# alainjungo/reliability-challenges-uncertainty

Hardware: AMD Instinct MI355X
Metric: MC-sample-volumes/sec (4x160x192x128, T=20) (higher is better)
Workload: dtype f32; 1 GPU; BraTS baseline_mc: 2D U-Net(2,4,depth 4,start_filters 32,dropout 0.05) over 160 slices of 4x192x128, T=20 MC-dropout passes + weight-scaling pass + mean/entropy aggregation per step; T=20, ws_pass=True, slices=160, height=192, width=128, pass_group=4, lanes=2, samples_per_launch=640, outputs=mean + entropy (MultiPredictionSummary() as every shipped script constructs it)

## Files before the change

### reliability-challenges-uncertainty_amd/csrc/rcu_api.hip

```cpp
#include "../../include/rcu.h"
#include "rcu_kernels.h"
#include "rcu_wpack.h"

#include <algorithm>
#include <cmath>
#include <cstdio>
#include <cstring>
#include <map>
#include <memory>
#include <string>
#include <vector>

using namespace rcu;

static thread_local std::string g_last_error;

static int fail(int code, const std::string& msg)
{
    g_last_error = msg;
    return code;
}
int rcu::report_error(int code, const std::string& msg) { return fail(code, msg); }
static int hip_fail(hipError_t e, const char* what)
{
    return fail(RCU_ERR_HIP, std::string(what) + ": " + hipGetErrorString(e));
}
#define RCU_HIP(call)                                      \
    do {                                                   \
        hipError_t e_ = (call);                            \
        if (e_ != hipSuccess) return hip_fail(e_, #call);  \
    } while (0)

static inline int round_up(int v, int m) { return (v + m - 1) / m * m; }

struct ConvLayer {
    std::string name;
    std::string bn;
    std::string name2, bn2;
    int cin1 = 0, cin2 = 0;
    int c1p = 0, c2p = 0;
    int cout = 0;
    int coutp = 0;
    int csplit = 0;
    int H = 0, W = 0;
    int level = 0;
    int gh = 0, gw = 0;
    int upsample = 0, relu = 0;
    int is_1x1 = 0;
    int accumulate = 0;
    int site = -1, site2 = -1;
    int cfg = 0, NT = 0;
    int t_src1 = -1, t_src2 = -1, t_out = -1, t_pool = -1;
    float *wpack = nullptr, *alpha = nullptr, *betab = nullptr, *beta = nullptr;
    size_t wpack_floats = 0;
};

struct Tensor {
    size_t floats_per_slice = 0;
    float* dev = nullptr;
    bool zero_fill = false;
    int H = 0, W = 0, cp = 0;
    int Hr = 0, Wr = 0;
    bool padded() const { return H != Hr || W != Wr; }
    bool blocked = false;
};

struct Workspace {
    std::vector<float*> dev;
    std::vector<size_t> bytes;
    int max_batch = 0;
    ~Workspace()
    {
        for (float* p : dev)
            if (p) (void)hipFree(p);
    }
};

struct rcu_unet {
    rcu_unet_desc d{};
    rcu_unet_options opt{};
    std::shared_ptr<Workspace> ws;
    bool ws_borrowed = false;
    std::vector<ConvLayer> layers;
    std::vector<Tensor> tensors;
    std::vector<std::pair<int, int>> level_ext;
    std::vector<std::pair<std::string, int>> sites;
    std::vector<int> site_offset;
    int mask_floats = 0;
    int in_cp = 0, head_cp = 0, head_cph = 0;
    int t_input = -1, t_head = -1;
    int t_features = -1;
    std::map<std::string, std::vector<float>> host_weights;
    float *w_cls = nullptr, *b_cls = nullptr, *w_sig = nullptr, *b_sig = nullptr;
    double temperature = 1.0;
    bool finalized = false;
    bool plan_only = false;
    int64_t workspace_bytes = 0;
    std::vector<void*> allocs;
    std::vector<hipEvent_t> prof_events;
    int prof_capacity = 0, prof_used = 0;
};

static int prof_slots(const rcu_unet* h) { return (int)h->layers.size() + 3; }

static int new_tensor(rcu_unet* h, int level, int Hr, int Wr, int cp)
{
    Tensor t;
    t.Hr = Hr; t.Wr = Wr; t.cp = cp;
    t.H = level >= 0 ? h->level_ext[level].first : Hr;
    t.W = level >= 0 ? h->level_ext[level].second : Wr;
    t.floats_per_slice = (size_t)t.H * t.W * cp;
    h->tensors.push_back(t);
    return (int)h->tensors.size() - 1;
}

static bool unit_has_dropout(const rcu_unet_desc& d, int level, bool is_down, int i)
{
    if (!d.has_dropout) return false;
    if (d.dropout_center < 0) return true;
    if (level == d.depth) return false;
    if (level + d.dropout_center >= d.depth) return is_down ? (i == 1) : (i == 0);
    return false;
}

static bool is_head_unit(const ConvLayer& L) { return L.name.rfind("conv_cls.0", 0) == 0; }

constexpr long kUpconv4MinItems = 480;
constexpr long long kUpconv4MinPlanPixels = 480LL * 192 * 128;
static bool upconv4_wins(int cfg, const ConvLayer& L, int n_slices)
{
    const ConvConfigInfo& ci = conv_config_info(cfg);
    const long items = (long)((n_slices + ci.TS - 1) / ci.TS) * (L.gh / ci.TH) * (L.gw / ci.TW) * (L.coutp / ci.BN);
    const int l = L.level - 1;
    const long long plan_pixels = (long long)n_slices * ((long long)L.H << l) * ((long long)L.W << l);
    return items >= kUpconv4MinItems && plan_pixels >= kUpconv4MinPlanPixels;
}

static int pick_config(const ConvLayer& L, int n_slices, const rcu_unet_options& opt, int oh, int ow)
{
    const bool wino_on = opt.conv_winograd != 0 && !L.accumulate;
    const int gh = L.gh, gw = L.gw;
    const size_t in_px = (size_t)gh * gw;
    const size_t max_bytes = (size_t)n_slices * std::max(in_px * (size_t)std::max(L.c1p, L.c2p), (size_t)oh * ow * (size_t)L.coutp) * 4;
    const bool center_pad = L.upsample && (2 * (L.H / 2) != L.H || 2 * (L.W / 2) != L.W);
    if (L.upsample && !center_pad && wino_on && L.c1p % 32 == 0 && L.c2p == 0 && max_bytes < ((size_t)1 << 31)) {
        const int lh = gh, lw = gw;
        const int u4_mode = opt.upconv_winograd4;
        const bool u4_fits = u4_mode != 0 && 2 * lh == L.H && 2 * lw == L.W && oh == L.H && ow == L.W &&
                             (size_t)(n_slices + 8) * std::max(in_px * (size_t)L.c1p, (size_t)oh * ow * (size_t)L.coutp) * 4 < ((size_t)1 << 32);
        if (u4_fits) {
            const int cfg4 = (lh % 16 == 0 && lw % 16 == 0) ? CONV_CFG_UPW4_T32x32_N32
                             : (lh % 8 == 0 && lw % 16 == 0) ? CONV_CFG_UPW4_S2T16x32_N32
                             : (lh % 4 == 0 && lw == 8)      ? CONV_CFG_UPW4_S8T8x16_N32
                                                             : -1;
            if (cfg4 >= 0 && (u4_mode == 2 || upconv4_wins(cfg4, L, n_slices))) return cfg4;
        }
        if (L.coutp == 32 && lh % 16 == 0 && lw % 32 == 0) return CONV_CFG_UPW_T16x32_N32;
        if (L.coutp > 32 && lh % 16 == 0 && lw % 16 == 0) return CONV_CFG_UPW_T16x16_N64;
        if (L.coutp > 32 && lh % 8 == 0 && lw % 16 == 0) return CONV_CFG_UPW_S2T8x16_N64;
        if (L.coutp > 32 && lh % 4 == 0 && lw == 8) return CONV_CFG_UPW_S8T4x8_N64;
    }
    if (L.upsample) {
        if (L.coutp <= 32) return (gh % 16 == 0 && gw % 16 == 0) ? CONV_CFG_UP_T16x16_N32 : CONV_CFG_UP_T8x16_N32;
        if (gh == 12 && gw == 8) return CONV_CFG_UP_S2T12x8_N64;
        return CONV_CFG_UP_T8x16_N64;
    }
    if (L.c1p + L.c2p == 8) {
        const bool first_on = opt.conv_first != 0;
        if (first_on && L.c2p == 0 && gh % 8 == 0 && gw % 32 == 0 && (L.coutp == 32 || L.coutp == 64) && L.t_pool < 0 &&
            L.name2.empty() && !L.accumulate)
            return CONV_CFG_FIRST_T8x32;
        return CONV_CFG_T8x16_N32_FIRST;
    }
    if (wino_on && (L.c1p + L.c2p) % 32 == 0 && (L.c2p == 0 || L.c2p == L.c1p) && max_bytes < ((size_t)1 << 31)) {
        const int w4_mode = opt.conv_winograd4;
        const bool lone_head = is_head_unit(L) && L.name2.empty();
        const bool w4_ok = w4_mode != 0 && (L.coutp >= 64 || w4_mode != 3) &&
                           !(lone_head && (opt.head_winograd4 == 0 || L.coutp != 32 || gh % 32 != 0 || gw % 32 != 0));
        if (w4_ok && gw % 32 == 0) {
            if (gh % 32 == 0) return CONV_CFG_WINO4_T32x32_N32;
            if (gh % 16 == 0) return CONV_CFG_WINO4_S2T16x32_N32;
        }
        if (w4_ok && gw == 32 && gh % 8 == 0) return CONV_CFG_WINO4_S4T8x32_N32;
        if (w4_ok && gw == 16 && gh % 8 == 0) return CONV_CFG_WINO4_S8T8x16_N32;
        if (w4_ok && gw == 8 && gh % 12 == 0 && L.t_pool < 0) {
            const long long plan_pixels = (long long)n_slices * ((long long)L.H << L.level) * ((long long)L.W << L.level);
            const long groups2 = (n_slices + 7) / 8;
            const long groups4 = plan_pixels >= kUpconv4MinPlanPixels ? (n_slices + 9) / 10 : groups2;
            const long rounds4 = (groups4 * (gh / 12) * (L.coutp / 32) + 255) / 256;
            const long rounds2 = (groups2 * (gh / 4) * ((L.coutp + 63) / 64) + 255) / 256;
            if (w4_mode == 2 || L.coutp <= 32 || (double)rounds4 * 1.35 < (double)rounds2) return CONV_CFG_WINO4_S8T12x8_N32;
        }
        if (L.coutp == 32 && gh % 16 == 0 && gw % 32 == 0) return CONV_CFG_WINO_T16x32_N32;
        if (L.coutp > 32 && gh % 16 == 0 && gw % 16 == 0) return CONV_CFG_WINO_T16x16_N64;
        if (L.coutp > 32 && gh % 8 == 0 && gw % 16 == 0) return CONV_CFG_WINO_S2T8x16_N64;
        if (L.coutp > 32 && gh % 4 == 0 && gw == 8) return CONV_CFG_WINO_S8T4x8_N64;
    }
    if (L.coutp > 32) {
        if (gh == 12 && gw == 8) return CONV_CFG_S2T12x8_N64;
        const int nt = (L.coutp + 63) / 64;
        const long items = (long)((gh + 7) / 8) * ((gw + 15) / 16) * n_slices * nt;
        const double fill = (double)items / (double)((items + 767) / 768 * 768);
        if (nt == 1 || fill < 0.9) {
            if (gh % 16 == 0 && gw % 16 == 0) return CONV_CFG_T16x16_N64;
            if (gh % 8 == 0 && gw % 16 == 0 && n_slices % 2 == 0) return CONV_CFG_S2T8x16_N64;
        }
        return CONV_CFG_T8x16_N64;
    }
    return (gh % 16 == 0 && gw % 16 == 0) ? CONV_CFG_T16x16_N32 : CONV_CFG_T8x16_N32;
}

static void add_unit(rcu_unet* h, const std::string& prefix, int cin1, int c1p, int cin2, int c2p, int cout, int level, int H, int W,
                     bool dropout, int t_src1, int t_src2, int t_out, int t_pool, bool residual_tail = false)
{
    ConvLayer L;
    L.name = prefix + ".conv2d_batch_relu.conv";
    if (h->d.bn) L.bn = prefix + ".conv2d_batch_relu.bn";
    L.cin1 = cin1; L.c1p = c1p; L.cin2 = cin2; L.c2p = c2p;
    L.cout = cout; L.coutp = round_up(cout, 32); L.csplit = L.coutp;
    L.H = H; L.W = W; L.relu = residual_tail ? 0 : 1;
    L.level = level; L.gh = h->level_ext[level].first; L.gw = h->level_ext[level].second;
    L.accumulate = residual_tail ? 1 : 0;
    if (dropout) {
        L.site = (int)h->sites.size();
        h->sites.push_back({prefix + ".conv2d_batch_relu.dropout", cout});
    }
    L.t_src1 = t_src1; L.t_src2 = t_src2; L.t_out = t_out; L.t_pool = t_pool;
    h->layers.push_back(L);
}

static void add_residual_conv(rcu_unet* h, const std::string& prefix, int cin1, int c1p, int cin2, int c2p, int cout, int level, int H, int W,
                              int t_src1, int t_src2, int t_out)
{
    ConvLayer L;
    L.name = prefix + ".residual";
    L.is_1x1 = 1;
    L.cin1 = cin1; L.c1p = c1p; L.cin2 = cin2; L.c2p = c2p;
    L.cout = cout; L.coutp = round_up(cout, 32); L.csplit = L.coutp;
    L.H = H; L.W = W; L.relu = 0;
    L.level = level; L.gh = h->level_ext[level].first; L.gw = h->level_ext[level].second;
    L.t_src1 = t_src1; L.t_src2 = t_src2; L.t_out = t_out;
    h->layers.push_back(L);
}

static void assign_layouts(rcu_unet* h);

static bool cfg_handles_padding(int cfg) { return conv_config_info(cfg).family.part; }

static int build_plan_for(rcu_unet* h, bool* valid)
{
    const rcu_unet_desc& d = h->d;
    const int depth = d.depth;
    h->layers.clear();
    h->tensors.clear();
    h->sites.clear();
    h->in_cp = round_up(d.in_channels, 8);
    h->t_input = new_tensor(h, 0, d.height, d.width, h->in_cp);
    std::vector<int> skip(depth), skip_c(depth);
    int cur = h->t_input, cur_c = d.in_channels, cur_cp = h->in_cp;
    int c = d.start_filters;
    char buf[128];
    for (int l = 0; l < depth; ++l) {
        const int H = d.height >> l, W = d.width >> l, cp = round_up(c, 32);
        const int t_tmp = new_tensor(h, l, H, W, cp), t_skip = new_tensor(h, l, H, W, cp);
        const int t_pool = new_tensor(h, l + 1, H / 2, W / 2, cp);
        snprintf(buf, sizeof buf, "down_convs.%d.block.block.0", l);
        add_unit(h, buf, cur_c, cur_cp, 0, 0, c, l, H, W, unit_has_dropout(d, l, true, 0), cur, -1, t_tmp, -1);
        if (d.residual) {
            snprintf(buf, sizeof buf, "down_convs.%d.block", l);
            add_residual_conv(h, buf, cur_c, cur_cp, 0, 0, c, l, H, W, cur, -1, t_skip);
        }
        snprintf(buf, sizeof buf, "down_convs.%d.block.block.1", l);
        add_unit(h, buf, c, cp, 0, 0, c, l, H, W, unit_has_dropout(d, l, true, 1), t_tmp, -1, t_skip, t_pool, d.residual != 0);
        skip[l] = t_skip; skip_c[l] = c;
        cur = t_pool; cur_c = c; cur_cp = cp;
        c *= 2;
    }
    {
        const int H = d.height >> depth, W = d.width >> depth, cp = round_up(c, 32);
        const int t_tmp = new_tensor(h, depth, H, W, cp), t_out = new_tensor(h, depth, H, W, cp);
        add_unit(h, "bottom_convs.block.0", cur_c, cur_cp, 0, 0, c, depth, H, W, unit_has_dropout(d, depth, true, 0), cur, -1,
                 t_tmp, -1);
        if (d.residual) add_residual_conv(h, "bottom_convs", cur_c, cur_cp, 0, 0, c, depth, H, W, cur, -1, t_out);
        add_unit(h, "bottom_convs.block.1", c, cp, 0, 0, c, depth, H, W, unit_has_dropout(d, depth, true, 1), t_tmp, -1, t_out,
                 -1, d.residual != 0);
        cur = t_out; cur_c = c; cur_cp = cp;
    }
    for (int j = 0; j < depth; ++j) {
        const int l = depth - 1 - j;
        const int H = d.height >> l, W = d.width >> l;
        const int co = cur_c / 2, cop = round_up(co, 32);
        const int t_up = new_tensor(h, l, H, W, cop), t_tmp = new_tensor(h, l, H, W, cop), t_out = new_tensor(h, l, H, W, cop);
        ConvLayer U;
        snprintf(buf, sizeof buf, "up_convs.%d.upconv.1", j);
        U.name = buf;
        U.cin1 = cur_c; U.c1p = cur_cp; U.cout = co; U.coutp = cop; U.csplit = cop;
        U.H = H; U.W = W; U.upsample = 1; U.relu = 0;
        U.level = l + 1; U.gh = h->level_ext[l + 1].first; U.gw = h->level_ext[l + 1].second;
        U.t_src1 = cur; U.t_out = t_up;
        if (2 * (H / 2) != H || 2 * (W / 2) != W) h->tensors[t_up].zero_fill = true;
        h->layers.push_back(U);
        snprintf(buf, sizeof buf, "up_convs.%d.block.block.0", j);
        add_unit(h, buf, co, cop, skip_c[l], round_up(skip_c[l], 32), co, l, H, W, unit_has_dropout(d, l, false, 0), t_up,
                 skip[l], t_tmp, -1);
        if (d.residual) {
            snprintf(buf, sizeof buf, "up_convs.%d.block", j);
            add_residual_conv(h, buf, co, cop, skip_c[l], round_up(skip_c[l], 32), co, l, H, W, t_up, skip[l], t_out);
        }
        snprintf(buf, sizeof buf, "up_convs.%d.block.block.1", j);
        add_unit(h, buf, co, cop, 0, 0, co, l, H, W, unit_has_dropout(d, l, false, 1), t_tmp, -1, t_out, -1, d.residual != 0);
        cur = t_out; cur_c = co; cur_cp = cop;
    }
    {
        const int cp = round_up(cur_c, 32);
        h->head_cph = cp;
        h->head_cp = d.sigma_out ? 2 * cp : cp;
        h->t_head = new_tensor(h, -1, d.height, d.width, h->head_cp);
        add_unit(h, "conv_cls.0", cur_c, cur_cp, 0, 0, cur_c, 0, d.height, d.width, d.has_dropout != 0, cur, -1, h->t_head,
                 -1);
        ConvLayer& L = h->layers.back();
        if (d.sigma_out) {
            L.name2 = "conv_sigma.0.conv2d_batch_relu.conv";
            if (d.bn) L.bn2 = "conv_sigma.0.conv2d_batch_relu.bn";
            L.csplit = cp;
            L.coutp = 2 * cp;
            if (d.has_dropout) {
                L.site2 = (int)h->sites.size();
                h->sites.push_back({"conv_sigma.0.conv2d_batch_relu.dropout", cur_c});
            }
        }
    }
    h->t_features = -1;
    if (d.provide_features && h->tensors[h->layers.back().t_src1].padded()) {
        const Tensor& f = h->tensors[h->layers.back().t_src1];
        h->t_features = new_tensor(h, -1, f.Hr, f.Wr, f.cp);
    }
    h->site_offset.assign(h->sites.size() + 1, 0);
    for (size_t s = 0; s < h->sites.size(); ++s) h->site_offset[s + 1] = h->site_offset[s] + h->sites[s].second;
    h->mask_floats = h->site_offset.back();
    if (valid) *valid = true;
    for (ConvLayer& L : h->layers) {
        const Tensor& to = h->tensors[L.t_out];
        L.cfg = pick_config(L, h->d.max_batch, h->opt, to.H, to.W);
        const ConvConfigInfo& ci = conv_config_info(L.cfg);
        if ((L.c1p % ci.KC) != 0 || (L.c2p % ci.KC) != 0)
            return fail(RCU_ERR_INVALID, "internal: channel chunking does not divide for layer " + L.name);
        L.NT = (L.coutp + ci.BN - 1) / ci.BN;
        const bool src_padded = h->tensors[L.t_src1].padded() && L.t_src1 != h->t_input;
        const bool first_reads_caller = L.t_src1 == h->t_input && h->tensors[L.t_src1].padded();
        const bool out_padded = to.padded() && !(L.upsample && !cfg_handles_padding(L.cfg) && !h->tensors[L.t_src1].padded());
        if ((src_padded || first_reads_caller || out_padded) && !cfg_handles_padding(L.cfg) && valid) *valid = false;
    }
    assign_layouts(h);
    return RCU_OK;
}

static double plan_cost(const rcu_unet* h)
{
    double total = 0.0;
    for (const ConvLayer& L : h->layers) {
        const ConvConfigInfo& ci = conv_config_info(L.cfg);
        const double tiles = (double)((L.gh + ci.TH - 1) / ci.TH) * ((L.gw + ci.TW - 1) / ci.TW);
        const double px = tiles * ci.TH * ci.TW;
        const double kn = (double)(L.c1p + L.c2p) * (double)(L.NT * ci.BN);
        double eff = 0.0;
        switch (ci.family.id) {
            case ConvFamily::First: eff = 0.25; break;
            case ConvFamily::Wino4: eff = (L.c1p + L.c2p) <= 32 ? 0.45 : 0.58; break;
            case ConvFamily::Wino2Up: eff = 0.72; break;
            case ConvFamily::Wino4Up: eff = 0.70; break;
            case ConvFamily::Wino2: eff = 0.62; break;
            case ConvFamily::DirectUp: eff = 0.72; break;
            case ConvFamily::Direct: eff = 0.75; break;
        }
        total += px * kn * (ci.family.mults * ci.slot_factor) / eff;
    }
    return total;
}

static int choose_level_extents(rcu_unet* h)
{
    const rcu_unet_desc& d = h->d;
    h->level_ext.resize(d.depth + 1);
    for (int l = 0; l <= d.depth; ++l) h->level_ext[l] = {d.height >> l, d.width >> l};
    bool valid = true;
    int rc = build_plan_for(h, &valid);
    if (rc != RCU_OK || h->opt.pad_levels == 0 || h->opt.conv_winograd == 0) return rc;
    double best = plan_cost(h);
    static const int kRound[] = {4, 8, 12, 16, 32};
    for (int sweep = 0; sweep < 2; ++sweep)
        for (int l = 0; l <= d.depth; ++l) {
            const int Hl = d.height >> l, Wl = d.width >> l;
            std::pair<int, int> keep = h->level_ext[l];
            for (int rh : kRound)
                for (int rw : kRound) {
                    const std::pair<int, int> cand = {round_up(Hl, rh), round_up(Wl, rw)};
                    if (cand == keep || (rw == 12)) continue;
                    h->level_ext[l] = cand;
                    rc = build_plan_for(h, &valid);
                    if (rc != RCU_OK) return rc;
                    const double cost = plan_cost(h);
                    if (valid && cost < best * 0.999) {
                        best = cost;
                        keep = cand;
                    }
                }
            h->level_ext[l] = keep;
        }
    return build_plan_for(h, &valid);
}

static int build_plan(rcu_unet* h) { return choose_level_extents(h); }

static void assign_layouts(rcu_unet* h)
{
    const bool on = h->opt.act_layout == 0;
    for (Tensor& t : h->tensors) t.blocked = on && t.cp % 8 == 0 && !t.zero_fill;
    h->tensors[h->t_input].blocked = false;
    h->tensors[h->t_head].blocked = false;
    if (h->d.provide_features) h->tensors[h->layers.back().t_src1].blocked = false;
    for (bool changed = true; changed;) {
        changed = false;
        auto clear = [&](int t) {
            if (t >= 0 && h->tensors[t].blocked) {
                h->tensors[t].blocked = false;
                changed = true;
            }
        };
        for (const ConvLayer& L : h->layers) {
            const ConvFamilyTraits& family = conv_config_info(L.cfg).family;
            if (!family.reads_blocked) {
                clear(L.t_src1);
                clear(L.t_src2);
            }
            if (!family.writes_blocked) {
                clear(L.t_out);
                clear(L.t_pool);
            }
            if (L.t_src2 >= 0 && h->tensors[L.t_src1].blocked != h->tensors[L.t_src2].blocked) {
                clear(L.t_src1);
                clear(L.t_src2);
            }
        }
    }
}

extern "C" const char* rcu_last_error(void) { return g_last_error.c_str(); }
extern "C" const char* rcu_version(void) { return "librcu_hip 0.1.0 gfx950"; }

extern "C" void rcu_unet_default_options(rcu_unet_options* opts)
{
    if (!opts) return;
    std::memset(opts, 0, sizeof *opts);
    opts->conv_winograd = 1;
    opts->conv_winograd4 = 1;
    opts->conv_first = 1;
    opts->act_layout = 0;
    opts->fuse_head = 1;
    opts->head_winograd4 = 1;
    opts->pad_levels = 1;
    opts->upconv_winograd4 = 1;
}

static int make_plan(const rcu_unet_desc* desc, const rcu_unet_options* opts, const rcu_unet* donor, rcu_unet** out)
{
    if (!desc || !out) return fail(RCU_ERR_INVALID, "rcu_unet_create: null argument");
    const rcu_unet_desc& d = *desc;
    if (d.nb_classes < 1 || d.nb_classes > MAX_CLASSES) return fail(RCU_ERR_INVALID, "nb_classes must be in 1..8");
    if (d.in_channels < 1 || d.depth < 1 || d.depth > 8 || d.start_filters < 1 || d.max_batch < 1)
        return fail(RCU_ERR_INVALID, "rcu_unet_create: bad in_channels / depth / start_filters / max_batch");
    if (d.in_channels > 8 && d.in_channels % 32 != 0)
        return fail(RCU_ERR_INVALID, "in_channels must be <= 8 or a multiple of 32");
    const int div = 1 << d.depth;
    if (d.height < div || d.width < div)
        return fail(RCU_ERR_INVALID, "height and width must be at least 2^depth (one pixel at the bottom level)");
    rcu_unet_options o;
    rcu_unet_default_options(&o);
    if (opts) {
        o = *opts;
        if ((o.conv_winograd | 1) != 1 || (o.conv_winograd4 < 0 || o.conv_winograd4 > 3) ||
            (o.conv_first | 1) != 1 || (o.act_layout | 1) != 1 || (o.fuse_head | 1) != 1 || (o.head_winograd4 | 1) != 1 || (o.pad_levels | 1) != 1 ||
            (o.upconv_winograd4 < 0 || o.upconv_winograd4 > 2))
            return fail(RCU_ERR_INVALID, "rcu_unet_create_with: bad rcu_unet_options value");
    }
    rcu_unet* h = new rcu_unet();
    h->d = d;
    h->opt = o;
    if (donor && donor->ws && donor->ws->max_batch >= d.max_batch) h->d.max_batch = donor->ws->max_batch;
    int rc = build_plan(h);
    if (rc != RCU_OK) {
        delete h;
        return rc;
    }
    *out = h;
    return RCU_OK;
}

extern "C" int rcu_unet_plan(const rcu_unet_desc* desc, const rcu_unet_options* opts, rcu_unet** out)
{
    int rc = make_plan(desc, opts, nullptr, out);
    if (rc == RCU_OK) (*out)->plan_only = true;
    return rc;
}

extern "C" int rcu_unet_create_with(const rcu_unet_desc* desc, const rcu_unet_options* opts, rcu_unet* donor, rcu_unet** out)
{
    rcu_unet* h = nullptr;
    int rc = make_plan(desc, opts, donor, &h);
    if (rc != RCU_OK) return rc;
    const rcu_unet_desc& d = *desc;
    for (const Tensor& t : h->tensors)
        if (t.floats_per_slice * (size_t)h->d.max_batch >= (size_t)1 << 31) {
            delete h;
            return fail(RCU_ERR_INVALID, "max_batch too large: an activation tensor would exceed 2^31 elements");
        }
    if (donor) {
        bool same = donor->ws && donor->tensors.size() == h->tensors.size() && donor->ws->max_batch >= d.max_batch;
        for (size_t i = 0; same && i < h->tensors.size(); ++i) {
            const Tensor &a = h->tensors[i], &b = donor->tensors[i];
            same = a.floats_per_slice == b.floats_per_slice && a.H == b.H && a.W == b.W && a.Hr == b.Hr && a.Wr == b.Wr && a.cp == b.cp &&
                   a.blocked == b.blocked && a.zero_fill == b.zero_fill;
        }
        if (!same) {
            delete h;
            return fail(RCU_ERR_INVALID, "rcu_unet_create_with: the workspace donor's plan differs (shape, options) or is sized for a smaller batch");
        }
        h->ws = donor->ws;
        h->ws_borrowed = true;
        for (size_t i = 0; i < h->tensors.size(); ++i) h->tensors[i].dev = h->ws->dev[i];
        *out = h;
        return RCU_OK;
    }
    h->ws = std::make_shared<Workspace>();
    h->ws->max_batch = d.max_batch;
    bool zeroed = false;
    for (Tensor& t : h->tensors) {
        const size_t bytes = t.floats_per_slice * (size_t)d.max_batch * sizeof(float);
        hipError_t e = hipMalloc(reinterpret_cast<void**>(&t.dev), bytes);
        if (e != hipSuccess) {
            rcu_unet_destroy(h);
            return hip_fail(e, "hipMalloc(activation workspace)");
        }
        h->ws->dev.push_back(t.dev);
        h->ws->bytes.push_back(bytes);
        h->workspace_bytes += (int64_t)bytes;
        if (t.zero_fill || t.padded()) {
            e = hipMemset(t.dev, 0, bytes);
            if (e != hipSuccess) {
                rcu_unet_destroy(h);
                return hip_fail(e, "hipMemset(centre-pad border / level padding)");
            }
            zeroed = true;
        }
    }
    if (zeroed) {
        hipError_t e = hipStreamSynchronize(nullptr);
        if (e != hipSuccess) {
            rcu_unet_destroy(h);
            return hip_fail(e, "hipStreamSynchronize(level padding)");
        }
    }
    *out = h;
    return RCU_OK;
}

extern "C" int rcu_unet_create(const rcu_unet_desc* desc, rcu_unet** out) { return rcu_unet_create_with(desc, nullptr, nullptr, out); }

extern "C" int rcu_unet_set_fuse_head(rcu_unet* h, int on)
{
    if (!h) return fail(RCU_ERR_INVALID, "rcu_unet_set_fuse_head: null handle");
    h->opt.fuse_head = on ? 1 : 0;
    return RCU_OK;
}

extern "C" int rcu_unet_set_temperature(rcu_unet* h, double temperature)
{
    if (!h) return fail(RCU_ERR_INVALID, "rcu_unet_set_temperature: null handle");
    if (!std::isfinite(temperature) || !(temperature > 0.0))
        return fail(RCU_ERR_INVALID, "rcu_unet_set_temperature: the temperature must be finite and > 0");
    if (h->d.sigma_out)
        return fail(RCU_ERR_INVALID, "rcu_unet_set_temperature: a sigma_out model's sigma is in logit units; scaling the logits alone is not defined");
    if (h->finalized) return fail(RCU_ERR_STATE, "rcu_unet_set_temperature after rcu_unet_finalize_weights");
    h->temperature = temperature;
    return RCU_OK;
}

extern "C" int rcu_unet_destroy(rcu_unet* h)
{
    if (!h) return RCU_OK;
    for (void* p : h->allocs) (void)hipFree(p);
    for (hipEvent_t e : h->prof_events) (void)hipEventDestroy(e);
    delete h;
    return RCU_OK;
}

extern "C" int64_t rcu_unet_workspace_bytes(const rcu_unet* h) { return h ? h->workspace_bytes : 0; }
extern "C" int rcu_unet_num_dropout_sites(const rcu_unet* h) { return h ? (int)h->sites.size() : 0; }
extern "C" int rcu_unet_dropout_site_channels(const rcu_unet* h, int site)
{
    if (!h || site < 0 || site >= (int)h->sites.size()) return fail(RCU_ERR_INVALID, "bad dropout site index");
    return h->sites[site].second;
}
extern "C" const char* rcu_unet_dropout_site_name(const rcu_unet* h, int site)
{
    if (!h || site < 0 || site >= (int)h->sites.size()) return "";
    return h->sites[site].first.c_str();
}
extern "C" int rcu_unet_mask_floats_per_sample(const rcu_unet* h) { return h ? h->mask_floats : 0; }

extern "C" int rcu_unet_load_weight(rcu_unet* h, const char* name, const float* data, size_t count)
{
    if (!h || !name || (!data && count)) return fail(RCU_ERR_INVALID, "rcu_unet_load_weight: null argument");
    std::string key(name);
    if (key.rfind("module.", 0) == 0) key = key.substr(7);
    h->host_weights[key].assign(data, data + count);
    h->finalized = false;
    return RCU_OK;
}

static int get_weight(rcu_unet* h, const std::string& key, size_t count, const std::vector<float>** out)
{
    auto it = h->host_weights.find(key);
    if (it == h->host_weights.end()) return fail(RCU_ERR_WEIGHTS, "missing weight tensor '" + key + "'");
    if (it->second.size() != count)
        return fail(RCU_ERR_WEIGHTS, "weight tensor '" + key + "' has " + std::to_string(it->second.size()) +
                                         " elements, expected " + std::to_string(count));
    *out = &it->second;
    return RCU_OK;
}

template <typename T>
static int upload(rcu_unet* h, const std::vector<T>& host, T** dev)
{
    RCU_HIP(hipMalloc(reinterpret_cast<void**>(dev), host.size() * sizeof(T)));
    h->allocs.push_back(*dev);
    h->workspace_bytes += (int64_t)(host.size() * sizeof(T));
    RCU_HIP(hipMemcpy(*dev, host.data(), host.size() * sizeof(T), hipMemcpyHostToDevice));
    return RCU_OK;
}

static int fold_conv(rcu_unet* h, const ConvLayer& L, const std::string& conv, const std::string& bn, int co0,
                     std::vector<float>& wpack, std::vector<float>& alpha, std::vector<float>& betab,
                     std::vector<float>& beta)
{
    const int cin = L.cin1 + L.cin2;
    const std::vector<float>*w, *b;
    std::vector<float> w_centre;
    int rc;
    if (L.is_1x1) {
        if ((rc = get_weight(h, conv + ".weight", (size_t)L.cout * cin, &w))) return rc;
        w_centre.assign((size_t)L.cout * cin * 9, 0.f);
        for (size_t i = 0; i < (size_t)L.cout * cin; ++i) w_centre[i * 9 + 4] = (*w)[i];
        w = &w_centre;
    } else {
        rc = get_weight(h, conv + ".weight", (size_t)L.cout * cin * 9, &w);
    }
    if (rc) return rc;
    rc = get_weight(h, conv + ".bias", (size_t)L.cout, &b);
    if (rc) return rc;
    const std::vector<float>*g = nullptr, *bt = nullptr, *mu = nullptr, *var = nullptr;
    if (!bn.empty()) {
        if ((rc = get_weight(h, bn + ".weight", L.cout, &g))) return rc;
        if ((rc = get_weight(h, bn + ".bias", L.cout, &bt))) return rc;
        if ((rc = get_weight(h, bn + ".running_mean", L.cout, &mu))) return rc;
        if ((rc = get_weight(h, bn + ".running_var", L.cout, &var))) return rc;
    }
    for (int co = 0; co < L.cout; ++co) {
        float A = 1.f, B = 0.f;
        if (g) {
            A = (*g)[co] / std::sqrt((*var)[co] + 1e-5f);
            B = (*bt)[co] - A * (*mu)[co];
        }
        alpha[co0 + co] = A;
        betab[co0 + co] = A * (*b)[co];
        beta[co0 + co] = B;
    }
    pack_conv_weights(wpack_kernel(conv_config_info(L.cfg)), WpackLayer{L.cin1, L.c1p, L.cin2, L.cout, L.NT, L.upsample}, w->data(), co0, wpack.data());
    return RCU_OK;
}

extern "C" int rcu_unet_finalize_weights(rcu_unet* h)
{
    if (!h) return fail(RCU_ERR_INVALID, "null handle");
    if (h->plan_only) return fail(RCU_ERR_STATE, "rcu_unet_finalize_weights: the handle is a plan without a workspace (rcu_unet_plan)");
    if (h->finalized) return RCU_OK;
    for (ConvLayer& L : h->layers) {
        const ConvConfigInfo& ci = conv_config_info(L.cfg);
        L.wpack_floats = wpack_floats(wpack_kernel(ci), L.c1p + L.c2p, L.NT);
        std::vector<float> wpack(L.wpack_floats, 0.f);
        const int cpad = L.NT * ci.BN;
        std::vector<float> alpha(cpad, 0.f), betab(cpad, 0.f), beta(cpad, 0.f);
        int rc = fold_conv(h, L, L.name, L.bn, 0, wpack, alpha, betab, beta);
        if (rc) return rc;
        if (!L.name2.empty()) {
            rc = fold_conv(h, L, L.name2, L.bn2, L.csplit, wpack, alpha, betab, beta);
            if (rc) return rc;
        }
        if ((rc = upload(h, wpack, &L.wpack))) return rc;
        if ((rc = upload(h, alpha, &L.alpha))) return rc;
        if ((rc = upload(h, betab, &L.betab))) return rc;
        if ((rc = upload(h, beta, &L.beta))) return rc;
    }
    const int C = h->d.nb_classes, cph = h->head_cph, creal = h->layers.back().cout;
    auto head = [&](const std::string& key, float** w_dev, float** b_dev, double temperature) -> int {
        const std::vector<float>*w, *b;
        int rc = get_weight(h, key + ".weight", (size_t)C * creal, &w);
        if (rc) return rc;
        if ((rc = get_weight(h, key + ".bias", (size_t)C, &b))) return rc;
        auto scaled = [temperature](float v) { return temperature == 1.0 ? v : (float)((double)v / temperature); };
        std::vector<float> wp((size_t)C * cph, 0.f);
        for (int c = 0; c < C; ++c)
            for (int k = 0; k < creal; ++k) wp[(size_t)c * cph + k] = scaled((*w)[(size_t)c * creal + k]);
        if ((rc = upload(h, wp, w_dev))) return rc;
        std::vector<float> bp(b->size());
        for (size_t c = 0; c < b->size(); ++c) bp[c] = scaled((*b)[c]);
        return upload(h, bp, b_dev);
    };
    int rc = head("conv_cls.1", &h->w_cls, &h->b_cls, h->temperature);
    if (rc) return rc;
    if (h->d.sigma_out && (rc = head("conv_sigma.1", &h->w_sig, &h->b_sig, 1.0))) return rc;
    h->host_weights.clear();
    h->finalized = true;
    return RCU_OK;
}

static bool head_fusable(const rcu_unet* h)
{
    const ConvLayer& last = h->layers.back();
    return conv_config_info(last.cfg).head_cfg >= 0 && h->d.nb_classes == 2 && last.name2.empty() && h->head_cph == 32;
}

struct FusedHead {
    float* logits;
    void* stats;
    int flags;
    int passes;
};

static int run_layer(rcu_unet* h, const ConvLayer& L, int n, const float* masks, hipStream_t stream, const FusedHead* head = nullptr,
                     const float* x_nchw = nullptr, int n_images = 0)
{
    const ConvConfigInfo& ci = conv_config_info(L.cfg);
    ConvArgs a{};
    a.src1 = h->tensors[L.t_src1].dev;
    a.src2 = L.t_src2 >= 0 ? h->tensors[L.t_src2].dev : nullptr;
    a.wpack = L.wpack; a.alpha = L.alpha; a.betab = L.betab; a.beta = L.beta;
    a.mask = (masks && L.site >= 0) ? masks + (size_t)n * h->site_offset[L.site] : nullptr;
    a.mask2 = (masks && L.site2 >= 0) ? masks + (size_t)n * h->site_offset[L.site2] : nullptr;
    a.out = h->tensors[L.t_out].dev;
    a.pooled = L.t_pool >= 0 ? h->tensors[L.t_pool].dev : nullptr;
    const int gh = L.gh, gw = L.gw;
    a.N = n; a.H = gh; a.W = gw;
    const Tensor& tsrc = h->tensors[L.t_src1];
    const Tensor& tout = h->tensors[L.t_out];
    const int os = L.upsample ? 2 : 1;
    if (cfg_handles_padding(L.cfg)) {
        const bool pool_differs = L.t_pool >= 0 && (h->tensors[L.t_pool].H != gh / 2 || h->tensors[L.t_pool].W != gw / 2);
        if (tsrc.padded() || tout.H != os * gh || tout.W != os * gw || pool_differs) {
            a.part = 1;
            a.Hr = L.upsample ? 2 * (L.H / 2) : L.H;
            a.Wr = L.upsample ? 2 * (L.W / 2) : L.W;
            a.out_H = tout.H; a.out_W = tout.W;
            if (L.t_pool >= 0) { a.pool_H = h->tensors[L.t_pool].H; a.pool_W = h->tensors[L.t_pool].W; }
        }
    } else if (L.t_pool >= 0 && h->tensors[L.t_pool].padded()) {
        a.pool_H = h->tensors[L.t_pool].H; a.pool_W = h->tensors[L.t_pool].W;
    } else if (L.upsample && (2 * gh != tout.H || 2 * gw != tout.W)) {
        a.out_H = tout.H; a.out_W = tout.W;
        a.out_y0 = (L.H - 2 * gh) / 2; a.out_x0 = (L.W - 2 * gw) / 2;
    }
    a.C1 = L.c1p; a.C2 = L.c2p; a.CoutP = L.coutp;
    a.cin_real = L.cin1;
    a.x_nchw = ci.family.id == ConvFamily::First ? x_nchw : nullptr;
    a.n_images = n_images;
    a.Cmask = L.cout; a.Csplit = L.csplit; a.Cmask2 = L.cout;
    a.relu = L.relu;
    a.accumulate = L.accumulate;
    a.tiles_y = (gh + ci.TH - 1) / ci.TH;
    a.tiles_x = (gw + ci.TW - 1) / ci.TW;
    a.slice_groups = (n + ci.TS - 1) / ci.TS;
    a.NT = L.NT;
    a.NTW_total = L.NT * ci.family.weight_sets;
    {
        const unsigned long long items = (unsigned long long)a.NTW_total * a.tiles_x * a.tiles_y * a.slice_groups;
        auto magic = [&](int d) -> uint32_t {
            return (d > 1 && items * (unsigned long long)d < (1ull << 32)) ? (uint32_t)(((1ull << 32) + d - 1) / d) : 0u;
        };
        a.magic_ntw = magic(a.NTW_total); a.magic_tx = magic(a.tiles_x); a.magic_ty = magic(a.tiles_y);
    }
    {
        auto strides = [](const Tensor& t, uint32_t& pix_bytes, uint32_t& chunk_bytes) {
            pix_bytes = t.blocked ? 32u : (uint32_t)t.cp * 4u;
            chunk_bytes = t.blocked ? (uint32_t)(t.H * t.W) * 32u : 32u;
        };
        strides(h->tensors[L.t_src1], a.in_pix_bytes, a.in_chunk_bytes);
        strides(h->tensors[L.t_out], a.out_pix_bytes, a.out_chunk_bytes);
        if (L.t_pool >= 0) strides(h->tensors[L.t_pool], a.pool_pix_bytes, a.pool_chunk_bytes);
    }
    a.src1_bytes = (uint32_t)std::min<size_t>(h->tensors[L.t_src1].floats_per_slice * (size_t)n * 4, 0xFFFFFFFFu);
    a.src2_bytes = L.t_src2 >= 0 ? (uint32_t)std::min<size_t>(h->tensors[L.t_src2].floats_per_slice * (size_t)n * 4, 0xFFFFFFFFu) : 0u;
    a.wpack_bytes = (uint32_t)std::min<size_t>(L.wpack_floats * 4, 0xFFFFFFFFu);
    int cfg = L.cfg;
    if (head) {
        cfg = ci.head_cfg;
        a.head_w = h->w_cls; a.head_b = h->b_cls;
        a.head_logits = head->logits; a.head_stats = head->stats; a.head_flags = head->flags;
        a.head_passes = head->passes;
        a.head_images = n / head->passes;
        a.head_V = (size_t)a.head_images * L.H * L.W;
    }
    RCU_HIP(launch_conv3x3(cfg, a, stream));
    return RCU_OK;
}

struct HeadSampling {
    const uint64_t* keys;
    uint64_t first_sample;
    int samples;
};

struct HeadVotes {
    uint32_t* plane;
    int n_words;
    const int32_t* bits;
};

static int forward_impl(rcu_unet* h, const float* x, int n, const float* masks, float* logits, float* sigma, void* stats,
                        int flags, hipStream_t stream, int passes = 1, float* sigma_sum = nullptr, int sigma_log = 0,
                        const HeadSampling* sampling = nullptr, const HeadVotes* votes = nullptr)
{
    if (!h || !x) return fail(RCU_ERR_INVALID, "rcu_unet_forward: null argument");
    if (!h->finalized) return fail(RCU_ERR_STATE, "rcu_unet_forward before rcu_unet_finalize_weights");
    if (n < 1 || passes < 1 || (long)n * passes > h->d.max_batch)
        return fail(RCU_ERR_INVALID, "batch size (times passes) outside 1..max_batch");
    if (passes > 1 && (!stats || logits || sigma)) return fail(RCU_ERR_INVALID, "pass groups only feed the statistics");
    const int n_one = n;
    n *= passes;
    if ((sigma || sigma_sum) && !h->d.sigma_out) return fail(RCU_ERR_INVALID, "sigma output requested from a model without sigma_out");
    hipEvent_t* ev = nullptr;
    if (h->prof_capacity > 0 && h->prof_used < h->prof_capacity)
        ev = h->prof_events.data() + (size_t)(h->prof_used++) * prof_slots(h);
    if (ev) RCU_HIP(hipEventRecord(*ev++, stream));
    const bool direct_input = conv_config_info(h->layers.front().cfg).family.id == ConvFamily::First;
    if (!direct_input)
        RCU_HIP(launch_pack_input(x, h->tensors[h->t_input].dev, n_one, h->d.in_channels, h->in_cp, h->d.height, h->d.width,
                                  h->tensors[h->t_input].H, h->tensors[h->t_input].W, passes, stream));
    if (ev) RCU_HIP(hipEventRecord(*ev++, stream));
    const ConvLayer& last = h->layers.back();
    const bool fuse = head_fusable(h) && sigma == nullptr && (logits != nullptr || stats != nullptr) && h->opt.fuse_head != 0 && sampling == nullptr &&
                      votes == nullptr;
    for (const ConvLayer& L : h->layers) {
        const FusedHead fh{logits, stats, flags, passes};
        int rc = run_layer(h, L, n, masks, stream, (fuse && &L == &last) ? &fh : nullptr, direct_input ? x : nullptr, n_one);
        if (rc) return rc;
        if (ev) RCU_HIP(hipEventRecord(*ev++, stream));
    }
    if (h->t_features >= 0) {
        const Tensor& f = h->tensors[h->layers.back().t_src1];
        RCU_HIP(launch_crop_nhwc(f.dev, h->tensors[h->t_features].dev, n, f.Hr, f.Wr, f.H, f.W, f.cp, stream));
    }
    if (fuse) {
        if (ev) RCU_HIP(hipEventRecord(*ev++, stream));
        return RCU_OK;
    }
    HeadArgs a{};
    a.act = h->tensors[h->t_head].dev;
    a.w_cls = h->w_cls; a.b_cls = h->b_cls; a.w_sig = h->w_sig; a.b_sig = h->b_sig;
    a.logits = logits; a.sigma = sigma; a.stats = stats;
    a.sigma_sum = sigma_sum; a.sigma_log = sigma_log;
    a.C = h->d.nb_classes; a.CP = h->head_cp; a.CPh = h->head_cph; a.stats_flags = flags;
    a.HW = (size_t)h->d.height * h->d.width;
    a.V = a.HW * n_one;
    a.passes = passes;
    if (sampling) {
        static_assert(sizeof(unsigned long long) == sizeof(uint64_t), "pass keys");
        RCU_HIP(launch_head_sampled(a, reinterpret_cast<const unsigned long long*>(sampling->keys), sampling->first_sample, sampling->samples, stream));
    } else if (votes) {
        RCU_HIP(launch_head_votes(a, votes->plane, votes->n_words, votes->bits, stream));
    } else {
        RCU_HIP(launch_head(a, stream));
    }
    if (ev) RCU_HIP(hipEventRecord(*ev++, stream));
    return RCU_OK;
}

extern "C" int rcu_unet_profile_begin(rcu_unet* h, int max_forwards)
{
    if (!h || max_forwards < 0) return fail(RCU_ERR_INVALID, "rcu_unet_profile_begin: bad argument");
    for (hipEvent_t e : h->prof_events) (void)hipEventDestroy(e);
    h->prof_events.clear();
    h->prof_capacity = h->prof_used = 0;
    const size_t total = (size_t)max_forwards * prof_slots(h);
    h->prof_events.resize(total);
    for (size_t i = 0; i < total; ++i) {
        hipError_t e = hipEventCreate(&h->prof_events[i]);
        if (e != hipSuccess) {
            h->prof_events.resize(i);
            return hip_fail(e, "hipEventCreate");
        }
    }
    h->prof_capacity = max_forwards;
    return RCU_OK;
}

extern "C" int rcu_unet_profile_collect(rcu_unet* h, double* ms_sum, int* forwards)
{
    if (!h || !ms_sum || !forwards) return fail(RCU_ERR_INVALID, "rcu_unet_profile_collect: null argument");
    const int slots = prof_slots(h);
    for (int i = 0; i < slots - 1; ++i) ms_sum[i] = 0.0;
    for (int f = 0; f < h->prof_used; ++f) {
        hipEvent_t* ev = h->prof_events.data() + (size_t)f * slots;
        RCU_HIP(hipEventSynchronize(ev[slots - 1]));
        for (int i = 0; i < slots - 1; ++i) {
            float ms = 0.f;
            RCU_HIP(hipEventElapsedTime(&ms, ev[i], ev[i + 1]));
            ms_sum[i] += ms;
        }
    }
    *forwards = h->prof_used;
    h->prof_used = 0;
    return RCU_OK;
}

extern "C" int rcu_unet_forward(rcu_unet* h, const float* x_dev, int n, const float* masks_dev, float* logits_dev,
                                float* sigma_dev, void* stream)
{
    return forward_impl(h, x_dev, n, masks_dev, logits_dev, sigma_dev, nullptr, 0, static_cast<hipStream_t>(stream));
}

extern "C" int rcu_unet_forward_accumulate(rcu_unet* h, const float* x_dev, int n, const float* masks_dev, void* stats_dev,
                                           int flags, void* stream)
{
    if (!stats_dev) return fail(RCU_ERR_INVALID, "rcu_unet_forward_accumulate: null stats");
    return forward_impl(h, x_dev, n, masks_dev, nullptr, nullptr, stats_dev, flags & (RCU_MC_MI | RCU_MC_VAR | RCU_MC_EXACT),
                        static_cast<hipStream_t>(stream));
}

extern "C" int rcu_unet_forward_accumulate_sigma(rcu_unet* h, const float* x_dev, int n, const float* masks_dev, void* stats_dev,
                                                 int flags, float* sigma_sum_dev, int is_log_sigma, void* stream)
{
    if (!stats_dev || !sigma_sum_dev) return fail(RCU_ERR_INVALID, "rcu_unet_forward_accumulate_sigma: null stats / sigma sum");
    return forward_impl(h, x_dev, n, masks_dev, nullptr, nullptr, stats_dev, flags & (RCU_MC_MI | RCU_MC_VAR | RCU_MC_EXACT),
                        static_cast<hipStream_t>(stream), 1, sigma_sum_dev, is_log_sigma ? 1 : 0);
}

extern "C" int rcu_unet_forward_accumulate_sigma_passes(rcu_unet* h, const float* x_dev, int n, int passes, const float* masks_dev,
                                                        void* stats_dev, int flags, float* sigma_sum_dev, int is_log_sigma, void* stream)
{
    if (!stats_dev || !sigma_sum_dev) return fail(RCU_ERR_INVALID, "rcu_unet_forward_accumulate_sigma_passes: null stats / sigma sum");
    return forward_impl(h, x_dev, n, masks_dev, nullptr, nullptr, stats_dev, flags & (RCU_MC_MI | RCU_MC_VAR | RCU_MC_EXACT),
                        static_cast<hipStream_t>(stream), passes, sigma_sum_dev, is_log_sigma ? 1 : 0);
}

extern "C" int rcu_unet_forward_sample_sigma_passes(rcu_unet* h, const float* x_dev, int n, int passes, const float* masks_dev,
                                                    const uint64_t* keys_host, uint64_t first_sample, int samples, void* stats_dev, int flags,
                                                    float* sigma_sum_dev, int is_log_sigma, void* stream)
{
    const char* fn = "rcu_unet_forward_sample_sigma_passes";
    if (!h) return fail(RCU_ERR_INVALID, std::string(fn) + ": null handle");
    if (!x_dev || !keys_host || !stats_dev || !sigma_sum_dev)
        return fail(RCU_ERR_INVALID, std::string(fn) + ": null x_dev / keys_host / stats_dev / sigma_sum_dev");
    if (!h->d.sigma_out) return fail(RCU_ERR_INVALID, std::string(fn) + ": the handle has no sigma head (sigma_out = 0)");
    if (n < 1 || passes < 1 || (long)n * passes > h->d.max_batch)
        return fail(RCU_ERR_INVALID, std::string(fn) + ": batch size (times passes) outside 1..max_batch");
    if (int st = check_logit_sampling_shape(fn, (size_t)n, (size_t)h->d.height * h->d.width, h->d.nb_classes, samples)) return st;
    const HeadSampling sampling{keys_host, first_sample, samples};
    return forward_impl(h, x_dev, n, masks_dev, nullptr, nullptr, stats_dev, flags & (RCU_MC_MI | RCU_MC_VAR | RCU_MC_EXACT),
                        static_cast<hipStream_t>(stream), passes, sigma_sum_dev, is_log_sigma ? 1 : 0, &sampling);
}

extern "C" int rcu_unet_features(const rcu_unet* h, const float** features_dev, int* channels, int* channel_pitch)
{
    if (!h || !features_dev) return fail(RCU_ERR_INVALID, "rcu_unet_features: null argument");
    if (!h->finalized) return fail(RCU_ERR_STATE, "rcu_unet_features before rcu_unet_finalize_weights");
    for (const ConvLayer& L : h->layers)
        if (L.name == "conv_cls.0.conv2d_batch_relu.conv") {
            if (h->tensors[L.t_src1].blocked || (h->tensors[L.t_src1].padded() && h->t_features < 0))
                return fail(RCU_ERR_STATE, "rcu_unet_features: the handle was created without rcu_unet_desc.provide_features (the feature "
                                           "tensor is held channel-blocked / on a padded level)");
            *features_dev = h->t_features >= 0 ? h->tensors[h->t_features].dev : h->tensors[L.t_src1].dev;
            if (channels) *channels = L.cin1;
            if (channel_pitch) *channel_pitch = L.c1p;
            return RCU_OK;
        }
    return fail(RCU_ERR_STATE, "rcu_unet_features: no conv_cls layer in the plan");
}

struct rcu_postnet {
    int in_channels = 0, nb_classes = 0, nb_convs = 0, bn = 1;
    std::map<std::string, std::vector<float>> host_weights;
    float* packed = nullptr;
    float* packed_mc = nullptr;
    bool finalized = false;
};

extern "C" int rcu_postnet_create(int in_channels, int nb_classes, int nb_convs, int bn, rcu_postnet** out)
{
    if (!out) return fail(RCU_ERR_INVALID, "rcu_postnet_create: null argument");
    if (in_channels < 1 || in_channels > 32 * PN_MAX_BLOCKS)
        return fail(RCU_ERR_INVALID, "PostNet kernel handles 1.." + std::to_string(32 * PN_MAX_BLOCKS) + " feature channels");
    if (nb_classes < 1 || nb_classes > 32) return fail(RCU_ERR_INVALID, "PostNet kernel handles 1..32 classes");
    if (nb_convs < 0 || nb_convs + 1 > PN_MAX_LAYERS)
        return fail(RCU_ERR_INVALID, "PostNet kernel handles at most " + std::to_string(PN_MAX_LAYERS - 1) + " hidden convs");
    const int cb = (in_channels + 31) / 32;
    if ((size_t)(nb_convs + 1) * pn_layer_floats(cb) * sizeof(float) > 160 * 1024)
        return fail(RCU_ERR_INVALID, "PostNet: the packed layers of " + std::to_string(nb_convs) + " hidden convs over " +
                                         std::to_string(in_channels) + " channels do not fit the 160 KB of LDS");
    rcu_postnet* h = new rcu_postnet;
    h->in_channels = in_channels; h->nb_classes = nb_classes; h->nb_convs = nb_convs; h->bn = bn ? 1 : 0;
    *out = h;
    return RCU_OK;
}

extern "C" void rcu_postnet_destroy(rcu_postnet* h)
{
    if (!h) return;
    if (h->packed) (void)hipFree(h->packed);
    if (h->packed_mc) (void)hipFree(h->packed_mc);
    delete h;
}

extern "C" int rcu_postnet_load_weight(rcu_postnet* h, const char* name, const float* data, size_t count)
{
    if (!h || !name || (!data && count)) return fail(RCU_ERR_INVALID, "rcu_postnet_load_weight: null argument");
    std::string key(name);
    if (key.rfind("module.", 0) == 0) key = key.substr(7);
    h->host_weights[key].assign(data, data + count);
    h->finalized = false;
    return RCU_OK;
}

static int postnet_weight(rcu_postnet* h, const std::string& key, size_t count, const std::vector<float>** out)
{
    auto it = h->host_weights.find(key);
    if (it == h->host_weights.end()) return fail(RCU_ERR_WEIGHTS, "missing weight tensor '" + key + "'");
    if (it->second.size() != count)
        return fail(RCU_ERR_WEIGHTS, "weight tensor '" + key + "' has " + std::to_string(it->second.size()) +
                                         " elements, expected " + std::to_string(count));
    *out = &it->second;
    return RCU_OK;
}

static void postnet_pack_layer(int cb, const std::vector<float>& w, const std::vector<float>& start, const std::vector<float>& after,
                               float* dst)
{
    const int cp = 32 * cb;
    for (int cob = 0; cob < cb; ++cob)
        for (int cib = 0; cib < cb; ++cib)
            for (int j = 0; j < 4; ++j)
                for (int lane = 0; lane < 64; ++lane)
                    for (int e = 0; e < 4; ++e)
                        dst[((((cob * cb + cib) * 4 + j) * 64) + lane) * 4 + e] =
                            w[(size_t)(32 * cob + (lane & 31)) * cp + 32 * cib + 8 * j + 4 * (lane >> 5) + e];
    float* bd = dst + cb * cb * 1024;
    for (int which = 0; which < 2; ++which)
        for (int cob = 0; cob < cb; ++cob)
            for (int j = 0; j < 4; ++j)
                for (int hf = 0; hf < 2; ++hf)
                    for (int e = 0; e < 4; ++e)
                        bd[which * cb * 32 + ((cob * 4 + j) * 2 + hf) * 4 + e] = (which ? after : start)[32 * cob + 8 * j + 4 * hf + e];
}

extern "C" int rcu_postnet_finalize_weights(rcu_postnet* h)
{
    if (!h) return fail(RCU_ERR_INVALID, "rcu_postnet_finalize_weights: null handle");
    const int C = h->in_channels, L = h->nb_convs + 1, cb = (C + 31) / 32, cp = 32 * cb;
    const size_t layer = pn_layer_floats(cb);
    std::vector<float> packed((size_t)L * layer, 0.f), packed_mc((size_t)L * layer, 0.f);
    for (int l = 0; l < L; ++l) {
        const bool last = (l == h->nb_convs);
        const std::string pre = last ? "conv_logits" : "convs." + std::to_string(l) + ".conv2d_batch_relu.conv";
        const int cout = last ? h->nb_classes : C;
        const std::vector<float>*w, *b;
        int rc = postnet_weight(h, pre + ".weight", (size_t)cout * C, &w);
        if (rc) return rc;
        if ((rc = postnet_weight(h, pre + ".bias", cout, &b))) return rc;
        std::vector<float> wf((size_t)cp * cp, 0.f), b_conv(cp, 0.f), b_shift(cp, 0.f), b_all(cp, 0.f);
        for (int o = 0; o < cout; ++o) {
            float alpha = 1.f, beta = 0.f, mean = 0.f;
            if (!last && h->bn) {
                const std::string bp = "convs." + std::to_string(l) + ".conv2d_batch_relu.bn";
                const std::vector<float>*g, *be, *rm, *rv;
                if ((rc = postnet_weight(h, bp + ".weight", C, &g))) return rc;
                if ((rc = postnet_weight(h, bp + ".bias", C, &be))) return rc;
                if ((rc = postnet_weight(h, bp + ".running_mean", C, &rm))) return rc;
                if ((rc = postnet_weight(h, bp + ".running_var", C, &rv))) return rc;
                alpha = (float)((double)(*g)[o] / std::sqrt((double)(*rv)[o] + 1e-5));
                beta = (*be)[o];
                mean = (*rm)[o];
            }
            for (int i = 0; i < C; ++i) wf[(size_t)o * cp + i] = alpha * (*w)[(size_t)o * C + i];
            b_all[o] = alpha * ((*b)[o] - mean) + beta;
            b_conv[o] = alpha * (*b)[o];
            b_shift[o] = beta - alpha * mean;
        }
        postnet_pack_layer(cb, wf, b_all, std::vector<float>(cp, 0.f), packed.data() + (size_t)l * layer);
        postnet_pack_layer(cb, wf, last ? b_all : b_conv, b_shift, packed_mc.data() + (size_t)l * layer);
    }
    if (!h->packed) RCU_HIP(hipMalloc(reinterpret_cast<void**>(&h->packed), packed.size() * sizeof(float)));
    if (!h->packed_mc) RCU_HIP(hipMalloc(reinterpret_cast<void**>(&h->packed_mc), packed_mc.size() * sizeof(float)));
    RCU_HIP(hipMemcpy(h->packed, packed.data(), packed.size() * sizeof(float), hipMemcpyHostToDevice));
    RCU_HIP(hipMemcpy(h->packed_mc, packed_mc.data(), packed_mc.size() * sizeof(float), hipMemcpyHostToDevice));
    h->finalized = true;
    return RCU_OK;
}

extern "C" int rcu_postnet_forward(rcu_postnet* h, const float* features_dev, int channel_pitch, int n, int hw,
                                   const float* masks_dev, float* logits_dev, void* stream)
{
    if (!h || !features_dev || !logits_dev) return fail(RCU_ERR_INVALID, "rcu_postnet_forward: null argument");
    if (!h->finalized) return fail(RCU_ERR_STATE, "rcu_postnet_forward before rcu_postnet_finalize_weights");
    if (n < 0 || hw < 1) return fail(RCU_ERR_INVALID, "rcu_postnet_forward: bad shape");
    const int cb = (h->in_channels + 31) / 32;
    if (channel_pitch < 32 * cb || channel_pitch % 4)
        return fail(RCU_ERR_INVALID, "rcu_postnet_forward: channel pitch must be >= in_channels rounded up to 32 and a multiple of 4");
    RCU_HIP(launch_postnet(features_dev, channel_pitch, (size_t)n * hw, hw, masks_dev ? h->packed_mc : h->packed, h->nb_convs + 1,
                           h->nb_classes, h->in_channels, masks_dev, logits_dev, static_cast<hipStream_t>(stream)));
    return RCU_OK;
}

extern "C" int rcu_unet_forward_accumulate_passes(rcu_unet* h, const float* x_dev, int n, int passes, const float* masks_dev,
                                                  void* stats_dev, int flags, void* stream)
{
    if (!stats_dev) return fail(RCU_ERR_INVALID, "rcu_unet_forward_accumulate_passes: null stats");
    return forward_impl(h, x_dev, n, masks_dev, nullptr, nullptr, stats_dev, flags & (RCU_MC_MI | RCU_MC_VAR | RCU_MC_EXACT),
                        static_cast<hipStream_t>(stream), passes);
}

static int check_vote_plane(const std::string& fn, int n_words)
{
    if (n_words < 1 || n_words > RCU_VOTES_MAX_PASSES / 32) return fail(RCU_ERR_INVALID, fn + ": n_words must be in 1..2, got " + std::to_string(n_words));
    return RCU_OK;
}
static int check_vote_bit(const std::string& fn, int bit, int n_words)
{
    if (bit < 0 || bit >= 32 * n_words)
        return fail(RCU_ERR_INVALID, fn + ": bit " + std::to_string(bit) + " outside [0, " + std::to_string(32 * n_words) + ")");
    return RCU_OK;
}

extern "C" int rcu_unet_forward_accumulate_votes(rcu_unet* h, const float* x_dev, int n, int passes, const float* masks_dev, void* stats_dev,
                                                 int flags, uint32_t* votes_dev, int n_words, const int32_t* bits_host, void* stream)
{
    const std::string fn = "rcu_unet_forward_accumulate_votes";
    if (!h) return fail(RCU_ERR_INVALID, fn + ": null handle");
    if (!x_dev || !stats_dev || !votes_dev || !bits_host) return fail(RCU_ERR_INVALID, fn + ": null x_dev / stats_dev / votes_dev / bits_host");
    if (int st = check_vote_plane(fn, n_words)) return st;
    if (h->d.nb_classes < 1 || h->d.nb_classes > MAX_CLASSES) return fail(RCU_ERR_INVALID, fn + ": nb_classes must be in 1..8");
    if (n < 1 || passes < 1 || (long)n * passes > h->d.max_batch) return fail(RCU_ERR_INVALID, fn + ": batch size (times passes) outside 1..max_batch");
    for (int t = 0; t < passes; ++t)
        if (int st = check_vote_bit(fn, bits_host[t], n_words)) return st;
    const HeadVotes votes{votes_dev, n_words, bits_host};
    return forward_impl(h, x_dev, n, masks_dev, nullptr, nullptr, stats_dev, flags & (RCU_MC_MI | RCU_MC_VAR | RCU_MC_EXACT),
                        static_cast<hipStream_t>(stream), passes, nullptr, 0, nullptr, &votes);
}

extern "C" int rcu_mc_votes(const float* in_dev, size_t n, size_t hw, int nb_classes, int flags, uint32_t* votes_dev, int n_words, int bit, void* stream)
{
    const std::string fn = "rcu_mc_votes";
    if (!in_dev || !votes_dev) return fail(RCU_ERR_INVALID, fn + ": null in_dev / votes_dev");
    if (int st = check_vote_plane(fn, n_words)) return st;
    if (int st = check_vote_bit(fn, bit, n_words)) return st;
    if (nb_classes < 1 || nb_classes > MAX_CLASSES) return fail(RCU_ERR_INVALID, fn + ": nb_classes must be in 1..8");
    if (n * hw == 0) return RCU_OK;
    RCU_HIP(launch_mc_votes(in_dev, nb_classes, n, hw, flags & RCU_MC_INPUT_PROBS, votes_dev, bit, static_cast<hipStream_t>(stream)));
    return RCU_OK;
}

extern "C" int rcu_unet_num_layers(const rcu_unet* h) { return h ? (int)h->layers.size() : 0; }

extern "C" int rcu_unet_layer_info(const rcu_unet* h, int layer, rcu_layer_info* out)
{
    if (!h || !out || layer < 0 || layer >= (int)h->layers.size()) return fail(RCU_ERR_INVALID, "bad layer index");
    const ConvLayer& L = h->layers[layer];
    std::memset(out, 0, sizeof *out);
    std::snprintf(out->name, sizeof out->name, "%s", L.name.c_str());
    std::snprintf(out->kernel, sizeof out->kernel, "%s", conv_config_info(L.cfg).kernel_name);
    out->cin = L.cin1 + L.cin2;
    out->cout = L.name2.empty() ? L.cout : 2 * L.cout;
    out->height = L.H; out->width = L.W;
    out->grid_height = L.gh; out->grid_width = L.gw;
    out->upsample = L.upsample; out->pooled = L.t_pool >= 0; out->dual_source = L.t_src2 >= 0;
    out->head_fusable = (layer + 1 == (int)h->layers.size() && head_fusable(h)) ? 1 : 0;
    out->flops_per_slice = 2.0 * out->cin * out->cout * (L.is_1x1 ? 1.0 : 9.0) * (L.upsample ? 4.0 * (L.H / 2) * (L.W / 2) : (double)L.H * L.W);
    {
        const ConvConfigInfo& ci = conv_config_info(L.cfg);
        const double tiles = (double)((L.gh + ci.TH - 1) / ci.TH) * ((L.gw + ci.TW - 1) / ci.TW);
        const double px = tiles * ci.TH * ci.TW;
        const double ncols = (double)L.NT * ci.BN;
        const int k = ci.family.id == ConvFamily::First ? (L.cin1 > 4 ? 8 : 4) : L.c1p + L.c2p;
        out->mfma_flops_per_slice = 2.0 * k * ncols * ci.family.mults * px * ci.slot_factor;
    }
    return RCU_OK;
}

extern "C" int rcu_unet_run_layer(rcu_unet* h, int layer, int n, const float* masks_dev, void* stream)
{
    if (!h || layer < 0 || layer >= (int)h->layers.size()) return fail(RCU_ERR_INVALID, "bad layer index");
    if (!h->finalized) return fail(RCU_ERR_STATE, "rcu_unet_run_layer before rcu_unet_finalize_weights");
    if (n < 1 || n > h->d.max_batch) return fail(RCU_ERR_INVALID, "batch size outside 1..max_batch");
    return run_layer(h, h->layers[layer], n, masks_dev, static_cast<hipStream_t>(stream));
}

static int check_classes(int c)
{
    if (c < 1 || c > MAX_CLASSES) return fail(RCU_ERR_INVALID, "nb_classes must be in 1..8");
    return RCU_OK;
}

extern "C" size_t rcu_mc_stats_bytes(size_t n, size_t hw, int C, int flags)
{
    const size_t V = n * hw;
    const size_t mi = (flags & RCU_MC_MI) ? 1 : 0;
    if (flags & (RCU_MC_VAR | RCU_MC_EXACT)) return V * ((size_t)C + ((flags & RCU_MC_VAR) ? (size_t)C : 0) + mi) * sizeof(double);
    return V * ((size_t)C + mi) * sizeof(float);
}

extern "C" int rcu_mc_begin(void* stats, size_t n, size_t hw, int C, int flags, void* stream)
{
    if (!stats) return fail(RCU_ERR_INVALID, "rcu_mc_begin: null stats");
    if (check_classes(C)) return RCU_ERR_INVALID;
    RCU_HIP(hipMemsetAsync(stats, 0, rcu_mc_stats_bytes(n, hw, C, flags), static_cast<hipStream_t>(stream)));
    return RCU_OK;
}

extern "C" int rcu_mc_accumulate(const float* in, void* stats, size_t n, size_t hw, int C, int flags, void* stream)
{
    if (!in || !stats) return fail(RCU_ERR_INVALID, "rcu_mc_accumulate: null argument");
    if (check_classes(C)) return RCU_ERR_INVALID;
    if (n * hw == 0) return RCU_OK;
    RCU_HIP(launch_mc_accumulate(in, stats, C, n, hw, flags, static_cast<hipStream_t>(stream)));
    return RCU_OK;
}

extern "C" int rcu_mc_finalize(const void* stats, size_t n, size_t hw, int C, int T, int flags, float* mean, float* entropy,
                               float* mi, float* var, void* stream)
{
    if (!stats) return fail(RCU_ERR_INVALID, "rcu_mc_finalize: null stats");
    if (check_classes(C)) return RCU_ERR_INVALID;
    if (T < 1) return fail(RCU_ERR_INVALID, "rcu_mc_finalize: T must be >= 1");
    if (mi && !(flags & RCU_MC_MI)) return fail(RCU_ERR_INVALID, "mutual_info requested without RCU_MC_MI statistics");
    if (var && !(flags & RCU_MC_VAR)) return fail(RCU_ERR_INVALID, "variance requested without RCU_MC_VAR statistics");
    if ((flags & RCU_MC_EXACT) && T > RCU_MC_EXACT_MAX_PASSES)
        return fail(RCU_ERR_INVALID, "RCU_MC_EXACT statistics hold at most 2048 passes (sums of multiples of 2^-40 below 2^13)");
    if (n * hw == 0) return RCU_OK;
    RCU_HIP(launch_mc_finalize(stats, C, n, hw, T, flags, mean, entropy, mi, var, static_cast<hipStream_t>(stream)));
    return RCU_OK;
}

extern "C" int rcu_softmax(const float* logits, float* probs, size_t n, size_t hw, int C, void* stream)
{
    if (!logits || !probs) return fail(RCU_ERR_INVALID, "rcu_softmax: null argument");
    if (check_classes(C)) return RCU_ERR_INVALID;
    if (n * hw == 0) return RCU_OK;
    RCU_HIP(launch_softmax_nchw(logits, probs, C, n, hw, static_cast<hipStream_t>(stream)));
    return RCU_OK;
}

extern "C" int rcu_aleatoric(const float* logits, const float* sigma_raw, size_t n, size_t hw, int C, int is_log_sigma,
                             float* probs, float* sigma, uint8_t* prediction, float* sigma_pred, void* stream)
{
    if (!logits || !sigma_raw) return fail(RCU_ERR_INVALID, "rcu_aleatoric: null argument");
    if (check_classes(C)) return RCU_ERR_INVALID;
    if (n * hw == 0) return RCU_OK;
    RCU_HIP(launch_aleatoric(logits, sigma_raw, C, n, hw, is_log_sigma, probs, sigma, prediction, sigma_pred,
                             static_cast<hipStream_t>(stream)));
    return RCU_OK;
}

extern "C" int rcu_prediction_and_foreground(const float* probs, size_t n, size_t hw, int C, uint8_t* prediction,
                                             float* p_fg, void* stream)
{
    if (!probs) return fail(RCU_ERR_INVALID, "rcu_prediction_and_foreground: null argument");
    if (check_classes(C)) return RCU_ERR_INVALID;
    if (n * hw == 0) return RCU_OK;
    RCU_HIP(launch_argmax_fg(probs, C, n, hw, prediction, p_fg, static_cast<hipStream_t>(stream)));
    return RCU_OK;
}

static int draw_dropout_masks(const std::string& fn, const uint64_t* seeds, int passes, int n, uint64_t first_sample, const int64_t* sample_index_dev,
                              const int32_t* site_channels, const float* site_keep, int n_sites, float* out, void* stream)
{
    if (!seeds || !site_channels || !site_keep || !out) return fail(RCU_ERR_INVALID, fn + ": null argument");
    if (passes < 1 || n < 1 || n_sites < 1 || n_sites > MASK_MAX_SITES) return fail(RCU_ERR_INVALID, fn + ": passes, n >= 1 and 1 <= n_sites <= 40");
    MaskArgs a{};
    long end = 0;
    for (int s = 0; s < n_sites; ++s) {
        if (site_channels[s] < 1 || !(site_keep[s] <= 1.f)) return fail(RCU_ERR_INVALID, fn + ": site_channels >= 1, site_keep <= 1");
        end += (long)n * site_channels[s];
        if (end * (long)passes >= (1l << 31)) return fail(RCU_ERR_INVALID, fn + ": more than 2^31 factors");
        a.site_end[s] = (int)end;
        a.site_keep[s] = site_keep[s];
        a.site_ch[s] = site_channels[s];
        a.site_off[s] = a.per_sample;
        a.per_sample += site_channels[s];
    }
    a.first_sample = first_sample;
    a.sites = n_sites;
    a.per_pass = (int)end;
    a.passes = passes;
    for (a.first = 0; a.first < passes; a.first += MASK_MAX_PASSES) {
        a.count = std::min(MASK_MAX_PASSES, passes - a.first);
        for (int t = 0; t < a.count; ++t) a.seed[t] = seeds[a.first + t];
        if (sample_index_dev) {
            RCU_HIP(launch_dropout_masks_indexed(a, reinterpret_cast<const long long*>(sample_index_dev), out, static_cast<hipStream_t>(stream)));
        } else {
            RCU_HIP(launch_dropout_masks(a, out, static_cast<hipStream_t>(stream)));
        }
    }
    return RCU_OK;
}

extern "C" int rcu_dropout_masks(const uint64_t* seeds, int passes, int n, uint64_t first_sample, const int32_t* site_channels,
                                 const float* site_keep, int n_sites, float* out, void* stream)
{
    return draw_dropout_masks("rcu_dropout_masks", seeds, passes, n, first_sample, nullptr, site_channels, site_keep, n_sites, out, stream);
}

static int check_adaptive_shape(const char* fn, size_t n, size_t hw, int C)
{
    if (check_classes(C)) return RCU_ERR_INVALID;
    if (n < 1 || hw < 1 || n > ((size_t)1 << 20) || hw > ((size_t)1 << 30))
        return fail(RCU_ERR_INVALID, std::string(fn) + ": n must be in 1..2^20 and hw in 1..2^30");
    return RCU_OK;
}

extern "C" int rcu_mc_slice_scores(const void* stats_dev, size_t n, size_t hw, int C, int flags, int64_t thr_q, uint32_t* unsettled_dev,
                                   int64_t* margin_q_dev, void* stream)
{
    if (!stats_dev || !unsettled_dev || !margin_q_dev) return fail(RCU_ERR_INVALID, "rcu_mc_slice_scores: null argument");
    if (check_adaptive_shape("rcu_mc_slice_scores", n, hw, C)) return RCU_ERR_INVALID;
    if (!(flags & RCU_MC_EXACT) || (flags & ~(RCU_MC_MI | RCU_MC_VAR | RCU_MC_EXACT)))
        return fail(RCU_ERR_INVALID, "rcu_mc_slice_scores: needs RCU_MC_EXACT statistics (the decision is made on exact integer sums), got flags " +
                                         std::to_string(flags));
    if (thr_q < 0) return fail(RCU_ERR_INVALID, "rcu_mc_slice_scores: thr_q must be >= 0");
    if (reinterpret_cast<uintptr_t>(stats_dev) % 8 != 0) return fail(RCU_ERR_INVALID, "rcu_mc_slice_scores: stats must be 8-byte aligned");
    RCU_HIP(launch_mc_slice_scores(stats_dev, C, n, hw, (long long)thr_q, unsettled_dev, reinterpret_cast<long long*>(margin_q_dev),
                                   static_cast<hipStream_t>(stream)));
    return RCU_OK;
}

extern "C" int rcu_dropout_masks_indexed(const uint64_t* seeds, int passes, int n, const int64_t* sample_index_dev, const int32_t* site_channels,
                                         const float* site_keep, int n_sites, float* out, void* stream)
{
    if (!sample_index_dev) return fail(RCU_ERR_INVALID, "rcu_dropout_masks_indexed: null argument");
    return draw_dropout_masks("rcu_dropout_masks_indexed", seeds, passes, n, 0, sample_index_dev, site_channels, site_keep, n_sites, out, stream);
}

extern "C" int rcu_mc_merge_slices(const void* src_stats_dev, size_t m, void* dst_stats_dev, size_t n, size_t hw, int C, int flags,
                                   const int32_t* index_dev, void* stream)
{
    if (!src_stats_dev || !dst_stats_dev || !index_dev) return fail(RCU_ERR_INVALID, "rcu_mc_merge_slices: null argument");
    if (check_adaptive_shape("rcu_mc_merge_slices", n, hw, C) || check_adaptive_shape("rcu_mc_merge_slices", m, hw, C)) return RCU_ERR_INVALID;
    if (flags & ~(RCU_MC_MI | RCU_MC_VAR | RCU_MC_EXACT))
        return fail(RCU_ERR_INVALID, "rcu_mc_merge_slices: flags must be a combination of RCU_MC_MI, RCU_MC_VAR and RCU_MC_EXACT, got " +
                                         std::to_string(flags));
    const uintptr_t s = reinterpret_cast<uintptr_t>(src_stats_dev), d = reinterpret_cast<uintptr_t>(dst_stats_dev);
    const size_t element = (flags & (RCU_MC_VAR | RCU_MC_EXACT)) ? 8 : 4;
    if (s % element != 0 || d % element != 0) return fail(RCU_ERR_INVALID, "rcu_mc_merge_slices: blobs must be aligned to their element");
    if (s < d + rcu_mc_stats_bytes(n, hw, C, flags) && d < s + rcu_mc_stats_bytes(m, hw, C, flags))
        return fail(RCU_ERR_INVALID, "rcu_mc_merge_slices: src and dst must not overlap");
    RCU_HIP(launch_mc_merge_slices(src_stats_dev, m, dst_stats_dev, n, hw, C, flags, index_dev, static_cast<hipStream_t>(stream)));
    return RCU_OK;
}

extern "C" int rcu_mc_finalize_counts(const void* stats, size_t n, size_t hw, int C, const int32_t* counts_dev, int flags, float* mean,
                                      float* entropy, float* mi, float* var, void* stream)
{
    if (!stats || !counts_dev) return fail(RCU_ERR_INVALID, "rcu_mc_finalize_counts: null argument");
    if (check_classes(C)) return RCU_ERR_INVALID;
    if (mi && !(flags & RCU_MC_MI)) return fail(RCU_ERR_INVALID, "mutual_info requested without RCU_MC_MI statistics");
    if (var && !(flags & RCU_MC_VAR)) return fail(RCU_ERR_INVALID, "variance requested without RCU_MC_VAR statistics");
    if (n * hw == 0) return RCU_OK;
    RCU_HIP(launch_mc_finalize_counts(stats, C, n, hw, counts_dev, flags, mean, entropy, mi, var, static_cast<hipStream_t>(stream)));
    return RCU_OK;
}

static_assert(sizeof(rcu_ece_result) == sizeof(EceResult), "ABI struct mismatch");
static_assert(RCU_MAX_BINS == MAX_BINS && RCU_MAX_THRESHOLDS == MAX_THR, "ABI constant mismatch");

extern "C" int rcu_ece_thresholds(int n_bins, float* thr)
{
    if (n_bins < 1 || n_bins > MAX_BINS || !thr) return fail(RCU_ERR_INVALID, "n_bins must be in 1..32");
    const double stop = 1.0 + 1e-8, step = stop / n_bins;
    for (int k = 1; k < n_bins; ++k) {
        const double edge = k * step;
        float t = (float)edge;
        if ((double)t < edge) t = std::nextafterf(t, INFINITY);
        thr[k - 1] = t;
    }
    return RCU_OK;
}

extern "C" size_t rcu_ece_workspace_bytes(size_t n, int nv) { return ece_workspace_bytes(n, nv < 1 ? 1 : nv); }

extern "C" int rcu_ece_hist(const float* p, const uint8_t* target, const uint8_t* mask, size_t n, int n_volumes,
                            const float* thr, int n_bins, rcu_ece_result* result, void* workspace, void* stream)
{
    if (!result || !thr || (n && (!p || !target || !workspace)))
        return fail(RCU_ERR_INVALID, "rcu_ece_hist: null argument");
    if (n_bins < 1 || n_bins > MAX_BINS || n_volumes < 1) return fail(RCU_ERR_INVALID, "rcu_ece_hist: bad n_bins / n_volumes");
    RCU_HIP(launch_ece_hist(p, target, mask, n, n_volumes, thr, n_bins, reinterpret_cast<EceResult*>(result), workspace,
                            static_cast<hipStream_t>(stream)));
    return RCU_OK;
}

extern "C" int rcu_ece_bin_ids(const float* p, size_t n, const float* thr, int n_bins, uint8_t* ids, void* stream)
{
    if ((n && (!p || !ids)) || !thr) return fail(RCU_ERR_INVALID, "rcu_ece_bin_ids: null argument");
    if (n_bins < 1 || n_bins > MAX_BINS) return fail(RCU_ERR_INVALID, "n_bins must be in 1..32");
    RCU_HIP(launch_bin_ids(p, n, thr, n_bins, ids, static_cast<hipStream_t>(stream)));
    return RCU_OK;
}

extern "C" int rcu_calib_set_blocks_per_workgroup(int ece_blocks, int unc_blocks)
{
    if (ece_blocks < 0 || unc_blocks < 0) return fail(RCU_ERR_INVALID, "rcu_calib_set_blocks_per_workgroup: negative block count");
    calib_set_blocks_per_workgroup(ece_blocks, unc_blocks);
    return RCU_OK;
}

extern "C" size_t rcu_unc_workspace_bytes(size_t n, int nv) { return unc_workspace_bytes(n, nv < 1 ? 1 : nv); }

extern "C" int rcu_unc_counts(const void* unc, int unc_is_f64, const uint8_t* prediction, const uint8_t* target,
                              const uint8_t* mask, size_t n, int n_volumes, const double* thr, int n_thr, uint64_t* counts,
                              void* workspace, void* stream)
{
    if (!counts || !thr || (n && (!unc || !prediction || !target || !workspace)))
        return fail(RCU_ERR_INVALID, "rcu_unc_counts: null argument");
    if (n_thr < 1 || n_thr > MAX_THR || n_volumes < 1)
        return fail(RCU_ERR_INVALID, "rcu_unc_counts: n_thr must be in 1..16 and n_volumes >= 1");
    RCU_HIP(launch_unc_counts(unc, unc_is_f64, prediction, target, mask, n, n_volumes, thr, n_thr,
                              reinterpret_cast<unsigned long long*>(counts), workspace, static_cast<hipStream_t>(stream)));
    return RCU_OK;
}

extern "C" int rcu_unc_from_p_num_thresholds(void) { return unc_from_p_num_thresholds(); }
extern "C" double rcu_unc_from_p_threshold(int i) { return unc_from_p_threshold(i); }
extern "C" int rcu_unc_from_p_supported(const double* thr, int n_thr) { return (thr && unc_from_p_supported(thr, n_thr)) ? 1 : 0; }
extern "C" int rcu_unc_from_p_exceeded(float p, const double* thr, int n_thr)
{
    if (!thr || n_thr < 1 || n_thr > MAX_THR) return -1;
    return unc_from_p_exceeded_host(p, thr, n_thr);
}
extern "C" size_t rcu_unc_from_p_workspace_bytes(size_t n, int nv) { return unc_from_p_workspace_bytes(n, nv < 1 ? 1 : nv); }

extern "C" int rcu_unc_counts_from_p(const float* p, const uint8_t* prediction, const uint8_t* target, const uint8_t* mask, size_t n,
                                     int n_volumes, const double* thr, int n_thr, uint64_t* counts, void* workspace, void* stream)
{
    if (!thr || !counts || !workspace || (n && (!p || !prediction || !target)))
        return fail(RCU_ERR_INVALID, "rcu_unc_counts_from_p: null argument");
    if (n_thr < 1 || n_thr > MAX_THR || n_volumes < 1) return fail(RCU_ERR_INVALID, "rcu_unc_counts_from_p: bad n_thr / n_volumes");
    if (!unc_from_p_supported(thr, n_thr))
        return fail(RCU_ERR_INVALID, "rcu_unc_counts_from_p: thresholds must be strictly ascending values of the built-in table (rcu_unc_from_p_threshold)");
    RCU_HIP(launch_unc_counts_from_p(p, prediction, target, mask, n, n_volumes, thr, n_thr, reinterpret_cast<unsigned long long*>(counts),
                                     workspace, static_cast<hipStream_t>(stream)));
    return RCU_OK;
}

extern "C" int rcu_normalised_entropy(const float* p_fg, size_t n, double* out64, float* out32, void* stream)
{
    if (n && !p_fg) return fail(RCU_ERR_INVALID, "rcu_normalised_entropy: null argument");
    RCU_HIP(launch_norm_entropy(p_fg, n, out64, out32, static_cast<hipStream_t>(stream)));
    return RCU_OK;
}
```

### reliability-challenges-uncertainty_amd/csrc/rcu_first.hip

```cpp
#include "rcu_kernels.h"

namespace rcu {

namespace {

typedef float f32x4 __attribute__((ext_vector_type(4)));

constexpr int FIRST_TH = 8, FIRST_TW = 32, FIRST_THREADS = 256;
constexpr int FIRST_HR = FIRST_TH + 2, FIRST_HC = FIRST_TW + 2;
constexpr int FIRST_TILE_FLOATS = 3072;

template <int KS, int NB>
__global__ __launch_bounds__(FIRST_THREADS) void conv3x3_first_kernel(const ConvArgs a, const int tiles_total)
{
    __shared__ __attribute__((aligned(16))) float tile[KS][FIRST_HR][FIRST_HC][4];
    const int tid = threadIdx.x, lane = tid & 63, wave = tid >> 6;
    const int n16 = lane & 15, g = lane >> 4;

    float wr[9][KS][NB];
#pragma unroll
    for (int tap = 0; tap < 9; ++tap)
#pragma unroll
        for (int ks = 0; ks < KS; ++ks)
#pragma unroll
            for (int b = 0; b < NB; ++b) {
                const int co = b * 16 + n16;
                wr[tap][ks][b] = a.wpack[(size_t)(co >> 5) * FIRST_TILE_FLOATS + (tap * 32 + (co & 31)) * 8 + ks * 4 + g];
            }
    f32x4 al[NB], bb[NB], be[NB];
#pragma unroll
    for (int b = 0; b < NB; ++b) {
        al[b] = *reinterpret_cast<const f32x4*>(a.alpha + b * 16 + 4 * g);
        bb[b] = *reinterpret_cast<const f32x4*>(a.betab + b * 16 + 4 * g);
        be[b] = *reinterpret_cast<const f32x4*>(a.beta + b * 16 + 4 * g);
    }
    const int tiles_x = a.W / FIRST_TW, tiles_y = a.H / FIRST_TH;
    const float floor_v = a.relu ? 0.f : -__builtin_inff();
    const int Hr = a.part ? a.Hr : a.H, Wr = a.part ? a.Wr : a.W;

    const int images = tiles_total / (tiles_x * tiles_y);
    const int passes = a.N / images;
    for (int t = blockIdx.x; t < tiles_total; t += gridDim.x) {
        const int tx = t % tiles_x, ty = (t / tiles_x) % tiles_y, n = t / (tiles_x * tiles_y);
        const int y0 = ty * FIRST_TH, x0 = tx * FIRST_TW;
        __syncthreads();
        for (int i = tid; i < KS * FIRST_HR * FIRST_HC; i += FIRST_THREADS) {
            const int ks = i / (FIRST_HR * FIRST_HC), rem = i % (FIRST_HR * FIRST_HC);
            const int r = rem / FIRST_HC, c = rem % FIRST_HC;
            const int gy = y0 + r - 1, gx = x0 + c - 1;
            f32x4 v = {0.f, 0.f, 0.f, 0.f};
            if (gy >= 0 && gy < Hr && gx >= 0 && gx < Wr) {
                if (a.x_nchw != nullptr) {
                    const size_t HW = (size_t)Hr * Wr;
                    const float* const px = a.x_nchw + (size_t)(n % a.n_images) * a.cin_real * HW + (size_t)gy * Wr + gx;
#pragma unroll
                    for (int k = 0; k < 4; ++k)
                        if (ks * 4 + k < a.cin_real) v[k] = px[(size_t)(ks * 4 + k) * HW];
                } else {
                    v = *reinterpret_cast<const f32x4*>(a.src1 + ((size_t)(n * a.H + gy) * a.W + gx) * a.C1 + ks * 4);
                }
            }
            *reinterpret_cast<f32x4*>(&tile[ks][r][c][0]) = v;
        }
        __syncthreads();
        f32x4 acc[4][NB];
#pragma unroll
        for (int seg = 0; seg < 4; ++seg) {
            const int r = 2 * wave + (seg >> 1), c0 = 16 * (seg & 1);
#pragma unroll
            for (int b = 0; b < NB; ++b) acc[seg][b] = f32x4{0.f, 0.f, 0.f, 0.f};
#pragma unroll
            for (int tap = 0; tap < 9; ++tap)
#pragma unroll
                for (int ks = 0; ks < KS; ++ks) {
                    const float xv = tile[ks][r + tap / 3][c0 + n16 + tap % 3][g];
#pragma unroll
                    for (int b = 0; b < NB; ++b) acc[seg][b] = __builtin_amdgcn_mfma_f32_16x16x4f32(wr[tap][ks][b], xv, acc[seg][b], 0, 0, 0);
                }
        }
        for (int pass = 0; pass < passes; ++pass) {
            const int ns = pass * images + n;
            f32x4 scale[NB], shift[NB];
#pragma unroll
            for (int b = 0; b < NB; ++b) {
                f32x4 mk = {1.f, 1.f, 1.f, 1.f};
                if (a.mask != nullptr) {
#pragma unroll
                    for (int j = 0; j < 4; ++j) {
                        const int c = b * 16 + 4 * g + j;
                        if (c < a.Cmask) mk[j] = a.mask[(size_t)ns * a.Cmask + c];
                    }
                }
                scale[b] = al[b] * mk;
                shift[b] = bb[b] * mk + be[b];
            }
#pragma unroll
            for (int seg = 0; seg < 4; ++seg) {
                const int r = 2 * wave + (seg >> 1), c0 = 16 * (seg & 1);
                if (y0 + r >= Hr || x0 + c0 + n16 >= Wr) continue;
                char* const op = reinterpret_cast<char*>(a.out) + (size_t)ns * a.H * a.W * a.CoutP * 4 +
                                 (size_t)((y0 + r) * a.W + x0 + c0 + n16) * a.out_pix_bytes + (size_t)(g >> 1) * a.out_chunk_bytes + (g & 1) * 16;
#pragma unroll
                for (int b = 0; b < NB; ++b) {
                    f32x4 v = acc[seg][b] * scale[b] + shift[b];
#pragma unroll
                    for (int j = 0; j < 4; ++j) v[j] = fmaxf(v[j], floor_v);
                    *reinterpret_cast<f32x4*>(op + (size_t)(2 * b) * a.out_chunk_bytes) = v;
                }
            }
        }
    }
}

template <int KS, int NB>
hipError_t launch_first(const ConvArgs& a, hipStream_t stream)
{
    const int images = (a.x_nchw != nullptr && a.n_images > 0 && a.N % a.n_images == 0) ? a.n_images : a.N;
    const int tiles = (a.H / FIRST_TH) * (a.W / FIRST_TW) * images;
    const int grid = tiles < 256 * 8 ? tiles : 256 * 8;
    hipLaunchKernelGGL((conv3x3_first_kernel<KS, NB>), dim3(grid), dim3(FIRST_THREADS), 0, stream, a, tiles);
    return hipGetLastError();
}

const ConvConfigInfo kFirstInfo = {1, FIRST_TH, FIRST_TW, 32, 8, 9, "conv3x3_first<T8x32,K36>", 8, 0, {ConvFamily::First, false, false, true, true, 1, 9.0}};

}

const ConvConfigInfo& first_config_info() { return kFirstInfo; }

hipError_t launch_conv_first(const ConvArgs& a, hipStream_t stream)
{
    if (a.C1 != 8 || a.C2 != 0 || a.H % FIRST_TH != 0 || a.W % FIRST_TW != 0 || a.pooled != nullptr || a.mask2 != nullptr ||
        (a.CoutP != 32 && a.CoutP != 64))
        return hipErrorInvalidValue;
    const bool wide = a.cin_real > 4;
    if (a.CoutP == 32) return wide ? launch_first<2, 2>(a, stream) : launch_first<1, 2>(a, stream);
    return wide ? launch_first<2, 4>(a, stream) : launch_first<1, 4>(a, stream);
}

}
```

### reliability-challenges-uncertainty_amd/csrc/rcu_kernels.h

```cpp
#pragma once
#include <hip/hip_runtime.h>
#include <stddef.h>
#include <stdint.h>

#include <string>

#include "../../include/rcu.h"

namespace rcu {

int report_error(int code, const std::string& msg);

inline int hip_failed(const char* fn, hipError_t e) { return report_error(RCU_ERR_HIP, std::string(fn) + ": " + hipGetErrorString(e)); }
inline size_t round256(size_t b) { return (b + 255) & ~(size_t)255; }
inline int check_n_volumes(const std::string& f, int n_volumes, int max_volumes)
{
    if (n_volumes >= 1 && n_volumes <= max_volumes) return RCU_OK;
    return report_error(RCU_ERR_INVALID, f + "n_volumes must be in 1.." + std::to_string(max_volumes) + ", got " + std::to_string(n_volumes));
}
inline bool batch_n_ok(size_t n) { return n != 0 && n < (size_t)0x7fffffff; }
inline bool batch_total_ok(size_t n, int n_volumes) { return (unsigned long long)n * (unsigned long long)n_volumes <= 0xffffffffull; }
inline bool batch_ok(size_t n, int n_volumes, int max_volumes)
{
    return batch_n_ok(n) && n_volumes >= 1 && n_volumes <= max_volumes && batch_total_ok(n, n_volumes);
}
inline int check_batch(const std::string& f, size_t n, int n_volumes, int max_volumes)
{
    if (!batch_n_ok(n)) return report_error(RCU_ERR_INVALID, f + "n_per_volume must be in 1..2^31-2, got " + std::to_string(n));
    if (int st = check_n_volumes(f, n_volumes, max_volumes)) return st;
    if (!batch_total_ok(n, n_volumes)) return report_error(RCU_ERR_INVALID, f + "n_per_volume * n_volumes must be below 2^32");
    return RCU_OK;
}

struct ConvArgs {
    const float* src1;
    const float* src2;
    const float* wpack;
    const float* alpha;
    const float* betab;
    const float* beta;
    const float* mask;
    const float* mask2;
    float* out;
    float* pooled;
    int out_H, out_W;
    int out_y0, out_x0;
    int N, H, W;
    int part;
    int Hr, Wr;
    int pool_H, pool_W;
    int C1, C2;
    int cin_real;
    const float* x_nchw;
    int n_images;
    int CoutP;
    int Cmask;
    int Csplit, Cmask2;
    int relu;
    int accumulate;
    int tiles_y, tiles_x, slice_groups;
    int NT;
    uint32_t magic_ntw, magic_tx, magic_ty;
    int NTW_total;
    uint32_t src1_bytes, src2_bytes, wpack_bytes;
    uint32_t in_pix_bytes, in_chunk_bytes;
    uint32_t out_pix_bytes, out_chunk_bytes;
    uint32_t pool_pix_bytes, pool_chunk_bytes;
    const float* head_w;
    const float* head_b;
    float* head_logits;
    void* head_stats;
    int head_flags;
    size_t head_V;
    int head_passes;
    int head_images;
};

enum ConvConfig {
    CONV_CFG_T8x16_N64 = 0,
    CONV_CFG_T8x16_N32 = 1,
    CONV_CFG_T8x16_N32_FIRST = 2,
    CONV_CFG_S2T12x8_N64 = 3,
    CONV_CFG_UP_T8x16_N64 = 4,
    CONV_CFG_UP_T8x16_N32 = 5,
    CONV_CFG_UP_S2T12x8_N64 = 6,
    CONV_CFG_T16x16_N32 = 7,
    CONV_CFG_UP_T16x16_N32 = 8,
    CONV_CFG_T16x16_N64 = 9,
    CONV_CFG_S2T8x16_N64 = 10,
    CONV_CFG_COUNT,
    CONV_CFG_WINO_T16x16_N64 = CONV_CFG_COUNT,
    CONV_CFG_WINO_T16x32_N32,
    CONV_CFG_WINO_S2T8x16_N64,
    CONV_CFG_WINO_S8T4x8_N64,
    CONV_CFG_WINO_T16x32_N32_HEAD,
    CONV_CFG_UPW_T16x16_N64,
    CONV_CFG_UPW_T16x32_N32,
    CONV_CFG_UPW_S2T8x16_N64,
    CONV_CFG_UPW_S8T4x8_N64,
    CONV_CFG_FIRST_T8x32,
    CONV_CFG_WINO4_T32x32_N32,
    CONV_CFG_WINO4_S2T16x32_N32,
    CONV_CFG_WINO4_S8T8x16_N32,
    CONV_CFG_WINO4_S8T12x8_N32,
    CONV_CFG_WINO4_T32x32_N32_HEAD,
    CONV_CFG_WINO4_S4T8x32_N32,
    CONV_CFG_UPW4_T32x32_N32,
    CONV_CFG_UPW4_S2T16x32_N32,
    CONV_CFG_UPW4_S8T8x16_N32,
    CONV_CFG_END
};

enum class ConvFamily {
    Direct,
    DirectUp,
    First,
    Wino2,
    Wino2Up,
    Wino4,
    Wino4Up,
};
struct ConvFamilyTraits {
    ConvFamily id;
    bool winograd;
    bool reads_blocked;
    bool writes_blocked;
    bool part;
    int weight_sets;
    double mults;
};
struct ConvConfigInfo {
    int TS, TH, TW, BN, KC, TAPS;
    const char* kernel_name;
    int KCP;
    int SWZ;
    ConvFamilyTraits family;
    double slot_factor = 1.0;
    int head_cfg = -1;
};
const ConvConfigInfo& conv_config_info(int cfg);
const ConvConfigInfo& wino_config_info(int cfg);
const ConvConfigInfo& wino_up_config_info(int cfg);
const ConvConfigInfo& wino4_config_info(int cfg);
const ConvConfigInfo& wino4_up_config_info(int cfg);
const ConvConfigInfo& first_config_info();
hipError_t launch_conv3x3(int cfg, const ConvArgs& a, hipStream_t stream);
hipError_t launch_conv_wino(int cfg, const ConvArgs& a, hipStream_t stream);
hipError_t launch_upconv_wino(int cfg, const ConvArgs& a, hipStream_t stream);
hipError_t launch_conv_wino4(int cfg, const ConvArgs& a, hipStream_t stream);
hipError_t launch_upconv_wino4(int cfg, const ConvArgs& a, hipStream_t stream);
hipError_t launch_conv_first(const ConvArgs& a, hipStream_t stream);

#if defined(__HIPCC__)
template <class V>
__device__ __forceinline__ V stream_load_as(const void* p)
{
    return __builtin_nontemporal_load(reinterpret_cast<const V*>(p));
}
__device__ __forceinline__ float stream_load(const float* p) { return stream_load_as<float>(p); }
__device__ __forceinline__ unsigned stream_load(const unsigned* p) { return stream_load_as<unsigned>(p); }
__device__ __forceinline__ float4 stream_load(const float4* p)
{
    typedef float v4 __attribute__((ext_vector_type(4)));
    const v4 v = stream_load_as<v4>(p);
    return float4{v.x, v.y, v.z, v.w};
}
__device__ __forceinline__ double2 stream_load(const double2* p)
{
    typedef double v2 __attribute__((ext_vector_type(2)));
    const v2 v = stream_load_as<v2>(p);
    return double2{v.x, v.y};
}
__device__ __forceinline__ void load4(const float* src, float (&q)[4])
{
    const float4 v = stream_load(reinterpret_cast<const float4*>(src));
    q[0] = v.x, q[1] = v.y, q[2] = v.z, q[3] = v.w;
}
__device__ __forceinline__ void load4(const double* src, double (&q)[4])
{
    const double2 a = stream_load(reinterpret_cast<const double2*>(src)), b = stream_load(reinterpret_cast<const double2*>(src + 2));
    q[0] = a.x, q[1] = a.y, q[2] = b.x, q[3] = b.y;
}
#endif

hipError_t set_max_dynamic_lds(const void* kernel, int bytes);

hipError_t launch_pack_input(const float* x_nchw, float* out_nhwc, int N, int C, int CP, int H, int W, int PH, int PW, int replicas,
                             hipStream_t stream);

hipError_t launch_crop_nhwc(const float* src, float* dst, int N, int H, int W, int PH, int PW, int CP, hipStream_t stream);

constexpr int MC_MI = 1;
constexpr int MC_VAR = 2;
constexpr int MC_INPUT_PROBS = 4;
constexpr int MC_EXACT = 8;
constexpr int MAX_CLASSES = 8;

struct HeadArgs {
    const float* act;
    const float* w_cls;
    const float* b_cls;
    const float* w_sig;
    const float* b_sig;
    float* logits;
    float* sigma;
    float* sigma_sum;
    int sigma_log;
    void* stats;
    int C, CP, CPh, stats_flags;
    size_t V, HW;
    int passes;
};
hipError_t launch_head(const HeadArgs& a, hipStream_t stream);
constexpr int LOGIT_MAX_SAMPLES = 1024;
constexpr int SAMPLE_MAX_PASSES = 32;
struct SampleArgs {
    unsigned long long keys[SAMPLE_MAX_PASSES];
    unsigned long long first_sample;
    int samples;
};
hipError_t launch_head_sampled(const HeadArgs& a, const unsigned long long* keys_host, unsigned long long first_sample, int samples,
                               hipStream_t stream);
constexpr int VOTES_MAX_PASSES = RCU_VOTES_MAX_PASSES;
struct VoteArgs {
    uint32_t* plane;
    int n_words;
    int word;
    unsigned char bit[SAMPLE_MAX_PASSES];
};
hipError_t launch_head_votes(const HeadArgs& a, uint32_t* votes, int n_words, const int32_t* bits_host, hipStream_t stream);
hipError_t launch_mc_votes(const float* in_nchw, int C, size_t N, size_t HW, int flags, uint32_t* votes, int bit, hipStream_t stream);
hipError_t launch_logit_normals(unsigned long long key, unsigned long long first_sample, size_t n, size_t hw, int C, int samples, float* out,
                                hipStream_t stream);
hipError_t launch_logit_sampling(const float* logits, const float* sigma_raw, size_t n, size_t hw, int C, int is_log_sigma, int samples,
                                 unsigned long long key, unsigned long long first_sample, float* probs, void* stats, int flags, hipStream_t stream);
int check_logit_sampling_shape(const char* fn, size_t n, size_t hw, int nb_classes, int samples);

hipError_t launch_mc_accumulate(const float* in_nchw, void* stats, int C, size_t N, size_t HW, int flags,
                                hipStream_t stream);
hipError_t launch_mc_finalize(const void* stats, int C, size_t N, size_t HW, int T, int flags, float* mean,
                              float* entropy, float* mi, float* var, hipStream_t stream);
hipError_t launch_softmax_nchw(const float* logits, float* probs, int C, size_t N, size_t HW, hipStream_t stream);
hipError_t launch_aleatoric(const float* logits, const float* sigma_raw, int C, size_t N, size_t HW, int is_log_sigma,
                            float* probs, float* sigma_out, uint8_t* prediction, float* sigma_pred,
                            hipStream_t stream);
hipError_t launch_argmax_fg(const float* probs_nchw, int C, size_t N, size_t HW, uint8_t* prediction, float* p_fg,
                            hipStream_t stream);
constexpr int MASK_MAX_PASSES = 32;
constexpr int MASK_MAX_SITES = 40;
struct MaskArgs {
    unsigned long long seed[MASK_MAX_PASSES];
    int site_end[MASK_MAX_SITES];
    float site_keep[MASK_MAX_SITES];
    int passes;
    int first, count;
    int sites, per_pass;
    int site_ch[MASK_MAX_SITES];
    int site_off[MASK_MAX_SITES];
    int per_sample;
    unsigned long long first_sample;
};
hipError_t launch_dropout_masks(const MaskArgs& a, float* out, hipStream_t stream);

hipError_t launch_mc_slice_scores(const void* stats, int C, size_t N, size_t HW, long long thr_q, uint32_t* unsettled, long long* margin_q,
                                  hipStream_t stream);
hipError_t launch_dropout_masks_indexed(const MaskArgs& a, const long long* sample_index, float* out, hipStream_t stream);
hipError_t launch_mc_merge_slices(const void* src, size_t M, void* dst, size_t N, size_t HW, int C, int flags, const int32_t* index, hipStream_t stream);
hipError_t launch_mc_finalize_counts(const void* stats, int C, size_t N, size_t HW, const int32_t* counts, int flags, float* mean, float* entropy,
                                     float* mi, float* var, hipStream_t stream);

constexpr int MAX_BINS = 32;
constexpr int MAX_THR = 16;
struct EceResult {
    unsigned long long count[MAX_BINS];
    double sum_conf[MAX_BINS];
    unsigned long long sum_pos[MAX_BINS];
};
void calib_set_blocks_per_workgroup(int ece, int unc);
size_t ece_workspace_bytes(size_t n_per_volume, int n_volumes);
hipError_t launch_ece_hist(const float* p, const uint8_t* target, const uint8_t* mask, size_t n_per_volume,
                           int n_volumes, const float* thr_host, int n_bins, EceResult* result_dev, void* workspace,
                           hipStream_t stream);
hipError_t launch_bin_ids(const float* p, size_t n, const float* thr_host, int n_bins, uint8_t* ids,
                          hipStream_t stream);
size_t unc_workspace_bytes(size_t n_per_volume, int n_volumes);
hipError_t launch_unc_counts(const void* unc, int unc_is_f64, const uint8_t* prediction, const uint8_t* target,
                             const uint8_t* mask, size_t n_per_volume, int n_volumes, const double* thr_host,
                             int n_thr, unsigned long long* out_dev, void* workspace, hipStream_t stream);
hipError_t launch_norm_entropy(const float* p_fg, size_t n, double* out_f64, float* out_f32, hipStream_t stream);
int unc_from_p_num_thresholds();
double unc_from_p_threshold(int i);
bool unc_from_p_supported(const double* thr, int n_thr);
int unc_from_p_exceeded_host(float p, const double* thr, int n_thr);
size_t unc_from_p_workspace_bytes(size_t n_per_volume, int n_volumes);
hipError_t launch_unc_counts_from_p(const float* p_fg, const uint8_t* prediction, const uint8_t* target, const uint8_t* mask, size_t n_per_volume,
                                    int n_volumes, const double* thr_host, int n_thr, unsigned long long* out_dev, void* workspace,
                                    hipStream_t stream);

constexpr int TN_MAX_CANDIDATES = 128;
size_t temperature_nll_workspace_bytes(size_t voxels, int n_candidates);

constexpr int pn_layer_floats(int cb) { return cb * cb * 1024 + 2 * cb * 32; }
constexpr int PN_MAX_LAYERS = 12;
constexpr int PN_MAX_BLOCKS = 3;
hipError_t launch_postnet(const float* x_nhwc, int channel_pitch, size_t nvox, int hw, const float* packed, int n_layers,
                          int nb_classes, int channels, const float* masks, float* logits_nchw, hipStream_t stream);

}
```

### reliability-challenges-uncertainty_amd/csrc/rcu_wino4.hip

```cpp
#include "rcu_wino_common.h"
#include "rcu_head_common.h"

namespace rcu {

template <int SB_, int BR_, int BC_, int WS_, int WR_, bool FULLW_ = false, bool FOLD_ = false>
struct Wino4Tile {
    static constexpr int SB = SB_, BR = BR_, BC = BC_, WS = WS_, WR = WR_;
    static constexpr bool FULLW = FULLW_, FOLD = FOLD_;
    static constexpr int FOLD_TS = 10;
    static constexpr int TS = FOLD ? FOLD_TS : SB * WS, TH = FOLD ? 12 : 4 * BR * WR, TW = FOLD ? 8 : 4 * BC;
    static constexpr int TCOLS = FOLD ? 2 : BC;
    static constexpr int BN = 32, KC = 8, THREADS = 256, WAVES = 4, NPOS = 36;
    static constexpr int XCOLS = FULLW ? TW : TW + 2;
    static constexpr int PITCH = (XCOLS + 3) / 4 * 4;
    static constexpr int SLICE_POS = ((TH + 2) * PITCH + 15) / 16 * 16;
    static constexpr int A_POS = 2 * TS * SLICE_POS;
    static constexpr int A_PIECES = (A_POS + 63) / 64;
    static constexpr int NA = (A_PIECES + WAVES - 1) / WAVES;
    static constexpr int A_DW = A_PIECES * 256;
    static constexpr int W_DW = NPOS * 4 * BN * 2;
    static constexpr int W_PIECES = W_DW / 256;
    static constexpr int NW = (W_PIECES + WAVES - 1) / WAVES;
    static constexpr int BUF_DW = A_DW + W_DW;
    static constexpr int LDS_BYTES = 2 * BUF_DW * 4;
    static_assert(SB * BR * BC == 16 && WS * WR == WAVES && BC % 4 == 0, "block geometry");
    static_assert(!FOLD || (SB == 2 && BR == 2 && BC == 4 && WS == 4 && WR == 1 && FULLW), "the folded 12x8 geometry descends from the S8 block");
    static_assert(!FOLD || 6 * TS <= 16 * WAVES, "a folded slice is 6 tiles");
    static_assert(W_DW % 256 == 0 && LDS_BYTES <= 160 * 1024, "LDS");
    static __device__ __forceinline__ void block_origin(int wave, int& s, int& y)
    {
        s = (wave / WR) * SB;
        y = (wave % WR) * (4 * BR);
    }
    static __device__ __forceinline__ void tile_of(int m, int& sb, int& tr, int& tc)
    {
        sb = m / (BR * BC);
        tr = (m / BC) % BR;
        tc = m % BC;
    }
    static __device__ __forceinline__ void row_tile(int wave, int m, int& s, int& y, int& tc)
    {
        if constexpr (FOLD) {
            const int k = min(16 * wave + m, 6 * TS - 1);
            s = k / 6;
            const int t = k - 6 * s;
            y = 4 * (t >> 1);
            tc = t & 1;
        } else {
            int bs, by, sb, tr;
            block_origin(wave, bs, by);
            tile_of(m, sb, tr, tc);
            s = bs + sb;
            y = by + 4 * tr;
        }
    }
    static __device__ __forceinline__ bool row_works(int wave, int m) { return !FOLD || 16 * wave + m < 6 * TS; }
    static __device__ __forceinline__ int swizzle(int x, int s, int R) { return (((x >> 3) ^ s) & 1) | (((R >> 2) & 1) << 1); }
};

template <class T>
__device__ __forceinline__ uint32_t wino4_slot_geometry(int j, int wave, int lane)
{
    const int f = (j * T::WAVES + wave) * 64 + lane;
    const int hh = f & 1, rem = f >> 1;
    const int s = rem / T::SLICE_POS, r2 = rem % T::SLICE_POS;
    const int yy = r2 / T::PITCH, pos = r2 % T::PITCH;
    const int x = pos ^ T::swizzle(pos, s, yy);
    const bool real = f < T::A_POS && yy < T::TH + 2 && x < T::XCOLS;
    return real ? (uint32_t)((x + (T::FULLW ? 1 : 0)) | (yy << 8) | (s << 16) | (hh << 24)) : 0xFFFFFFFFu;
}

template <class T>
__device__ __forceinline__ WinoEpiRaw wino4_epilogue_load(const ConvArgs& a, int ntile, int n0, int wave, int lane, int r = 0)
{
    WinoEpiRaw e;
    const int co = ntile * T::BN + 2 * (lane & 15);
    int s, ty, tc;
    T::row_tile(wave, 4 * (lane >> 4) + r, s, ty, tc);
    const float *alpha = a.alpha, *betab = a.betab, *beta = a.beta, *mask = a.mask, *mask2 = a.mask2;
    int N = a.N, Cmask = a.Cmask, Cmask2 = a.Cmask2, Csplit = a.Csplit;
    asm volatile("" : "+s"(alpha), "+s"(betab), "+s"(beta), "+s"(mask), "+s"(mask2), "+s"(N), "+s"(Cmask), "+s"(Cmask2), "+s"(Csplit));
    const int n = min(n0 + s, N - 1);
    e.al = *reinterpret_cast<const f32x2*>(alpha + co);
    e.bb = *reinterpret_cast<const f32x2*>(betab + co);
    e.be = *reinterpret_cast<const f32x2*>(beta + co);
    e.site = 0;
    e.mk[0] = e.mk[1] = 1.f;
    if (mask != nullptr) {
#pragma unroll
        for (int b = 0; b < 2; ++b) {
            const int c = co + b;
            const bool second = mask2 != nullptr && c >= Csplit;
            const int cm = second ? Cmask2 : Cmask, ci = second ? c - Csplit : c;
            const float* const row = second ? mask2 + (size_t)n * Cmask2 : mask + (size_t)n * Cmask;
            e.mk[b] = row[min(ci, cm - 1)];
            e.site |= (ci < cm ? 1 : 0) << b;
        }
    }
    return e;
}

#define WINO4_ALL_AGPRS \
    "a0", "a1", "a2", "a3", "a4", "a5", "a6", "a7", "a8", "a9", "a10", "a11", "a12", "a13", "a14", "a15", \
    "a16", "a17", "a18", "a19", "a20", "a21", "a22", "a23", "a24", "a25", "a26", "a27", "a28", "a29", "a30", "a31", \
    "a32", "a33", "a34", "a35", "a36", "a37", "a38", "a39", "a40", "a41", "a42", "a43", "a44", "a45", "a46", "a47", \
    "a48", "a49", "a50", "a51", "a52", "a53", "a54", "a55", "a56", "a57", "a58", "a59", "a60", "a61", "a62", "a63", \
    "a64", "a65", "a66", "a67", "a68", "a69", "a70", "a71", "a72", "a73", "a74", "a75", "a76", "a77", "a78", "a79", \
    "a80", "a81", "a82", "a83", "a84", "a85", "a86", "a87", "a88", "a89", "a90", "a91", "a92", "a93", "a94", "a95", \
    "a96", "a97", "a98", "a99", "a100", "a101", "a102", "a103", "a104", "a105", "a106", "a107", "a108", "a109", "a110", "a111", \
    "a112", "a113", "a114", "a115", "a116", "a117", "a118", "a119", "a120", "a121", "a122", "a123", "a124", "a125", "a126", "a127", \
    "a128", "a129", "a130", "a131", "a132", "a133", "a134", "a135", "a136", "a137", "a138", "a139", "a140", "a141", "a142", "a143", \
    "a144", "a145", "a146", "a147", "a148", "a149", "a150", "a151", "a152", "a153", "a154", "a155", "a156", "a157", "a158", "a159", \
    "a160", "a161", "a162", "a163", "a164", "a165", "a166", "a167", "a168", "a169", "a170", "a171", "a172", "a173", "a174", "a175", \
    "a176", "a177", "a178", "a179", "a180", "a181", "a182", "a183", "a184", "a185", "a186", "a187", "a188", "a189", "a190", "a191", \
    "a192", "a193", "a194", "a195", "a196", "a197", "a198", "a199", "a200", "a201", "a202", "a203", "a204", "a205", "a206", "a207", \
    "a208", "a209", "a210", "a211", "a212", "a213", "a214", "a215", "a216", "a217", "a218", "a219", "a220", "a221", "a222", "a223", \
    "a224", "a225", "a226", "a227", "a228", "a229", "a230", "a231", "a232", "a233", "a234", "a235", "a236", "a237", "a238", "a239", \
    "a240", "a241", "a242", "a243", "a244", "a245", "a246", "a247", "a248", "a249", "a250", "a251", "a252", "a253", "a254", "a255"
__host__ __device__ constexpr bool wino4_in_vgpr(int b, int p) { return b == 1 && p >= 18 && p < 26; }
__host__ __device__ constexpr int wino4_areg(int b, int p) { return 4 * (b == 0 ? p : 36 + (p < 18 ? p : p - 8)); }

template <int B, int P, bool ZERO>
__device__ __forceinline__ void wino4_mfma(f32x4 (&accv)[8], float av, float wv)
{
    if constexpr (wino4_in_vgpr(B, P)) {
        if constexpr (ZERO)
            asm volatile("s_nop 1\n\tv_mfma_f32_16x16x4_f32 %0, %1, %2, 0\n\ts_nop 11" : "=v"(accv[P - 18]) : "v"(av), "v"(wv));
        else
            asm volatile("s_nop 1\n\tv_mfma_f32_16x16x4_f32 %0, %1, %2, %0\n\ts_nop 11" : "+v"(accv[P - 18]) : "v"(av), "v"(wv));
    } else {
        constexpr int R = wino4_areg(B, P);
        if constexpr (ZERO)
            asm volatile("s_nop 1\n\tv_mfma_f32_16x16x4_f32 a[%c2:%c3], %0, %1, 0" ::"v"(av), "v"(wv), "i"(R), "i"(R + 3) : WINO4_ALL_AGPRS);
        else
            asm volatile("s_nop 1\n\tv_mfma_f32_16x16x4_f32 a[%c2:%c3], %0, %1, a[%c2:%c3]" ::"v"(av), "v"(wv), "i"(R), "i"(R + 3) : WINO4_ALL_AGPRS);
    }
}

template <int B, int P, int R>
__device__ __forceinline__ float wino4_acc(const f32x4 (&accv)[8])
{
    if constexpr (wino4_in_vgpr(B, P)) {
        return accv[P - 18][R];
    } else {
        float v;
        asm volatile("v_accvgpr_read_b32 %0, a%c1" : "=v"(v) : "i"(wino4_areg(B, P) + R));
        return v;
    }
}

struct Wino4StorePlan {
    uint32_t out, pool;
};
template <class T, bool PART>
__device__ __forceinline__ Wino4StorePlan wino4_store_plan(const ConvArgs& a, int wave, int lane)
{
    int s, ty, tc;
    T::row_tile(wave, 4 * (lane >> 4), s, ty, tc);
    if constexpr (T::FOLD) s = ty = tc = 0;
    const int n16 = lane & 15, odd = n16 & 1, c = 2 * n16 - 2 * odd;
    const int oH = PART ? a.out_H : a.H, oW = PART ? a.out_W : a.W;
    const int Hp = PART ? a.pool_H : a.H >> 1, Wp = PART ? a.pool_W : a.W >> 1;
    Wino4StorePlan p;
    p.out = wino_out_offset(s, oH * oW, a.CoutP, (uint32_t)(ty * oW + 4 * tc + odd), c, a.out_pix_bytes, a.out_chunk_bytes);
    p.pool = wino_out_offset(s, Hp * Wp, a.CoutP, (uint32_t)((ty >> 1) * Wp + 2 * tc + odd), c, a.pool_pix_bytes, a.pool_chunk_bytes);
    return p;
}

template <int R>
__device__ __forceinline__ void wino4_output_tile(const f32x4 (&accv)[8], const WinoEpi& ep, float relu_floor, f32x2 (&y)[4][4])
{
    constexpr int r = R;
    const f32x2 scale = {ep.scale[0], ep.scale[1]}, shift = {ep.shift[0], ep.shift[1]}, floor2 = {relu_floor, relu_floor};
    f32x2 nn[6][4];
    wino_static_for<0, 6>([&](auto i_c) {
        constexpr int i = decltype(i_c)::value;
        auto m = [&](auto j_c) {
            constexpr int j = decltype(j_c)::value;
            return f32x2{wino4_acc<0, 6 * i + j, r>(accv), wino4_acc<1, 6 * i + j, r>(accv)};
        };
        const f32x2 m0 = m(std::integral_constant<int, 0>{}), m1 = m(std::integral_constant<int, 1>{}), m2 = m(std::integral_constant<int, 2>{}),
                    m3 = m(std::integral_constant<int, 3>{}), m4 = m(std::integral_constant<int, 4>{}), m5 = m(std::integral_constant<int, 5>{});
        const f32x2 s1 = m1 + m2, s2 = m1 - m2, s3 = m3 + m4, s4 = m3 - m4;
        nn[i][0] = (m0 + s1) + s3;
        nn[i][1] = s2 + 2.f * s4;
        nn[i][2] = s1 + 4.f * s3;
        nn[i][3] = (s2 + 8.f * s4) + m5;
    });
#pragma unroll
    for (int q = 0; q < 4; ++q) {
        const f32x2 s1 = nn[1][q] + nn[2][q], s2 = nn[1][q] - nn[2][q], s3 = nn[3][q] + nn[4][q], s4 = nn[3][q] - nn[4][q];
        const f32x2 v0 = (nn[0][q] + s1) + s3;
        const f32x2 v1 = s2 + 2.f * s4;
        const f32x2 v2 = s1 + 4.f * s3;
        const f32x2 v3 = (s2 + 8.f * s4) + nn[5][q];
        y[0][q] = __builtin_elementwise_max(v0 * scale + shift, floor2);
        y[1][q] = __builtin_elementwise_max(v1 * scale + shift, floor2);
        y[2][q] = __builtin_elementwise_max(v2 * scale + shift, floor2);
        y[3][q] = __builtin_elementwise_max(v3 * scale + shift, floor2);
    }
}

template <class T, bool PART = false>
__device__ __forceinline__ void wino4_epilogue(const ConvArgs& a, const f32x4 (&accv)[8], const WinoEpi& ep, int ntile, int n0, int y0, int x0,
                                               int wave, int lane, const Wino4StorePlan& plan)
{
    asm volatile("s_nop 15\n\ts_nop 7");
    const int odd = lane & 1;
    const int H = a.H, W = a.W, CoutP = a.CoutP, N = a.N;
    const uint32_t px_bytes = a.out_pix_bytes, chunk_bytes = a.out_chunk_bytes, ppx_bytes = a.pool_pix_bytes, pchunk_bytes = a.pool_chunk_bytes;
    float* const out = a.out;
    float* const pooled = a.pooled;
    const float relu_floor = a.relu ? 0.f : -__builtin_inff();
    const bool pool = pooled != nullptr;
    const int oH = PART ? a.out_H : H, oW = PART ? a.out_W : W;
    const int Hp = PART ? a.pool_H : H >> 1, Wp = PART ? a.pool_W : W >> 1;
    const uint32_t row_bytes = (uint32_t)oW * px_bytes, prow_bytes = (uint32_t)Wp * ppx_bytes;
    const __amdgpu_buffer_rsrc_t ro = __builtin_amdgcn_make_buffer_rsrc(out, 0, (uint32_t)(N * oH * oW) * (uint32_t)CoutP * 4u, 0x00020000);
    const uint32_t vo = plan.out + wino_out_offset(n0, oH * oW, CoutP, (uint32_t)(y0 * oW + x0), ntile * T::BN, px_bytes, chunk_bytes);
    const __amdgpu_buffer_rsrc_t rp = __builtin_amdgcn_make_buffer_rsrc(pool ? pooled : out, 0, pool ? (uint32_t)(N * Hp * Wp * CoutP) * 4u : 0u, 0x00020000);
    const uint32_t vp = plan.pool + wino_out_offset(n0, Hp * Wp, CoutP, (uint32_t)((y0 >> 1) * Wp + (x0 >> 1)), ntile * T::BN, ppx_bytes, pchunk_bytes);
    [[maybe_unused]] int ylim = 0, xlim = 0, pylim = 0, pxlim = 0;
    [[maybe_unused]] int Hr = 0, Wr = 0;
    if constexpr (PART) {
        Hr = a.Hr;
        Wr = a.Wr;
        if constexpr (!T::FOLD) {
            int s, ty, tc;
            T::row_tile(wave, 4 * (lane >> 4), s, ty, tc);
            ylim = Hr - (y0 + ty);
            xlim = Wr - (x0 + 4 * tc + odd);
            pylim = (Hr >> 1) - ((y0 + ty) >> 1);
            pxlim = (Wr >> 1) - (((x0 + 4 * tc) >> 1) + odd);
        }
    }
    [[maybe_unused]] int s_first = 0;
    [[maybe_unused]] WinoEpi ep_last = ep;
    if constexpr (T::FOLD) {
        int ty, tc;
        T::row_tile(wave, 4 * (lane >> 4), s_first, ty, tc);
        ep_last = wino_epilogue_fold(wino4_epilogue_load<T>(a, ntile, n0, wave, lane, 3));
    }
    wino_static_for<0, 4>([&](auto r_c) {
        constexpr int r = decltype(r_c)::value;
        constexpr int tdx = T::FOLD ? 0 : 4 * r, tdy = 0;
        uint32_t vo_r = vo;
        WinoEpi ep_r = ep;
        if constexpr (T::FOLD) {
            int s, ty, tc;
            T::row_tile(wave, 4 * (lane >> 4) + r, s, ty, tc);
            vo_r = T::row_works(wave, 4 * (lane >> 4) + r) ? vo + wino_out_offset(s, oH * oW, CoutP, (uint32_t)(ty * oW + 4 * tc), 0, px_bytes, chunk_bytes) : WINO_OOB;
            if (s != s_first) ep_r = ep_last;
            if constexpr (PART) {
                ylim = Hr - (y0 + ty);
                xlim = Wr - (x0 + 4 * tc + odd);
            }
        }
        f32x2 y[4][4];
        wino4_output_tile<r>(accv, ep_r, relu_floor, y);
#pragma unroll
        for (int aa = 0; aa < 4; ++aa) {
#pragma unroll
            for (int h2 = 0; h2 < 2; ++h2) {
                const f32x2 keep = odd ? y[aa][2 * h2 + 1] : y[aa][2 * h2];
                const f32x2 send = odd ? y[aa][2 * h2] : y[aa][2 * h2 + 1];
                f32x2 recv;
                recv.x = wino_swap_adjacent(send.x);
                recv.y = wino_swap_adjacent(send.y);
                const f32x4 o = odd ? f32x4{recv.x, recv.y, keep.x, keep.y} : f32x4{keep.x, keep.y, recv.x, recv.y};
                const uint32_t vo_s = (PART && !(tdy + aa < ylim && tdx + 2 * h2 < xlim)) ? WINO_OOB : vo_r;
                wino_store16(o, ro, vo_s, (uint32_t)(tdx + 2 * h2) * px_bytes + (uint32_t)(tdy + aa) * row_bytes);
            }
        }
        if (!T::FOLD && pool) {
#pragma unroll
            for (int a2 = 0; a2 < 2; ++a2) {
                f32x2 mx[2];
#pragma unroll
                for (int b2 = 0; b2 < 2; ++b2)
                    mx[b2] = __builtin_elementwise_max(__builtin_elementwise_max(y[2 * a2][2 * b2], y[2 * a2][2 * b2 + 1]),
                                                       __builtin_elementwise_max(y[2 * a2 + 1][2 * b2], y[2 * a2 + 1][2 * b2 + 1]));
                const f32x2 keep = odd ? mx[1] : mx[0];
                const f32x2 send = odd ? mx[0] : mx[1];
                f32x2 recv;
                recv.x = wino_swap_adjacent(send.x);
                recv.y = wino_swap_adjacent(send.y);
                const f32x4 o = odd ? f32x4{recv.x, recv.y, keep.x, keep.y} : f32x4{keep.x, keep.y, recv.x, recv.y};
                const uint32_t vp_s = (PART && !(a2 < pylim && 2 * r < pxlim)) ? WINO_OOB : vp;
                wino_store16(o, rp, vp_s, (uint32_t)(2 * r) * ppx_bytes + (uint32_t)a2 * prow_bytes);
            }
        }
    });
}

constexpr int WINO4_HEAD_LDS_BYTES = 512;
template <class T, bool PART = false>
__device__ __forceinline__ void wino4_epilogue_head(const ConvArgs& a, const f32x4 (&accv)[8], const WinoEpi& ep, int n0, int nstat, int y0, int x0,
                                                    int wave, int lane, uint32_t area, uint32_t wlds)
{
    asm volatile("" : "+v"(lane));
    static_assert(T::TS == 1 && !T::FOLD && T::BC % 4 == 0 && T::BN == 32, "whole tiles of one slice, one 32-cout tile");
    static_assert(7 * 4096 + 3 * 1024 + 1024 <= T::W_DW * 4, "the hand-over area lies inside the weight region");
    asm volatile("s_nop 15\n\ts_nop 7");
    const int n16 = lane & 15, g = lane >> 4;
    const int H = PART ? a.Hr : a.H, W = PART ? a.Wr : a.W, flags = a.head_flags;
    float* const logits = a.head_logits;
    void* const stats = a.head_stats;
    const size_t V = a.head_V;
    const float relu_floor = a.relu ? 0.f : -__builtin_inff();
    int bs, by, sb, tr, tc;
    T::block_origin(wave, bs, by);
    T::tile_of(4 * g, sb, tr, tc);
    const size_t HW = (size_t)H * W;
    const size_t hw0 = (size_t)(y0 + by + 4 * tr + (n16 >> 2)) * W + (size_t)(x0 + 4 * tc + (n16 & 3));
    [[maybe_unused]] const bool row_in = y0 + by + 4 * tr + (n16 >> 2) < H;
    [[maybe_unused]] const int xlim = W - (x0 + 4 * tc + (n16 & 3));
    typedef volatile __attribute__((address_space(3))) f32x2 lds_f32x2;
    const uint32_t mine = area + (uint32_t)wave * 1024u + (uint32_t)g * 128u;
    const uint32_t wbase = mine + 8u * (uint32_t)n16;
    const uint32_t rbase = mine + (uint32_t)(n16 >> 1) * 4096u + (uint32_t)(n16 & 1) * 512u + 8u * (uint32_t)n16;
    wino_static_for<0, 4>([&](auto r_c) {
        constexpr int r = decltype(r_c)::value;
        const size_t hw = hw0 + 4 * r;
        const bool inside = !PART || (row_in && 4 * r < xlim);
        VoxelStats<2> st;
        if (stats != nullptr && inside) st.load(stats, (size_t)nstat * HW + hw, V, flags);
        {
            f32x2 y[4][4];
            wino4_output_tile<r>(accv, ep, relu_floor, y);
#pragma unroll
            for (int k = 0; k < 16; ++k)
                *(lds_f32x2*)(uintptr_t)((wbase ^ (8u * k)) + (uint32_t)((k >> 1) * 4096 + (k & 1) * 512)) = y[k >> 2][k & 3];
        }
        __builtin_amdgcn_fence(__ATOMIC_RELEASE, "wavefront");
        __builtin_amdgcn_wave_barrier();
        __builtin_amdgcn_fence(__ATOMIC_ACQUIRE, "wavefront");
        float row[32];
#pragma unroll
        for (int j = 0; j < 16; ++j) {
            const f32x2 v = *(lds_f32x2*)(uintptr_t)(rbase ^ (8u * j));
            row[2 * j] = v.x;
            row[2 * j + 1] = v.y;
        }
        __builtin_amdgcn_fence(__ATOMIC_RELEASE, "wavefront");
        __builtin_amdgcn_wave_barrier();
        float l[2];
#pragma unroll
        for (int c = 0; c < 2; ++c) {
            float p[8];
#pragma unroll
            for (int sgm = 0; sgm < 8; ++sgm) {
                const f32x4 w = *(const __attribute__((address_space(3))) f32x4*)(uintptr_t)(wlds + (uint32_t)(c * 32 + 4 * sgm) * 4u);
                float t = fmaf(w.x, row[4 * sgm], 0.f);
                t = fmaf(w.y, row[4 * sgm + 1], t);
                t = fmaf(w.z, row[4 * sgm + 2], t);
                p[sgm] = fmaf(w.w, row[4 * sgm + 3], t);
            }
            const float bias = *(const __attribute__((address_space(3))) float*)(uintptr_t)(wlds + (uint32_t)(64 + c) * 4u);
            l[c] = (((p[0] + p[1]) + (p[2] + p[3])) + ((p[4] + p[5]) + (p[6] + p[7]))) + bias;
        }
        if (logits != nullptr && inside) {
            logits[((size_t)n0 * 2 + 0) * HW + hw] = l[0];
            logits[((size_t)n0 * 2 + 1) * HW + hw] = l[1];
        }
        if (stats != nullptr && inside) {
            softmax_inplace<2>(l);
            st.add(flags, l);
            st.store(stats, (size_t)nstat * HW + hw, V, flags);
        }
    });
}

__host__ __device__ constexpr int wino4_row_of(int k) { return k == 0 ? 0 : k == 1 ? 5 : k - 1; }
__host__ __device__ constexpr int wino4_pos_of(int q) { return 6 * wino4_row_of(q / 6) + q % 6; }

template <class T, bool HEAD = false, bool PART = false>
__global__ __launch_bounds__(256, 1) void conv_wino4_stream(const ConvArgs a, const int total_items)
{
#if defined(__HIP_DEVICE_COMPILE__)
    extern __shared__ __attribute__((aligned(1024))) float smem[];
    constexpr int KC = T::KC;

    const int tid = threadIdx.x;
    const int lane = tid & 63;
    const int wave = __builtin_amdgcn_readfirstlane(tid >> 6);
    const int m16 = lane & 15, kq = lane >> 4;
    const int nchunks = (a.C1 + a.C2) / KC;
    const uint32_t wchunk_bytes = (uint32_t)a.NT * T::W_DW * 4u;
    const uint32_t in_chunk_bytes = a.in_chunk_bytes;

    const __amdgpu_buffer_rsrc_t rs1 = __builtin_amdgcn_make_buffer_rsrc(const_cast<float*>(a.src1), 0, a.src1_bytes, 0x00020000);
    const __amdgpu_buffer_rsrc_t rs2 =
        __builtin_amdgcn_make_buffer_rsrc(const_cast<float*>(a.src2 ? a.src2 : a.src1), 0, a.src2 ? a.src2_bytes : 0u, 0x00020000);
    const __amdgpu_buffer_rsrc_t rsw = __builtin_amdgcn_make_buffer_rsrc(const_cast<float*>(a.wpack), 0, a.wpack_bytes, 0x00020000);

    int aCol[2][6];
    bool zero_left = false, zero_right = false;
    {
        int s, R0, tc;
        T::row_tile(wave, m16, s, R0, tc);
        const int base = (s * T::SLICE_POS + R0 * T::PITCH) * 8 + 2 * kq;
#pragma unroll
        for (int ip = 0; ip < 2; ++ip)
#pragma unroll
            for (int j = 0; j < 6; ++j) {
                int x = 4 * tc + j - (T::FULLW ? 1 : 0);
                if (T::FULLW) x = min(max(x, 0), T::TW - 1);
                aCol[ip][j] = base + 8 * (x ^ T::swizzle(x, s, R0 + 4 * ip));
            }
        if (T::FULLW) {
            zero_left = tc == 0;
            zero_right = tc == T::TCOLS - 1;
        }
    }
    const int b_addr = T::A_DW + (kq * T::BN + 2 * m16) * 2;
    const uint32_t w_voff = (uint32_t)(lane * 16);

    int item = wino_xcd_virtual_block(a.NT < 4 ? 4 : a.NT);
    [[maybe_unused]] int pass = 0;
    auto more_passes = [&]() {
        if constexpr (HEAD) return pass + 1 < wino_cold_args().head_passes;
        return false;
    };
    bool has_next = more_passes() || item + (int)gridDim.x < total_items;
    WinoTileId tile = wino_tile_id<T>(a, item), ntile = tile;
    uint32_t dp[T::NA], dpn[T::NA], geo[T::NA];
    int dp_wtile = tile.wtile, dpn_wtile = tile.wtile;
#pragma unroll
    for (int j = 0; j < T::NA; ++j) {
        geo[j] = wino_slot_plan<T>(a, wino4_slot_geometry<T>(j, wave, lane));
        asm volatile("" : "+v"(geo[j]));
        dp[j] = dpn[j] = wino_slot_offset(geo[j], wino_tile_offset<T>(a, tile));
    }

    Wino4StorePlan store_plan = wino4_store_plan<T, PART>(a, wave, lane);
    asm volatile("" : "+v"(store_plan.out), "+v"(store_plan.pool));

    struct DmaJob {
        __amdgpu_buffer_rsrc_t rs;
        uint32_t cb, wso, lb;
    };
    auto dma_job = [&](int wtile, int kc, int buf, bool active) {
        DmaJob j;
        const int c0 = kc * KC;
        const bool first = c0 < a.C1;
        j.rs = first ? rs1 : rs2;
        j.cb = active ? wino_chunk_offset(in_chunk_bytes, first ? c0 : c0 - a.C1) : WINO_OOB;
        j.wso = active ? (uint32_t)kc * wchunk_bytes + (uint32_t)wtile * (T::W_DW * 4u) : WINO_OOB;
        j.lb = (uint32_t)buf * (T::BUF_DW * 4u);
        return j;
    };
    const uint32_t lds_base = (uint32_t)(uintptr_t)(lds_ptr_t)smem;
    auto dma_piece = [&](const DmaJob& job, const uint32_t (&off)[T::NA], auto i_c) {
        constexpr int I = decltype(i_c)::value;
        if constexpr (I < T::NA) {
            constexpr int j = I;
            if ((j + 1) * T::WAVES <= T::A_PIECES || j * T::WAVES + wave < T::A_PIECES)
                __builtin_amdgcn_raw_ptr_buffer_load_lds(job.rs, (lds_ptr_t)(uintptr_t)(lds_base + job.lb + (j * T::WAVES + wave) * 1024), 16, off[j],
                                                         job.cb, 0, 0);
        } else if constexpr (I < T::NW + T::NA) {
            constexpr int k = I - T::NA;
            if ((k + 1) * T::WAVES <= T::W_PIECES || k * T::WAVES + wave < T::W_PIECES)
                __builtin_amdgcn_raw_ptr_buffer_load_lds(rsw, (lds_ptr_t)(uintptr_t)(lds_base + job.lb + T::A_DW * 4 + (k * T::WAVES + wave) * 1024),
                                                         16, w_voff, job.wso + (uint32_t)(k * T::WAVES + wave) * 1024u, 0, 0);
        }
    };

    constexpr int PB = (T::TS == 1 && T::TH == 32) ? 4 : 0;
    static_assert(PB <= T::NA, "the back part consists of input pieces");
    {
        const DmaJob job = dma_job(dp_wtile, 0, 0, true);
        wino_static_for<0, T::NW + T::NA>([&](auto i_c) { dma_piece(job, dp, i_c); });
    }
    if constexpr (HEAD) {
        if (tid < 66) smem[2 * T::BUF_DW + tid] = tid < 64 ? a.head_w[tid] : a.head_b[tid - 64];
    }
    __builtin_amdgcn_s_waitcnt(0x0F70);
    __syncthreads();
    {
        const DmaJob job = dma_job(dp_wtile, 1, 1, true);
        wino_static_for<0, PB>([&](auto i_c) { dma_piece(job, dp, i_c); });
    }

    f32x4 accv[8];
    WinoEpiRaw epr;

    constexpr int AHEAD = 4, NPRE = 14;
    auto load_patch_row = [&](f32x2 (&d)[36], const float* Ab, int i) {
#pragma unroll
        for (int j = 0; j < 6; ++j)
            d[6 * i + j] = *(const volatile __attribute__((address_space(3))) f32x2*)(Ab + aCol[i >> 2][j] + i * (T::PITCH * 8));
        if constexpr (T::FULLW) {
            const f32x2 z = {0.f, 0.f};
            d[6 * i] = zero_left ? z : d[6 * i];
            d[6 * i + 5] = zero_right ? z : d[6 * i + 5];
        }
    };
    auto load_weights = [&](f32x4 (&bv)[36], const float* Ab, int p) { bv[p] = *reinterpret_cast<const f32x4*>(Ab + b_addr + p * (8 * T::BN)); };
    auto row_transform = [&](f32x2 (&d)[36], int i) {
        f32x2* const x = d + 6 * i;
        const f32x2 t0 = 4.f * x[0] + (x[4] - 5.f * x[2]);
        const f32x2 t5 = 4.f * x[1] + (x[5] - 5.f * x[3]);
        const f32x2 aa = x[4] - 4.f * x[2], bb = x[3] - 4.f * x[1], cc = x[4] - x[2], ee = x[3] - x[1];
        x[0] = t0;
        x[1] = aa + bb;
        x[2] = aa - bb;
        x[3] = cc + 2.f * ee;
        x[4] = cc - 2.f * ee;
        x[5] = t5;
    };
    auto transform_head = [&](f32x2 (&d)[36]) {
#pragma unroll
        for (int j = 0; j < 6; ++j) d[j] = 4.f * d[j] + (d[24 + j] - 5.f * d[12 + j]);
        row_transform(d, 0);
    };
    auto transform_clump = [&](f32x2 (&d)[36], int G) {
        if (G == 0) {
#pragma unroll
            for (int j = 0; j < 6; ++j) d[30 + j] = 4.f * d[6 + j] + (d[30 + j] - 5.f * d[18 + j]);
        }
        if (G == 1) row_transform(d, 5);
        if (G == 2 || G == 3) {
#pragma unroll
            for (int jj = 0; jj < 3; ++jj) {
                const int j = 3 * (G - 2) + jj;
                const f32x2 x1 = d[6 + j], x2 = d[12 + j], x3 = d[18 + j], x4 = d[24 + j];
                d[12 + j] = x4 - 4.f * x2;
                d[24 + j] = x4 - x2;
                d[6 + j] = x3 - 4.f * x1;
                d[18 + j] = x3 - x1;
            }
        }
        if (G == 4) {
#pragma unroll
            for (int j = 0; j < 6; ++j) {
                const f32x2 aa = d[12 + j], bb = d[6 + j];
                d[6 + j] = aa + bb;
                d[12 + j] = aa - bb;
            }
        }
        if (G == 5) row_transform(d, 1);
        if (G == 6) row_transform(d, 2);
        if (G == 7) {
#pragma unroll
            for (int j = 0; j < 6; ++j) {
                const f32x2 cc = d[24 + j], ee = d[18 + j];
                d[18 + j] = cc + 2.f * ee;
                d[24 + j] = cc - 2.f * ee;
            }
        }
        if (G == 8) row_transform(d, 3);
        if (G == 9) row_transform(d, 4);
    };

    auto chunk = [&](auto buf_c, auto first_c, int kc, f32x2 (&d)[36], f32x2 (&dn)[36], f32x4 (&bv)[36], f32x4 (&bvn)[36]) {
        constexpr int BUF = decltype(buf_c)::value;
        constexpr bool FIRST = decltype(first_c)::value;
        const float* const Ab = smem + BUF * T::BUF_DW;
        const float* const An = smem + (BUF ^ 1) * T::BUF_DW;
        const bool more = kc + 1 < nchunks, more2 = kc + 2 < nchunks;
        if (kc == nchunks - 2 && has_next) {
            const WinoTileConsts ca = wino_tile_consts(wino_cold_args());
            if (more_passes()) {
                ntile = tile;
                ntile.n0 = tile.n0 + wino_cold_args().head_images;
            } else {
                ntile = wino_tile_id<T>(ca, item + (int)gridDim.x);
            }
            dpn_wtile = ntile.wtile;
            const WinoTileOffset nto = wino_tile_offset<T>(ca, ntile);
#pragma unroll
            for (int j = 0; j < T::NA; ++j) dpn[j] = wino_slot_offset(geo[j], nto);
        }
        if (!more) {
            dp_wtile = dpn_wtile;
#pragma unroll
            for (int j = 0; j < T::NA; ++j) dp[j] = dpn[j];
        }
        if (kc == nchunks - 2) epr = wino4_epilogue_load<T>(wino_cold_args(), tile.wtile, tile.n0, wave, lane);
        const DmaJob job = dma_job(dp_wtile, more ? kc + 1 : 0, BUF ^ 1, more || has_next);
        const DmaJob jobb = dma_job(dpn_wtile, more2 ? kc + 2 : kc + 2 - nchunks, BUF, more2 || has_next);
        transform_head(d);
        wino_static_for<0, 18>([&](auto g_c) {
            constexpr int G = decltype(g_c)::value;
            constexpr int p0 = wino4_pos_of(2 * G), p1 = wino4_pos_of(2 * G + 1);
            __builtin_amdgcn_sched_barrier(0);
            if constexpr (G == NPRE) {
                __builtin_amdgcn_s_waitcnt(0x0F70);
                __syncthreads();
                __builtin_amdgcn_sched_barrier(0);
            }
            auto filler = [&](auto u_c) {
                constexpr int U = decltype(u_c)::value;
                if constexpr (G < NPRE) {
                    if constexpr (U == 0 || U == 4) {
                        constexpr int q = 2 * G + AHEAD + (U == 4 ? 1 : 0);
                        if constexpr (q < 2 * NPRE) load_weights(bv, Ab, wino4_pos_of(q));
                    }
                    if constexpr (G >= NPRE - 4 && (U == 2 || U == 6)) {
                        constexpr int q = 2 * NPRE + 2 * (G - (NPRE - 4)) + (U == 6 ? 1 : 0);
                        load_weights(bv, Ab, wino4_pos_of(q));
                    }
                    if constexpr (G < 10 && (U == 1 || U == 5)) dma_piece(job, dp, std::integral_constant<int, PB + 2 * G + (U == 5 ? 1 : 0)>{});
                } else {
                    if constexpr ((U == 1 || U == 5) && 2 * (G - NPRE) + (U == 5 ? 1 : 0) < PB)
                        dma_piece(jobb, dpn, std::integral_constant<int, 2 * (G - NPRE) + (U == 5 ? 1 : 0)>{});
                    {
                        constexpr int slot = 8 * (G - NPRE) + U;
                        constexpr int order[6] = {0, 2, 4, 1, 3, 5};
                        if constexpr (slot < 30) {
                            constexpr int r = order[slot / 5];
                            if constexpr (slot % 5 == 0) load_patch_row(dn, An, r);
                        }
                        if constexpr (slot == 30)
                            wino_static_for<0, AHEAD>([&](auto q_c) { load_weights(bvn, An, wino4_pos_of(decltype(q_c)::value)); });
                    }
                }
                __builtin_amdgcn_sched_barrier(0);
            };
            wino4_mfma<0, p0, FIRST>(accv, d[p0].x, bv[p0].x);
            filler(std::integral_constant<int, 0>{});
            wino4_mfma<1, p0, FIRST>(accv, d[p0].x, bv[p0].z);
            filler(std::integral_constant<int, 1>{});
            wino4_mfma<0, p1, FIRST>(accv, d[p1].x, bv[p1].x);
            filler(std::integral_constant<int, 2>{});
            wino4_mfma<1, p1, FIRST>(accv, d[p1].x, bv[p1].z);
            filler(std::integral_constant<int, 3>{});
            wino4_mfma<0, p0, false>(accv, d[p0].y, bv[p0].y);
            filler(std::integral_constant<int, 4>{});
            wino4_mfma<1, p0, false>(accv, d[p0].y, bv[p0].w);
            filler(std::integral_constant<int, 5>{});
            wino4_mfma<0, p1, false>(accv, d[p1].y, bv[p1].y);
            filler(std::integral_constant<int, 6>{});
            wino4_mfma<1, p1, false>(accv, d[p1].y, bv[p1].w);
            filler(std::integral_constant<int, 7>{});
            transform_clump(d, G);
        });
    };

    f32x2 dA[36], dB[36];
    f32x4 bvA[36], bvB[36];
    auto load_first = [&]() {
#pragma unroll
        for (int ii = 0; ii < 6; ++ii) load_patch_row(dA, smem, ii < 3 ? 2 * ii : 2 * (ii - 3) + 1);
        wino_static_for<0, AHEAD>([&](auto q_c) { load_weights(bvA, smem, wino4_pos_of(decltype(q_c)::value)); });
    };
    load_first();

    for (;;) {
        chunk(std::integral_constant<int, 0>{}, std::true_type{}, 0, dA, dB, bvA, bvB);
        chunk(std::integral_constant<int, 1>{}, std::false_type{}, 1, dB, dA, bvB, bvA);
        for (int kc = 2; kc < nchunks; kc += 2) {
            chunk(std::integral_constant<int, 0>{}, std::false_type{}, kc, dA, dB, bvA, bvB);
            chunk(std::integral_constant<int, 1>{}, std::false_type{}, kc + 1, dB, dA, bvB, bvA);
        }
        if constexpr (HEAD)
            wino4_epilogue_head<T, PART>(wino_cold_args(), accv, wino_epilogue_fold(epr), tile.n0, tile.n0 - pass * wino_cold_args().head_images, tile.y0, tile.x0,
                                         wave, lane, lds_base + (uint32_t)(T::BUF_DW + T::A_DW) * 4u, lds_base + (uint32_t)(2 * T::BUF_DW) * 4u);
        else
            wino4_epilogue<T, PART>(wino_cold_args(), accv, wino_epilogue_fold(epr), tile.wtile, tile.n0, tile.y0, tile.x0, wave, lane, store_plan);
        if (!has_next) break;
        load_first();
        if (more_passes()) {
            ++pass;
        } else {
            pass = 0;
            item += (int)gridDim.x;
        }
        tile = ntile;
        has_next = more_passes() || item + (int)gridDim.x < total_items;
    }
#endif
}

using W4Cfg0 = Wino4Tile<1, 2, 8, 1, 4>;
using W4Cfg1 = Wino4Tile<1, 2, 8, 2, 2>;
using W4Cfg2 = Wino4Tile<2, 2, 4, 4, 1, true>;
using W4Cfg3 = Wino4Tile<2, 2, 4, 4, 1, true, true>;
using W4Cfg4 = Wino4Tile<1, 2, 8, 4, 1, true>;

static constexpr ConvFamilyTraits kWino4 = {ConvFamily::Wino4, true, true, true, true, 1, 2.25};

static const ConvConfigInfo kWino4Info[6] = {
    {W4Cfg0::TS, W4Cfg0::TH, W4Cfg0::TW, W4Cfg0::BN, 8, 36, "conv3x3_winograd4<T32x32,N32,K8>", 8, 0, kWino4, 1.0, CONV_CFG_WINO4_T32x32_N32_HEAD},
    {W4Cfg1::TS, W4Cfg1::TH, W4Cfg1::TW, W4Cfg1::BN, 8, 36, "conv3x3_winograd4<S2T16x32,N32,K8>", 8, 0, kWino4},
    {W4Cfg2::TS, W4Cfg2::TH, W4Cfg2::TW, W4Cfg2::BN, 8, 36, "conv3x3_winograd4<S8T8x16,N32,K8>", 8, 0, kWino4},
    {W4Cfg3::TS, W4Cfg3::TH, W4Cfg3::TW, W4Cfg3::BN, 8, 36, "conv3x3_winograd4<S8T12x8,N32,K8>", 8, 0, kWino4, 64.0 / 60.0},
    {W4Cfg0::TS, W4Cfg0::TH, W4Cfg0::TW, W4Cfg0::BN, 8, 36, "conv3x3_winograd4<T32x32,N32,K8>+head", 8, 0, kWino4},
    {W4Cfg4::TS, W4Cfg4::TH, W4Cfg4::TW, W4Cfg4::BN, 8, 36, "conv3x3_winograd4<S4T8x32,N32,K8>", 8, 0, kWino4},
};

const ConvConfigInfo& wino4_config_info(int cfg) { return kWino4Info[cfg - CONV_CFG_WINO4_T32x32_N32]; }

template <class T, bool HEAD, bool PART>
static hipError_t launch_wino4_kernel(const ConvArgs& a, hipStream_t stream)
{
    constexpr int lds_bytes = T::LDS_BYTES + (HEAD ? WINO4_HEAD_LDS_BYTES : 0);
    static_assert(lds_bytes <= 160 * 1024, "LDS");
    hipError_t e = set_max_dynamic_lds(reinterpret_cast<const void*>(&conv_wino4_stream<T, HEAD, PART>), lds_bytes);
    if (e != hipSuccess) return e;
    const unsigned items = (unsigned)a.NT * a.tiles_x * a.tiles_y * (HEAD ? a.head_images : a.slice_groups);
    const unsigned grid = wino_persistent_grid(items);
    hipLaunchKernelGGL((conv_wino4_stream<T, HEAD, PART>), dim3(grid), dim3(T::THREADS), lds_bytes, stream, a, (int)items);
    return hipGetLastError();
}

template <class T, bool HEAD = false>
static hipError_t launch_wino4_cfg(const ConvArgs& a, hipStream_t stream)
{
    if (HEAD && (a.head_w == nullptr || a.head_b == nullptr || a.NT != 1 || a.pooled != nullptr || a.mask2 != nullptr || a.head_passes < 1 ||
                 a.head_images * a.head_passes != a.N || (a.head_passes > 1 && a.head_logits != nullptr) ||
                 (a.head_logits == nullptr && a.head_stats == nullptr)))
        return hipErrorInvalidValue;
    const int nchunks = (a.C1 + a.C2) / T::KC;
    if (nchunks < 4 || (nchunks & 1) != 0 || a.NTW_total != a.NT || a.src1_bytes == 0 || a.wpack_bytes == 0 ||
        (a.C2 != 0 && a.C2 != a.C1) || a.H % T::TH != 0 || a.W % T::TW != 0 || (T::FULLW && a.W != T::TW) || (T::FOLD && a.pooled != nullptr) ||
        (size_t)a.N * a.H * a.W * a.CoutP * 4 >= ((size_t)1 << 31))
        return hipErrorInvalidValue;
    if (a.part && (a.Hr < 1 || a.Wr < 1 || a.Hr > a.H || a.Wr > a.W || a.out_H < a.Hr || a.out_W < a.Wr ||
                   (size_t)a.N * a.out_H * a.out_W * a.CoutP * 4 >= ((size_t)1 << 31) ||
                   (a.pooled != nullptr && (a.pool_H < (a.Hr >> 1) || a.pool_W < (a.Wr >> 1)))))
        return hipErrorInvalidValue;
    if (a.part) return launch_wino4_kernel<T, HEAD, true>(a, stream);
    return launch_wino4_kernel<T, HEAD, false>(a, stream);
}

hipError_t launch_conv_wino4(int cfg, const ConvArgs& a, hipStream_t stream)
{
    switch (cfg) {
        case CONV_CFG_WINO4_T32x32_N32: return launch_wino4_cfg<W4Cfg0>(a, stream);
        case CONV_CFG_WINO4_S2T16x32_N32: return launch_wino4_cfg<W4Cfg1>(a, stream);
        case CONV_CFG_WINO4_S8T8x16_N32: return launch_wino4_cfg<W4Cfg2>(a, stream);
        case CONV_CFG_WINO4_S8T12x8_N32: return launch_wino4_cfg<W4Cfg3>(a, stream);
        case CONV_CFG_WINO4_T32x32_N32_HEAD: return launch_wino4_cfg<W4Cfg0, true>(a, stream);
        case CONV_CFG_WINO4_S4T8x32_N32: return launch_wino4_cfg<W4Cfg4>(a, stream);
        default: return hipErrorInvalidValue;
    }
}

}
```

### reliability-challenges-uncertainty_amd/csrc/rcu_wino_common.h

```cpp
#pragma once
#include "rcu_kernels.h"

#include <type_traits>

namespace rcu {

typedef float f32x2 __attribute__((ext_vector_type(2)));
typedef float f32x4 __attribute__((ext_vector_type(4)));
typedef unsigned u32x4 __attribute__((ext_vector_type(4)));
typedef __attribute__((address_space(3))) void* lds_ptr_t;

__device__ __forceinline__ float wino_swap_adjacent(float v)
{
    return __builtin_bit_cast(float, __builtin_amdgcn_update_dpp(0, __builtin_bit_cast(int, v), 0xB1, 0xF, 0xF, false));
}

__device__ __forceinline__ const ConvArgs& wino_cold_args()
{
    auto p = __builtin_amdgcn_kernarg_segment_ptr();
    asm volatile("" : "+s"(p));
    return *(const ConvArgs*)p;
}

__device__ __forceinline__ void wino_store16(const f32x4& v, __amdgpu_buffer_rsrc_t rsrc, uint32_t voff, uint32_t soff)
{
    __builtin_amdgcn_raw_buffer_store_b128(__builtin_bit_cast(u32x4, v), rsrc, voff, soff, 0);
    __builtin_amdgcn_sched_barrier(0);
    asm volatile("s_nop 1");
    __builtin_amdgcn_sched_barrier(0);
}

template <int I, int N, class F>
__device__ __forceinline__ void wino_static_for(F&& f)
{
    if constexpr (I < N) {
        f(std::integral_constant<int, I>{});
        wino_static_for<I + 1, N>(f);
    }
}

__device__ __forceinline__ int wino_xcd_virtual_block(int group)
{
    const int g = (int)gridDim.x, b = (int)blockIdx.x;
    if ((g & 7) != 0 || ((g >> 3) % group) != 0) return b;
    const int xcd = b & 7, slot = b >> 3;
    return ((slot / group) * 8 + xcd) * group + slot % group;
}

template <int TS_, int TH_, int TW_, int BN_, int WM_, int WN_, int SW_ = 1, int NPOS_ = 16>
struct WinoTile {
    static constexpr int TS = TS_, TH = TH_, TW = TW_, BN = BN_, WM = WM_, WN = WN_, SW = SW_;
    static constexpr int NPOS = NPOS_;
    static constexpr int KC = 8, THREADS = 512, WAVES = 8;
    static constexpr int TILES = TS * (TH / 2) * (TW / 2);
    static constexpr int BPS = (TH / 4) * (TW * SW / 16);
    static constexpr int PITCH = (TW + 2 + 7) / 8 * 8;
    static constexpr int SLICE_POS = (TH + 2) * PITCH + (SW == 2 ? 8 : 0);
    static constexpr int HALF_POS = TS * SLICE_POS;
    static constexpr int A_POS = 2 * HALF_POS;
    static constexpr int A_PIECES = (A_POS + 63) / 64;
    static constexpr int NA = (A_PIECES + WAVES - 1) / WAVES;
    static constexpr int A_DW = A_PIECES * 256;
    static constexpr int W_DW = NPOS * 4 * BN * 2;
    static constexpr int W_PIECES = W_DW / 256;
    static constexpr int NW = (W_PIECES + WAVES - 1) / WAVES;
    static constexpr int BUF_DW = A_DW + W_DW;
    static constexpr int LDS_BYTES = 2 * BUF_DW * 4;
    static_assert(WM * WN == 8, "8 waves per workgroup");
    static_assert(TILES == 16 * WM && BN == 32 * WN, "wave tiling");
    static_assert(TH % 4 == 0 && (TW * SW) % 16 == 0 && (SW == 1 || (SW == 2 && TW == 8 && TS % 2 == 0)), "block geometry");
    static_assert(SW == 1 || SLICE_POS % 16 == 8, "slice stride");
    static_assert(W_DW % 256 == 0, "weight staging");
    static_assert(LDS_BYTES <= 160 * 1024, "LDS");
    static __device__ __forceinline__ void block_origin(int blk, int& s, int& y, int& x)
    {
        const int grp = blk / BPS, rb = blk % BPS;
        s = grp * SW;
        y = 4 * (rb / (TW * SW / 16));
        x = SW == 1 ? 16 * (rb % (TW / 16)) : 0;
    }
};

struct WinoEpiRaw {
    f32x2 al, bb, be;
    float mk[2];
    int site;
};
struct WinoEpi {
    float scale[2], shift[2];
};
__device__ __forceinline__ WinoEpi wino_epilogue_fold(const WinoEpiRaw& r)
{
    WinoEpi e;
#pragma unroll
    for (int b = 0; b < 2; ++b) {
        const float mk = (r.site >> b) & 1 ? r.mk[b] : 1.f;
        e.scale[b] = r.al[b] * mk;
        e.shift[b] = r.bb[b] * mk + r.be[b];
    }
    return e;
}

template <class T>
__device__ __forceinline__ WinoEpiRaw wino_epilogue_load(const ConvArgs& a, int ntile, int n0, int wm, int wn, int lane)
{
    WinoEpiRaw e;
    const int co = ntile * T::BN + wn * 32 + 2 * (lane & 15);
    int bs, by, bx;
    T::block_origin(wm, bs, by, bx);
    const int n = min(n0 + bs + (T::SW == 2 ? (lane >> 4) & 1 : 0), a.N - 1);
    e.al = *reinterpret_cast<const f32x2*>(a.alpha + co);
    e.bb = *reinterpret_cast<const f32x2*>(a.betab + co);
    e.be = *reinterpret_cast<const f32x2*>(a.beta + co);
    e.site = 0;
    e.mk[0] = e.mk[1] = 1.f;
    if (a.mask != nullptr) {
#pragma unroll
        for (int b = 0; b < 2; ++b) {
            const int c = co + b;
            const bool second = a.mask2 != nullptr && c >= a.Csplit;
            const int cm = second ? a.Cmask2 : a.Cmask, ci = second ? c - a.Csplit : c;
            const float* const row = second ? a.mask2 + (size_t)n * a.Cmask2 : a.mask + (size_t)n * a.Cmask;
            e.mk[b] = row[min(ci, cm - 1)];
            e.site |= (ci < cm ? 1 : 0) << b;
        }
    }
    return e;
}

constexpr uint32_t WINO_OOB = 0x80000000u;

struct WinoTileId {
    int wtile, n0, y0, x0;
};

struct WinoTileConsts {
    int NTW_total, tiles_x, tiles_y, H, W, C1;
    uint32_t magic_ntw, magic_tx, magic_ty, in_pix_bytes;
};
__device__ __forceinline__ WinoTileConsts wino_tile_consts(const ConvArgs& a)
{
    WinoTileConsts c{a.NTW_total, a.tiles_x, a.tiles_y, a.H, a.W, a.C1, a.magic_ntw, a.magic_tx, a.magic_ty, a.in_pix_bytes};
    asm volatile("" : "+s"(c.NTW_total), "+s"(c.tiles_x), "+s"(c.tiles_y), "+s"(c.H), "+s"(c.W), "+s"(c.C1), "+s"(c.magic_ntw), "+s"(c.magic_tx),
                      "+s"(c.magic_ty), "+s"(c.in_pix_bytes));
    return c;
}

template <class T, class A>
__device__ __forceinline__ WinoTileId wino_tile_id(const A& a, int item)
{
    WinoTileId t;
    auto div = [](int x, int d, uint32_t magic) { return magic ? (int)__umulhi((uint32_t)x, magic) : x / d; };
    int mtile = div(item, a.NTW_total, a.magic_ntw);
    t.wtile = item - mtile * a.NTW_total;
    const int q = div(mtile, a.tiles_x, a.magic_tx);
    const int tx = mtile - q * a.tiles_x;
    const int sg = div(q, a.tiles_y, a.magic_ty);
    const int ty = q - sg * a.tiles_y;
    t.n0 = sg * T::TS;
    t.y0 = ty * T::TH;
    t.x0 = tx * T::TW;
    return t;
}

constexpr int WINO_POS_DW = 4;
template <class T>
__device__ __forceinline__ uint32_t wino_slot_geometry(int j, int wave, int lane)
{
    const int f = (j * T::WAVES + wave) * 64 + lane;
    const int hh = f / T::HALF_POS, rem = f % T::HALF_POS;
    const int s = rem / T::SLICE_POS, r2 = rem % T::SLICE_POS;
    const int yy = r2 / T::PITCH, pos = r2 % T::PITCH;
    const int x = pos ^ ((yy >> 1) & 1);
    const bool real = f < T::A_POS && yy < T::TH + 2 && x < T::TW + 2;
    return real ? (uint32_t)(x | (yy << 8) | (s << 16) | (hh << 24)) : 0xFFFFFFFFu;
}

template <class T>
__device__ __forceinline__ uint32_t wino_slot_plan(const ConvArgs& a, uint32_t geo)
{
    const int x = geo & 0xFF, yy = (geo >> 8) & 0xFF, s = (geo >> 16) & 0xFF, hh = (geo >> 24) & 1;
    const uint32_t off = (uint32_t)s * ((uint32_t)(a.H * a.W) * (uint32_t)a.C1 * 4u) + (uint32_t)((yy - 1) * a.W + (x - 1)) * a.in_pix_bytes + (uint32_t)hh * 16u;
    const uint32_t flags = (yy == 0 ? 1u : 0u) | (yy == T::TH + 1 ? 2u : 0u) | (x == 0 ? 4u : 0u) | (x == T::TW + 1 ? 8u : 0u);
    return geo != 0xFFFFFFFFu ? (off | flags) : 0x80000000u;
}

struct WinoTileOffset {
    uint32_t off, border;
};
template <class T, class A>
__device__ __forceinline__ WinoTileOffset wino_tile_offset(const A& a, const WinoTileId& t)
{
    WinoTileOffset o;
    o.off = (uint32_t)t.n0 * ((uint32_t)(a.H * a.W) * (uint32_t)a.C1 * 4u) + (uint32_t)(t.y0 * a.W + t.x0) * a.in_pix_bytes;
    o.border = (t.y0 == 0 ? 1u : 0u) | (t.y0 + T::TH == a.H ? 2u : 0u) | (t.x0 == 0 ? 4u : 0u) | (t.x0 + T::TW == a.W ? 8u : 0u);
    return o;
}

__device__ __forceinline__ uint32_t wino_slot_offset(uint32_t plan, const WinoTileOffset& t)
{
    return (plan & t.border) != 0u ? WINO_OOB : ((plan + t.off) & ~15u);
}

inline unsigned wino_persistent_grid(unsigned items)
{
    constexpr unsigned cap = 256u;
    return items < cap ? items : cap;
}

__device__ __forceinline__ uint32_t wino_chunk_offset(uint32_t in_chunk_bytes, int c0) { return (uint32_t)(c0 >> 3) * in_chunk_bytes; }

__device__ __forceinline__ uint32_t wino_out_offset(int n, int hw, int CoutP, uint32_t pix, int c, uint32_t pix_bytes, uint32_t chunk_bytes)
{
    return (uint32_t)n * ((uint32_t)hw * (uint32_t)CoutP * 4u) + (uint32_t)(c >> 3) * chunk_bytes + pix * pix_bytes + (uint32_t)(c & 7) * 4u;
}

}
```

### reliability-challenges-uncertainty_amd/model.py

```python
import ctypes
import itertools

import torch
import torch.nn as nn

from . import _lib


class _Holder(nn.Module):
    """Plain container; children are added by dotted path to reproduce the reference's key names."""


def _add(root, path, module):
    parts = path.split('.')
    cur = root
    for p in parts[:-1]:
        if p not in cur._modules:
            cur.add_module(p, _Holder())
        cur = cur._modules[p]
    cur.add_module(parts[-1], module)


def _dropout_rule(dropout_center, level, depth, is_down):
    if dropout_center is None:
        return 'all'
    if level == depth:
        return 'no'
    if level + dropout_center >= depth:
        return 'last' if is_down else 'first'
    return 'no'


def _has_dropout(dropout, rule, i):
    if dropout is None:
        return False
    return rule == 'all' or (rule == 'first' and i == 0) or (rule == 'last' and i == 1)


class UNet(nn.Module):
    DEFAULT_DEPTH = 4
    DEFAULT_START_FILTERS = 16
    DEFAULT_DROPOUT = 0.2
    MAX_HANDLES = 6
    PLAN_DEFAULTS = dict(conv_winograd=1, conv_winograd4=1, conv_first=1, act_layout=0, head_winograd4=1, pad_levels=1, upconv_winograd4=1)
    _generations = itertools.count(1)

    def __init__(self, nb_classes, in_channels, depth=DEFAULT_DEPTH, start_filters=DEFAULT_START_FILTERS,
                 dropout=DEFAULT_DROPOUT, dropout_center: int = None, residual=False, sigma_out=False,
                 provide_features=False, bn=True):
        super().__init__()
        self.nb_classes, self.in_channels, self.depth = nb_classes, in_channels, depth
        self.start_filters, self.dropout, self.dropout_center = start_filters, dropout, dropout_center
        self.sigma_out, self.bn, self.residual = sigma_out, bn, bool(residual)
        self.provide_features = provide_features
        self.features = None
        self._site_modules = []
        self._sites = None

        def unit(prefix, cin, cout, with_dropout):
            base = prefix + '.conv2d_batch_relu'
            _add(self, base + '.conv', nn.Conv2d(cin, cout, 3, padding=1))
            if with_dropout:
                do = nn.Dropout2d(p=dropout)
                _add(self, base + '.dropout', do)
                self._site_modules.append(do)
            if bn:
                _add(self, base + '.bn', nn.BatchNorm2d(cout))

        def block(prefix, cin, cout, rule):
            for i in range(2):
                unit('{}.{}'.format(prefix, i), cin if i == 0 else cout, cout, _has_dropout(dropout, rule, i))
            if residual:
                _add(self, prefix[:-len('.block')] + '.residual', nn.Conv2d(cin, cout, 1))

        cin, cout = in_channels, start_filters
        for lvl in range(depth):
            block('down_convs.{}.block.block'.format(lvl), cin, cout, _dropout_rule(dropout_center, lvl, depth, True))
            cin, cout = cout, cout * 2
        block('bottom_convs.block', cin, cout, _dropout_rule(dropout_center, depth, depth, True))
        for j, lvl in enumerate(range(depth - 1, -1, -1)):
            cin, cout = cout, cout // 2
            block('up_convs.{}.block.block'.format(j), 2 * cout, cout,
                  _dropout_rule(dropout_center, lvl, depth, False))
            _add(self, 'up_convs.{}.upconv.1'.format(j), nn.Conv2d(cin, cout, 3, padding=1))
        unit('conv_cls.0', cout, cout, dropout is not None)
        _add(self, 'conv_cls.1', nn.Conv2d(cout, nb_classes, 1))
        if sigma_out:
            unit('conv_sigma.0', cout, cout, dropout is not None)
            _add(self, 'conv_sigma.1', nn.Conv2d(cout, nb_classes, 1))
        for p in self.parameters():
            p.requires_grad = False
        self._handles = {}
        self._weights_version = 0
        self.plan_options = {}
        self.fuse_head = True
        self._donor = None
        self._last_generation = 0
        self.temperature = 1.0
        self.eval()

    def load_state_dict(self, state_dict, strict=True, **kwargs):
        state_dict = {(k[len('module.'):] if k.startswith('module.') else k): v for k, v in state_dict.items()}
        result = super().load_state_dict(state_dict, strict=strict, **kwargs)
        self.weights_changed()
        return result

    def weights_changed(self):
        self._weights_version += 1

    def set_temperature(self, t):
        import math
        try:
            value = float(t)
        except (TypeError, ValueError):
            raise ValueError('the temperature must be a number, got {!r}'.format(t)) from None
        if isinstance(t, bool) or not math.isfinite(value) or value <= 0:
            raise ValueError('the temperature must be finite and > 0, got {!r}'.format(t))
        if self.sigma_out:
            raise ValueError('temperature scaling is not defined for a sigma_out model (its sigma is in logit units)')
        if value != self.temperature:
            self.temperature = value
            self.weights_changed()

    def share_workspace(self, donor):
        if donor is self:
            donor = None
        if donor is not None:
            mine = (self.nb_classes, self.in_channels, self.depth, self.start_filters, self.dropout is not None, self.dropout_center,
                    self.residual, self.sigma_out, bool(self.provide_features), self.bn)
            theirs = (donor.nb_classes, donor.in_channels, donor.depth, donor.start_filters, donor.dropout is not None,
                      donor.dropout_center, donor.residual, donor.sigma_out, bool(donor.provide_features), donor.bn)
            if mine != theirs:
                raise ValueError('share_workspace: the donor is a different architecture')
            if donor._donor is not None:
                donor = donor._donor
            if donor is self:
                return
        self._release()
        self._donor = donor

    def set_fuse_head(self, on):
        self.fuse_head = bool(on)
        lib = _lib.load()
        for entry in self._handles.values():
            _lib.check(lib.rcu_unet_set_fuse_head(entry[0], int(self.fuse_head)))

    def _options(self):
        unknown = set(self.plan_options) - set(self.PLAN_DEFAULTS)
        if unknown:
            raise ValueError('unknown plan options: {}'.format(sorted(unknown)))
        return dict(self.PLAN_DEFAULTS, **self.plan_options)

    def _release(self):
        lib = _lib.load()
        for entry in self._handles.values():
            lib.rcu_unet_destroy(entry[0])
        self._handles = {}
        self.features = None

    def __del__(self):
        try:
            self._release()
        except Exception:
            pass

    def _handle(self, h, w, n, lane=0):
        lib = _lib.load()
        options = self._options()
        slot = (h, w) if lane == 0 else (h, w, lane)
        if self.provide_features:
            slot = slot + ('features',)
        slot = slot + (tuple(sorted(options.items())),)
        entry = self._handles.get(slot)
        donor_handle = None
        donor_key = None
        if self._donor is not None:
            donor_handle = self._donor._handle(h, w, n if entry is None else max(n, entry[1]), lane)
            donor_key = self._donor._last_generation
        if entry is not None and entry[1] >= n and entry[2] == self._weights_version and entry[3] == donor_key:
            self._handles[slot] = self._handles.pop(slot)
            self._last_generation = entry[4]
            return entry[0]
        max_batch = n if entry is None else max(n, entry[1])
        if entry is not None:
            lib.rcu_unet_destroy(entry[0])
            del self._handles[slot]
            self.features = None
        desc = _lib.UnetDesc(nb_classes=self.nb_classes, in_channels=self.in_channels, depth=self.depth,
                             start_filters=self.start_filters, has_dropout=int(self.dropout is not None),
                             dropout_center=-1 if self.dropout_center is None else int(self.dropout_center),
                             sigma_out=int(self.sigma_out), bn=int(self.bn), height=h, width=w, max_batch=max_batch,
                             residual=int(self.residual), provide_features=int(bool(self.provide_features)))
        opts = _lib.UnetOptions(fuse_head=int(self.fuse_head), **options)
        handle = ctypes.c_void_p()
        _lib.check(lib.rcu_unet_create_with(ctypes.byref(desc), ctypes.byref(opts), donor_handle, ctypes.byref(handle)))
        try:
            for key, value in self.state_dict().items():
                if not torch.is_floating_point(value):
                    continue
                host = value.detach().to('cpu', torch.float32).contiguous()
                _lib.check(lib.rcu_unet_load_weight(handle, key.encode(), ctypes.c_void_p(host.data_ptr()),
                                                    host.numel()))
            if self.temperature != 1.0:
                _lib.check(lib.rcu_unet_set_temperature(handle, float(self.temperature)))
            _lib.check(lib.rcu_unet_finalize_weights(handle))
        except Exception:
            lib.rcu_unet_destroy(handle)
            raise
        self._last_generation = next(UNet._generations)
        self._handles[slot] = (handle, max_batch, self._weights_version, donor_key, self._last_generation)
        while len(self._handles) > self.MAX_HANDLES:
            old = next(iter(self._handles))
            lib.rcu_unet_destroy(self._handles.pop(old)[0])
            self.features = None
        return handle

    def max_group_samples(self, h, w):
        widest = max(8, (self.start_filters + 31) // 32 * 32 * (2 if self.sigma_out else 1))
        h, w = int(h), int(w)
        if self._options().get('pad_levels', 1) and (h % 32 or w % 32):
            h, w = (h + 31) // 32 * 32, (w + 31) // 32 * 32
        return max(1, ((1 << 31) - 1) // (h * w * 4 * widest))

    def reserve(self, h, w, n, lane=0):
        self._handle(h, w, n, lane)

    def dropout_sites(self):
        if self._sites is None:
            modules = dict(self.named_modules())
            names = {id(m): n for n, m in modules.items()}
            self._sites = [(names[id(m)], modules[names[id(m)][:-len('.dropout')] + '.conv'].out_channels)
                           for m in self._site_modules]
        return list(self._sites)

    def mc_active(self):
        return any(m.training for m in self._site_modules)

    def sample_masks(self, n, device, generator=None):
        groups = []
        for m, (_, c) in zip(self._site_modules, self.dropout_sites()):
            state = float(m.p) if (m.training and m.p > 0) else None
            if groups and groups[-1][0] == state:
                groups[-1][1] += n * c
            else:
                groups.append([state, n * c])
        chunks = []
        for state, count in groups:
            if state is None:
                chunks.append(torch.ones(count, device=device))
            elif state >= 1:
                chunks.append(torch.zeros(count, device=device))
            else:
                keep = 1.0 - state
                chunks.append(torch.empty(count, device=device).bernoulli_(keep, generator=generator).div_(keep))
        if not chunks:
            return None
        return chunks[0] if len(chunks) == 1 else torch.cat(chunks)

    def seeded_masks(self, n, device, seeds, first_sample=0, sample_index=None):
        sites = self.dropout_sites()
        if not sites:
            return None
        g, count = len(seeds), len(sites)
        keeps = [(max(0.0, 1.0 - float(m.p)) if (m.training and m.p > 0) else -1.0) for m in self._site_modules]
        out = torch.empty(g * n * sum(c for _, c in sites), device=device, dtype=torch.float32)
        if sample_index is not None:
            if (not torch.is_tensor(sample_index) or sample_index.dtype != torch.int64 or sample_index.numel() != n or
                    not sample_index.is_contiguous() or sample_index.device != out.device):
                raise ValueError('sample_index must be a contiguous int64 tensor of {} entries on {}'.format(n, out.device))
            _lib.check(_lib.load().rcu_dropout_masks_indexed((ctypes.c_uint64 * g)(*[int(v) & 0xFFFFFFFFFFFFFFFF for v in seeds]), g, n,
                                                             _lib.ptr(sample_index), (ctypes.c_int32 * count)(*[c for _, c in sites]),
                                                             (ctypes.c_float * count)(*keeps), count, _lib.ptr(out), _lib.current_stream()))
            return out
        _lib.check(_lib.load().rcu_dropout_masks((ctypes.c_uint64 * g)(*[int(v) & 0xFFFFFFFFFFFFFFFF for v in seeds]), g, n, int(first_sample),
                                                 (ctypes.c_int32 * count)(*[c for _, c in sites]), (ctypes.c_float * count)(*keeps), count,
                                                 _lib.ptr(out), _lib.current_stream()))
        return out

    def pack_masks(self, masks, n, device):
        sites = self.dropout_sites()
        if len(masks) != len(sites):
            raise ValueError('expected {} dropout masks, got {}'.format(len(sites), len(masks)))
        flat = []
        for m, (_, c) in zip(masks, sites):
            t = torch.as_tensor(m, dtype=torch.float32)
            if tuple(t.shape) != (n, c):
                raise ValueError('mask shape {} does not match (n={}, channels={})'.format(tuple(t.shape), n, c))
            flat.append(t.reshape(-1))
        return torch.cat(flat).to(device).contiguous() if flat else None

    def _check_input(self, x):
        if not isinstance(x, torch.Tensor) or x.dim() != 4 or x.shape[1] != self.in_channels:
            raise ValueError('expected a [N, {}, H, W] tensor'.format(self.in_channels))
        if not x.is_cuda:
            raise RuntimeError('rcu_amd.model.UNet only runs on the GPU (librcu_hip); got a {} tensor'.format(x.device))
        return x.to(torch.float32).contiguous()

    def forward(self, x, masks=None):
        x = self._check_input(x)
        n, _, h, w = x.shape
        handle = self._handle(h, w, n)
        if masks is None and self.mc_active():
            masks = self.sample_masks(n, x.device)
        elif isinstance(masks, (list, tuple)):
            masks = self.pack_masks(masks, n, x.device)
        logits = torch.empty((n, self.nb_classes, h, w), device=x.device, dtype=torch.float32)
        sigma = torch.empty_like(logits) if self.sigma_out else None
        _lib.check(_lib.load().rcu_unet_forward(handle, _lib.ptr(x), n, _lib.ptr(masks), _lib.ptr(logits),
                                                _lib.ptr(sigma), _lib.current_stream()))
        if self.provide_features:
            self.features = self._features_view(handle, n, h, w, x.device)
        if self.sigma_out:
            return logits, sigma
        return logits

    def _features_view(self, handle, n, h, w, device):
        ptr, ch, pitch = ctypes.c_void_p(), ctypes.c_int(), ctypes.c_int()
        _lib.check(_lib.load().rcu_unet_features(handle, ctypes.byref(ptr), ctypes.byref(ch), ctypes.byref(pitch)))
        nhwc = _lib.device_view(ptr.value, (n, h, w, pitch.value), device, owner=self)
        return nhwc[..., :ch.value].permute(0, 3, 1, 2)

    def forward_accumulate(self, x, stats, masks=None, passes=1, lane=0, votes=None, bits=None):
        x = self._check_input(x)
        n, _, h, w = x.shape
        if (n, self.nb_classes, h * w) != (stats.n, stats.nb_classes, stats.hw):
            raise ValueError('statistics blob shape does not match the batch')
        if passes < 1:
            raise ValueError('passes must be >= 1')
        if votes is not None:
            bits = [int(b) for b in (bits if bits is not None else ())]
            if len(bits) != passes:
                raise ValueError('a voting pass needs one bit per pass (bits)')
            if tuple(votes.plane.shape[1:]) != (n, h, w) or votes.plane.device != x.device:
                raise ValueError('vote plane shape does not match the batch')
            if any(not 0 <= b < 32 * votes.n_words for b in bits):
                raise ValueError('vote bits must be in [0, {})'.format(32 * votes.n_words))
        handle = self._handle(h, w, n * passes, lane)
        if masks is None:
            if passes > 1 and not self.mc_active():
                raise ValueError('a pass group needs stochastic passes: set_dropout_mode(model, True) or inject masks')
            masks = self.sample_masks(n * passes, x.device) if self.mc_active() else None
        elif isinstance(masks, (list, tuple)):
            masks = self.group_masks(masks, n, x.device) if passes > 1 else self.pack_masks(masks, n, x.device)
        lib, stream = _lib.load(), _lib.current_stream()
        if votes is not None:
            status = lib.rcu_unet_forward_accumulate_votes(handle, _lib.ptr(x), n, passes, _lib.ptr(masks), _lib.ptr(stats.blob), stats.flags,
                                                           _lib.ptr(votes.plane), votes.n_words, (ctypes.c_int32 * passes)(*bits), stream)
        elif passes == 1:
            status = lib.rcu_unet_forward_accumulate(handle, _lib.ptr(x), n, _lib.ptr(masks), _lib.ptr(stats.blob), stats.flags, stream)
        else:
            status = lib.rcu_unet_forward_accumulate_passes(handle, _lib.ptr(x), n, passes, _lib.ptr(masks), _lib.ptr(stats.blob), stats.flags,
                                                            stream)
        _lib.check(status)
        stats.count += passes

    def forward_accumulate_sigma(self, x, stats, sigma_sum, masks=None, is_log_sigma=False, lane=0, passes=1):
        if not self.sigma_out:
            raise ValueError('forward_accumulate_sigma needs a model built with sigma_out=True')
        x = self._check_input(x)
        n, _, h, w = x.shape
        if (n, self.nb_classes, h * w) != (stats.n, stats.nb_classes, stats.hw):
            raise ValueError('statistics blob shape does not match the batch')
        if (tuple(sigma_sum.shape) != (n, self.nb_classes, h, w) or sigma_sum.dtype != torch.float32 or
                not sigma_sum.is_contiguous() or sigma_sum.device != x.device):
            raise ValueError('sigma_sum must be a contiguous float32 [N, C, H, W] tensor on the input device')
        if passes < 1:
            raise ValueError('passes must be >= 1')
        handle = self._handle(h, w, n * passes, lane)
        if passes > 1:
            if masks is None:
                if not self.mc_active():
                    raise ValueError('a pass group needs stochastic passes: set_dropout_mode(model, True) or inject masks')
                masks = self.sample_masks(n * passes, x.device)
            elif isinstance(masks, (list, tuple)):
                masks = self.group_masks(masks, n, x.device)
            _lib.check(_lib.load().rcu_unet_forward_accumulate_sigma_passes(handle, _lib.ptr(x), n, passes, _lib.ptr(masks),
                                                                            _lib.ptr(stats.blob), stats.flags, _lib.ptr(sigma_sum),
                                                                            int(bool(is_log_sigma)), _lib.current_stream()))
            stats.count += passes
            return
        if masks is None and self.mc_active():
            masks = self.sample_masks(n, x.device)
        elif isinstance(masks, (list, tuple)):
            masks = self.pack_masks(masks, n, x.device)
        _lib.check(_lib.load().rcu_unet_forward_accumulate_sigma(handle, _lib.ptr(x), n, _lib.ptr(masks), _lib.ptr(stats.blob),
                                                                 stats.flags, _lib.ptr(sigma_sum), int(bool(is_log_sigma)),
                                                                 _lib.current_stream()))
        stats.count += 1

    def forward_sample_sigma(self, x, stats, sigma_sum, keys, first_sample, samples, masks=None, is_log_sigma=False, lane=0):
        if not self.sigma_out:
            raise ValueError('forward_sample_sigma needs a model built with sigma_out=True')
        x = self._check_input(x)
        n, _, h, w = x.shape
        passes = len(keys)
        if passes < 1:
            raise ValueError('forward_sample_sigma needs one key per pass')
        if (n, self.nb_classes, h * w) != (stats.n, stats.nb_classes, stats.hw):
            raise ValueError('statistics blob shape does not match the batch')
        if (tuple(sigma_sum.shape) != (n, self.nb_classes, h, w) or sigma_sum.dtype != torch.float32 or
                not sigma_sum.is_contiguous() or sigma_sum.device != x.device):
            raise ValueError('sigma_sum must be a contiguous float32 [N, C, H, W] tensor on the input device')
        handle = self._handle(h, w, n * passes, lane)
        if masks is None:
            if passes > 1 and not self.mc_active():
                raise ValueError('a pass group needs stochastic passes: set_dropout_mode(model, True) or inject masks')
            masks = self.sample_masks(n * passes, x.device) if self.mc_active() else None
        elif isinstance(masks, (list, tuple)):
            masks = self.group_masks(masks, n, x.device) if passes > 1 else self.pack_masks(masks, n, x.device)
        key_arr = (ctypes.c_uint64 * passes)(*[int(k) for k in keys])
        _lib.check(_lib.load().rcu_unet_forward_sample_sigma_passes(handle, _lib.ptr(x), n, passes, _lib.ptr(masks), key_arr, int(first_sample),
                                                                    int(samples), _lib.ptr(stats.blob), stats.flags, _lib.ptr(sigma_sum),
                                                                    int(bool(is_log_sigma)), _lib.current_stream()))
        stats.count += passes

    def group_masks(self, mask_sets, n, device):
        sites = self.dropout_sites()
        per_set = []
        for ms in mask_sets:
            flat = self.pack_masks(ms, n, device) if isinstance(ms, (list, tuple)) else ms.to(device)
            per_set.append(torch.split(flat, [n * c for _, c in sites]) if sites else [])
        chunks = [torch.cat([ps[i] for ps in per_set]) for i in range(len(sites))]
        return torch.cat(chunks).contiguous() if chunks else None

    def layer_table(self, h, w, n=1):
        lib = _lib.load()
        handle = self._handle(h, w, n)
        rows = []
        for i in range(lib.rcu_unet_num_layers(handle)):
            info = _lib.LayerInfo()
            _lib.check(lib.rcu_unet_layer_info(handle, i, ctypes.byref(info)))
            rows.append(dict(index=i, name=info.name.decode(), kernel=info.kernel.decode(), cin=info.cin,
                             cout=info.cout, height=info.height, width=info.width, grid_height=info.grid_height, grid_width=info.grid_width,
                             upsample=bool(info.upsample),
                             pooled=bool(info.pooled), dual_source=bool(info.dual_source), head_fusable=bool(info.head_fusable),
                             flops_per_slice=info.flops_per_slice,
                             mfma_flops_per_slice=info.mfma_flops_per_slice))
        return rows

    def run_layer(self, h, w, n, layer, masks=None):
        _lib.check(_lib.load().rcu_unet_run_layer(self._handle(h, w, n), layer, n, _lib.ptr(masks),
                                                  _lib.current_stream()))

    def profile_begin(self, h, w, n, max_forwards):
        _lib.check(_lib.load().rcu_unet_profile_begin(self._handle(h, w, n), max_forwards))

    def profile_collect(self, h, w, n):
        lib = _lib.load()
        handle = self._handle(h, w, n)
        slots = lib.rcu_unet_num_layers(handle) + 2
        ms = (ctypes.c_double * slots)()
        cnt = ctypes.c_int()
        _lib.check(lib.rcu_unet_profile_collect(handle, ms, ctypes.byref(cnt)))
        return cnt.value, list(ms)

    def workspace_bytes(self, h, w, n, lane=0):
        return int(_lib.load().rcu_unet_workspace_bytes(self._handle(h, w, n, lane)))


class PostNet(nn.Module):

    def __init__(self, in_channels, nb_classes, nb_convs=3, dropout=None):
        super().__init__()
        self.in_channels, self.nb_classes, self.nb_convs = in_channels, nb_classes, nb_convs
        self._dropouts = []
        for i in range(nb_convs):
            base = 'convs.{}.conv2d_batch_relu'.format(i)
            _add(self, base + '.conv', nn.Conv2d(in_channels, in_channels, 1))
            if dropout is not None:
                do = nn.Dropout2d(p=dropout)
                _add(self, base + '.dropout', do)
                self._dropouts.append(do)
            _add(self, base + '.bn', nn.BatchNorm2d(in_channels))
        _add(self, 'conv_logits', nn.Conv2d(in_channels, nb_classes, 1))
        for p in self.parameters():
            p.requires_grad = False
        self._handle_entry = None
        self._weights_version = 0
        self.eval()

    def load_state_dict(self, state_dict, strict=True, **kwargs):
        state_dict = {(k[len('module.'):] if k.startswith('module.') else k): v for k, v in state_dict.items()}
        result = super().load_state_dict(state_dict, strict=strict, **kwargs)
        self.weights_changed()
        return result

    def weights_changed(self):
        self._weights_version += 1

    def __del__(self):
        try:
            if self._handle_entry is not None:
                _lib.load().rcu_postnet_destroy(self._handle_entry[0])
        except Exception:
            pass

    def _handle(self):
        lib = _lib.load()
        if self._handle_entry is not None and self._handle_entry[1] == self._weights_version:
            return self._handle_entry[0]
        if self._handle_entry is not None:
            lib.rcu_postnet_destroy(self._handle_entry[0])
            self._handle_entry = None
        handle = ctypes.c_void_p()
        _lib.check(lib.rcu_postnet_create(self.in_channels, self.nb_classes, self.nb_convs, 1, ctypes.byref(handle)))
        try:
            for key, value in self.state_dict().items():
                if not torch.is_floating_point(value):
                    continue
                host = value.detach().to('cpu', torch.float32).contiguous()
                _lib.check(lib.rcu_postnet_load_weight(handle, key.encode(), ctypes.c_void_p(host.data_ptr()),
                                                       host.numel()))
            _lib.check(lib.rcu_postnet_finalize_weights(handle))
        except Exception:
            lib.rcu_postnet_destroy(handle)
            raise
        self._handle_entry = (handle, self._weights_version)
        return handle

    def sample_masks(self, n, device, generator=None):
        if not self._dropouts or not any(m.training for m in self._dropouts):
            return None
        rows = []
        for m in self._dropouts:
            if m.training and 0 < m.p < 1:
                keep = 1.0 - float(m.p)
                rows.append(torch.empty(n * self.in_channels, device=device).bernoulli_(keep, generator=generator).div_(keep))
            elif m.training and m.p >= 1:
                rows.append(torch.zeros(n * self.in_channels, device=device))
            else:
                rows.append(torch.ones(n * self.in_channels, device=device))
        return torch.cat(rows)

    def forward(self, x, masks=None):
        if not isinstance(x, torch.Tensor) or x.dim() != 4 or x.shape[1] != self.in_channels:
            raise ValueError('expected a [N, {}, H, W] tensor'.format(self.in_channels))
        if not x.is_cuda:
            raise RuntimeError('rcu_amd.model.PostNet only runs on the GPU (librcu_hip); got a {} tensor'.format(x.device))
        n, c, h, w = x.shape
        if masks is None:
            masks = self.sample_masks(n, x.device)
        elif isinstance(masks, (list, tuple)):
            if len(masks) != self.nb_convs:
                raise ValueError('expected {} dropout masks, got {}'.format(self.nb_convs, len(masks)))
            masks = torch.cat([torch.as_tensor(m, dtype=torch.float32).reshape(n * c) for m in masks]).to(x.device)
        if masks is not None:
            masks = masks.to(torch.float32).contiguous()
            if masks.numel() != self.nb_convs * n * c:
                raise ValueError('dropout masks must hold nb_convs x N x C factors')
        cp = (c + 31) // 32 * 32
        nhwc = x.permute(0, 2, 3, 1)
        pitch = nhwc.stride(2)
        in_place = (x.dtype == torch.float32 and nhwc.stride(3) == 1 and pitch >= cp and pitch % 4 == 0 and
                    nhwc.stride(1) == w * pitch and nhwc.stride(0) == h * w * pitch and x.data_ptr() % 16 == 0)
        if not in_place:
            pitch = cp
            buf = torch.zeros((n, h, w, pitch), device=x.device, dtype=torch.float32)
            buf[..., :c] = nhwc
            nhwc = buf
        logits = torch.empty((n, self.nb_classes, h, w), device=x.device, dtype=torch.float32)
        _lib.check(_lib.load().rcu_postnet_forward(self._handle(), ctypes.c_void_p(nhwc.data_ptr()), pitch, n, h * w,
                                                   _lib.ptr(masks), _lib.ptr(logits), _lib.current_stream()))
        return logits


model_registry = {'unet': UNet, 'postnet': PostNet}


def get_model(model_type, **params):
    return model_registry[model_type](**params)
```

Before: 189.1 MC-sample-volumes/s.

## Share first-unit output planes across MC passes for channels unaffected by dropout

Adds a shared per-image copy of the first conv unit's output, stored with the all-kept dropout scale. A small kernel builds per-sample bitmasks marking which 8-channel chunks have every mask value equal to the keep scale. The first conv skips storing those chunks for each MC pass, and a new specialised Winograd-4 kernel for the single reader layer redirects its loads of those chunks to the shared planes. The goal is to cut write and read traffic on the largest activation tensor. In exchange it adds an extra mask-scan kernel launch, a more complex DMA resource setup, and a new option path that the Python defaults turn on.

```diff
diff --git a/reliability-challenges-uncertainty_amd/csrc/rcu_api.hip b/reliability-challenges-uncertainty_amd/csrc/rcu_api.hip
--- a/reliability-challenges-uncertainty_amd/csrc/rcu_api.hip
+++ b/reliability-challenges-uncertainty_amd/csrc/rcu_api.hip
@@ -63,6 +63,7 @@
     int Hr = 0, Wr = 0;
     bool padded() const { return H != Hr || W != Wr; }
     bool blocked = false;
+    int batch_div = 1;
 };
 
 struct Workspace {
@@ -90,6 +91,7 @@
     int in_cp = 0, head_cp = 0, head_cph = 0;
     int t_input = -1, t_head = -1;
     int t_features = -1;
+    int t_share = -1, t_share_bits = -1, share_reader = -1;
     std::map<std::string, std::vector<float>> host_weights;
     float *w_cls = nullptr, *b_cls = nullptr, *w_sig = nullptr, *b_sig = nullptr;
     double temperature = 1.0;
@@ -244,6 +246,7 @@
 }
 
 static void assign_layouts(rcu_unet* h);
+static void plan_shared_first(rcu_unet* h);
 
 static bool cfg_handles_padding(int cfg) { return conv_config_info(cfg).family.part; }
 
@@ -352,6 +355,7 @@
         if ((src_padded || first_reads_caller || out_padded) && !cfg_handles_padding(L.cfg) && valid) *valid = false;
     }
     assign_layouts(h);
+    plan_shared_first(h);
     return RCU_OK;
 }
 
@@ -445,6 +449,43 @@
     }
 }
 
+static bool layer_runs_part(const rcu_unet* h, const ConvLayer& L)
+{
+    if (!cfg_handles_padding(L.cfg)) return false;
+    const Tensor &tsrc = h->tensors[L.t_src1], &tout = h->tensors[L.t_out];
+    const int os = L.upsample ? 2 : 1;
+    const bool pool_differs = L.t_pool >= 0 && (h->tensors[L.t_pool].H != L.gh / 2 || h->tensors[L.t_pool].W != L.gw / 2);
+    return tsrc.padded() || tout.H != os * L.gh || tout.W != os * L.gw || pool_differs;
+}
+
+static void plan_shared_first(rcu_unet* h)
+{
+    h->t_share = h->t_share_bits = h->share_reader = -1;
+    if (h->opt.conv_first != 1 || h->d.max_batch < 2 || h->layers.size() < 3) return;
+    const ConvLayer& F = h->layers.front();
+    if (F.cfg != CONV_CFG_FIRST_T8x32 || F.site < 0 || F.t_src1 != h->t_input || F.coutp / 8 > 8 || layer_runs_part(h, F)) return;
+    const Tensor& to = h->tensors[F.t_out];
+    if (!to.blocked || to.padded() || F.t_out == h->t_head || F.t_out == h->layers.back().t_src1) return;
+    int reader = -1, readers = 0;
+    for (size_t i = 1; i < h->layers.size(); ++i) {
+        const ConvLayer& L = h->layers[i];
+        if (L.t_out == F.t_out || L.t_pool == F.t_out) return;
+        if (L.t_src1 == F.t_out || L.t_src2 == F.t_out) {
+            ++readers;
+            reader = (int)i;
+        }
+    }
+    if (readers != 1 || reader + 1 == (int)h->layers.size()) return;
+    const ConvLayer& R = h->layers[reader];
+    if (R.cfg != CONV_CFG_WINO4_T32x32_N32 || R.t_src1 != F.t_out || R.t_src2 >= 0 || layer_runs_part(h, R)) return;
+    h->share_reader = reader;
+    h->t_share = new_tensor(h, 0, to.Hr, to.Wr, to.cp);
+    h->tensors[h->t_share].blocked = true;
+    h->tensors[h->t_share].batch_div = 2;
+    const ConvConfigInfo& rci = conv_config_info(R.cfg);
+    h->t_share_bits = new_tensor(h, -1, 1, 1, 2 + R.NT * (R.gh / rci.TH) * (R.gw / rci.TW));
+}
+
 extern "C" const char* rcu_last_error(void) { return g_last_error.c_str(); }
 extern "C" const char* rcu_version(void) { return "librcu_hip 0.1.0 gfx950"; }
 
@@ -479,7 +520,7 @@
     if (opts) {
         o = *opts;
         if ((o.conv_winograd | 1) != 1 || (o.conv_winograd4 < 0 || o.conv_winograd4 > 3) ||
-            (o.conv_first | 1) != 1 || (o.act_layout | 1) != 1 || (o.fuse_head | 1) != 1 || (o.head_winograd4 | 1) != 1 || (o.pad_levels | 1) != 1 ||
+            (o.conv_first < 0 || o.conv_first > 2) || (o.act_layout | 1) != 1 || (o.fuse_head | 1) != 1 || (o.head_winograd4 | 1) != 1 || (o.pad_levels | 1) != 1 ||
             (o.upconv_winograd4 < 0 || o.upconv_winograd4 > 2))
             return fail(RCU_ERR_INVALID, "rcu_unet_create_with: bad rcu_unet_options value");
     }
@@ -519,7 +560,7 @@
         for (size_t i = 0; same && i < h->tensors.size(); ++i) {
             const Tensor &a = h->tensors[i], &b = donor->tensors[i];
             same = a.floats_per_slice == b.floats_per_slice && a.H == b.H && a.W == b.W && a.Hr == b.Hr && a.Wr == b.Wr && a.cp == b.cp &&
-                   a.blocked == b.blocked && a.zero_fill == b.zero_fill;
+                   a.blocked == b.blocked && a.zero_fill == b.zero_fill && a.batch_div == b.batch_div;
         }
         if (!same) {
             delete h;
@@ -535,7 +576,7 @@
     h->ws->max_batch = d.max_batch;
     bool zeroed = false;
     for (Tensor& t : h->tensors) {
-        const size_t bytes = t.floats_per_slice * (size_t)d.max_batch * sizeof(float);
+        const size_t bytes = t.floats_per_slice * (size_t)((d.max_batch + t.batch_div - 1) / t.batch_div) * sizeof(float);
         hipError_t e = hipMalloc(reinterpret_cast<void**>(&t.dev), bytes);
         if (e != hipSuccess) {
             rcu_unet_destroy(h);
@@ -800,6 +841,27 @@
     a.src1_bytes = (uint32_t)std::min<size_t>(h->tensors[L.t_src1].floats_per_slice * (size_t)n * 4, 0xFFFFFFFFu);
     a.src2_bytes = L.t_src2 >= 0 ? (uint32_t)std::min<size_t>(h->tensors[L.t_src2].floats_per_slice * (size_t)n * 4, 0xFFFFFFFFu) : 0u;
     a.wpack_bytes = (uint32_t)std::min<size_t>(L.wpack_floats * 4, 0xFFFFFFFFu);
+    if (h->t_share >= 0 && x_nchw != nullptr && masks != nullptr && n_images > 0 && n % n_images == 0 && n / n_images >= 2 &&
+        (&L == &h->layers.front() || &L == &h->layers[h->share_reader])) {
+        const ConvLayer& F = h->layers.front();
+        const ConvLayer& R = h->layers[h->share_reader];
+        const ConvConfigInfo& rci = conv_config_info(R.cfg);
+        uint32_t* const bits = reinterpret_cast<uint32_t*>(h->tensors[h->t_share_bits].dev);
+        uint32_t* const items = bits + 2 * (size_t)h->d.max_batch;
+        a.share_planes = h->tensors[h->t_share].dev;
+        a.share_bits = bits;
+        a.share_items = items;
+        if (&L == &F) {
+            RCU_HIP(launch_share_bits(a.mask, n, a.Cmask, L.coutp / 8, bits, items, R.NT * (R.gh / rci.TH) * (R.gw / rci.TW), n_images,
+                                      (uint32_t)(h->tensors[F.t_out].floats_per_slice * 4), stream));
+        } else {
+            a.n_images = n_images;
+            a.share_passes = n / n_images;
+            a.share_bytes = (uint32_t)(h->tensors[h->t_share].floats_per_slice * (size_t)n_images * 4);
+            const unsigned long long items = (unsigned long long)a.NTW_total * a.tiles_x * a.tiles_y * a.slice_groups;
+            a.magic_share_passes = items * (unsigned long long)a.share_passes < (1ull << 32) ? (uint32_t)(((1ull << 32) + a.share_passes - 1) / a.share_passes) : 0u;
+        }
+    }
     int cfg = L.cfg;
     if (head) {
         cfg = ci.head_cfg;
diff --git a/reliability-challenges-uncertainty_amd/csrc/rcu_first.hip b/reliability-challenges-uncertainty_amd/csrc/rcu_first.hip
--- a/reliability-challenges-uncertainty_amd/csrc/rcu_first.hip
+++ b/reliability-challenges-uncertainty_amd/csrc/rcu_first.hip
@@ -78,37 +78,89 @@
                     for (int b = 0; b < NB; ++b) acc[seg][b] = __builtin_amdgcn_mfma_f32_16x16x4f32(wr[tap][ks][b], xv, acc[seg][b], 0, 0, 0);
                 }
         }
-        for (int pass = 0; pass < passes; ++pass) {
-            const int ns = pass * images + n;
+        auto store_tile = [&](float* dst, int ns, const f32x4 (&mk)[NB], uint32_t skip) {
             f32x4 scale[NB], shift[NB];
 #pragma unroll
             for (int b = 0; b < NB; ++b) {
-                f32x4 mk = {1.f, 1.f, 1.f, 1.f};
-                if (a.mask != nullptr) {
-#pragma unroll
-                    for (int j = 0; j < 4; ++j) {
-                        const int c = b * 16 + 4 * g + j;
-                        if (c < a.Cmask) mk[j] = a.mask[(size_t)ns * a.Cmask + c];
-                    }
-                }
-                scale[b] = al[b] * mk;
-                shift[b] = bb[b] * mk + be[b];
+                scale[b] = al[b] * mk[b];
+                shift[b] = bb[b] * mk[b] + be[b];
             }
 #pragma unroll
             for (int seg = 0; seg < 4; ++seg) {
                 const int r = 2 * wave + (seg >> 1), c0 = 16 * (seg & 1);
                 if (y0 + r >= Hr || x0 + c0 + n16 >= Wr) continue;
-                char* const op = reinterpret_cast<char*>(a.out) + (size_t)ns * a.H * a.W * a.CoutP * 4 +
+                char* const op = reinterpret_cast<char*>(dst) + (size_t)ns * a.H * a.W * a.CoutP * 4 +
                                  (size_t)((y0 + r) * a.W + x0 + c0 + n16) * a.out_pix_bytes + (size_t)(g >> 1) * a.out_chunk_bytes + (g & 1) * 16;
 #pragma unroll
                 for (int b = 0; b < NB; ++b) {
+                    if ((skip >> (2 * b + (g >> 1))) & 1u) continue;
                     f32x4 v = acc[seg][b] * scale[b] + shift[b];
 #pragma unroll
                     for (int j = 0; j < 4; ++j) v[j] = fmaxf(v[j], floor_v);
                     *reinterpret_cast<f32x4*>(op + (size_t)(2 * b) * a.out_chunk_bytes) = v;
                 }
             }
-        }
+        };
+        const bool share = a.share_planes != nullptr;
+        if (share) {
+            const float keep = __builtin_bit_cast(float, a.share_bits[a.N]);
+            f32x4 mk[NB];
+#pragma unroll
+            for (int b = 0; b < NB; ++b)
+#pragma unroll
+                for (int j = 0; j < 4; ++j) mk[b][j] = b * 16 + 4 * g + j < a.Cmask ? keep : 1.f;
+            store_tile(a.share_planes, n, mk, 0u);
+        }
+        for (int pass = 0; pass < passes; ++pass) {
+            const int ns = pass * images + n;
+            f32x4 mk[NB];
+#pragma unroll
+            for (int b = 0; b < NB; ++b) {
+                mk[b] = f32x4{1.f, 1.f, 1.f, 1.f};
+                if (a.mask != nullptr) {
+#pragma unroll
+                    for (int j = 0; j < 4; ++j) {
+                        const int c = b * 16 + 4 * g + j;
+                        if (c < a.Cmask) mk[b][j] = a.mask[(size_t)ns * a.Cmask + c];
+                    }
+                }
+            }
+            store_tile(a.out, ns, mk, share ? a.share_bits[ns] : 0u);
+        }
+    }
+}
+
+constexpr int SHARE_THREADS = 1024;
+__global__ __launch_bounds__(SHARE_THREADS) void share_bits_kernel(const uint32_t* __restrict__ mask, int N, int Cmask, int chunks, uint32_t* bits,
+                                                                   uint32_t* __restrict__ items, int items_per_sample, int n_images, uint32_t sample_bytes)
+{
+    __shared__ uint32_t top;
+    if (threadIdx.x == 0) top = 0u;
+    __syncthreads();
+    uint32_t m = 0u;
+    for (int i = threadIdx.x; i < N * Cmask; i += SHARE_THREADS) m = max(m, mask[i]);
+    for (int d = 32; d > 0; d >>= 1) m = max(m, (uint32_t)__shfl_xor((int)m, d));
+    if ((threadIdx.x & 63) == 0) atomicMax(&top, m);
+    __syncthreads();
+    const uint32_t keep = top;
+    for (int n = threadIdx.x; n < N; n += SHARE_THREADS) {
+        uint32_t w = 0u;
+        for (int c = 0; c < chunks; ++c) {
+            bool same = true;
+            for (int k = 0; k < 8; ++k) {
+                const int ch = 8 * c + k;
+                if (ch < Cmask && mask[(size_t)n * Cmask + ch] != keep) same = false;
+            }
+            w |= (same ? 1u : 0u) << c;
+        }
+        bits[n] = w;
+    }
+    if (threadIdx.x == 0) bits[N] = keep;
+    __syncthreads();
+    const int passes = N / n_images;
+    for (int i = threadIdx.x; i < N * items_per_sample; i += SHARE_THREADS) {
+        const int pass = i % passes, image = i / passes / items_per_sample;
+        items[i] = (uint32_t)(pass * n_images) * sample_bytes | bits[pass * n_images + image];
     }
 }
 
@@ -133,9 +185,23 @@
     if (a.C1 != 8 || a.C2 != 0 || a.H % FIRST_TH != 0 || a.W % FIRST_TW != 0 || a.pooled != nullptr || a.mask2 != nullptr ||
         (a.CoutP != 32 && a.CoutP != 64))
         return hipErrorInvalidValue;
+    if (a.share_planes != nullptr && (a.share_bits == nullptr || a.mask == nullptr || a.x_nchw == nullptr || a.n_images < 1 || a.N % a.n_images != 0 ||
+                                      a.N / a.n_images < 2 || a.part || a.out_pix_bytes != 32u))
+        return hipErrorInvalidValue;
     const bool wide = a.cin_real > 4;
     if (a.CoutP == 32) return wide ? launch_first<2, 2>(a, stream) : launch_first<1, 2>(a, stream);
     return wide ? launch_first<2, 4>(a, stream) : launch_first<1, 4>(a, stream);
 }
 
-}
+hipError_t launch_share_bits(const float* mask, int N, int Cmask, int chunks, uint32_t* bits, uint32_t* items, int items_per_sample, int n_images,
+                             uint32_t sample_bytes, hipStream_t stream)
+{
+    if (mask == nullptr || bits == nullptr || items == nullptr || N < 1 || Cmask < 1 || chunks < 1 || chunks > 8 || items_per_sample < 1 || n_images < 1 ||
+        N % n_images != 0 || sample_bytes % 256u != 0u || (unsigned long long)N * sample_bytes >= (1ull << 31))
+        return hipErrorInvalidValue;
+    hipLaunchKernelGGL(share_bits_kernel, dim3(1), dim3(SHARE_THREADS), 0, stream, reinterpret_cast<const uint32_t*>(mask), N, Cmask, chunks, bits, items,
+                       items_per_sample, n_images, sample_bytes);
+    return hipGetLastError();
+}
+
+}
diff --git a/reliability-challenges-uncertainty_amd/csrc/rcu_kernels.h b/reliability-challenges-uncertainty_amd/csrc/rcu_kernels.h
--- a/reliability-challenges-uncertainty_amd/csrc/rcu_kernels.h
+++ b/reliability-challenges-uncertainty_amd/csrc/rcu_kernels.h
@@ -74,7 +74,15 @@
     size_t head_V;
     int head_passes;
     int head_images;
-};
+    float* share_planes;
+    const uint32_t* share_bits;
+    const uint32_t* share_items;
+    uint32_t share_bytes;
+    int share_passes;
+    uint32_t magic_share_passes;
+};
+hipError_t launch_share_bits(const float* mask, int N, int Cmask, int chunks, uint32_t* bits, uint32_t* items, int items_per_sample, int n_images,
+                             uint32_t sample_bytes, hipStream_t stream);
 
 enum ConvConfig {
     CONV_CFG_T8x16_N64 = 0,
diff --git a/reliability-challenges-uncertainty_amd/csrc/rcu_wino4.hip b/reliability-challenges-uncertainty_amd/csrc/rcu_wino4.hip
--- a/reliability-challenges-uncertainty_amd/csrc/rcu_wino4.hip
+++ b/reliability-challenges-uncertainty_amd/csrc/rcu_wino4.hip
@@ -374,8 +374,8 @@
 __host__ __device__ constexpr int wino4_row_of(int k) { return k == 0 ? 0 : k == 1 ? 5 : k - 1; }
 __host__ __device__ constexpr int wino4_pos_of(int q) { return 6 * wino4_row_of(q / 6) + q % 6; }
 
-template <class T, bool HEAD = false, bool PART = false>
-__global__ __launch_bounds__(256, 1) void conv_wino4_stream(const ConvArgs a, const int total_items)
+template <class T, bool HEAD, bool PART, bool SHARE>
+__device__ __forceinline__ void conv_wino4_body(const ConvArgs& a, const int total_items)
 {
 #if defined(__HIP_DEVICE_COMPILE__)
     extern __shared__ __attribute__((aligned(1024))) float smem[];
@@ -391,7 +391,7 @@
 
     const __amdgpu_buffer_rsrc_t rs1 = __builtin_amdgcn_make_buffer_rsrc(const_cast<float*>(a.src1), 0, a.src1_bytes, 0x00020000);
     const __amdgpu_buffer_rsrc_t rs2 =
-        __builtin_amdgcn_make_buffer_rsrc(const_cast<float*>(a.src2 ? a.src2 : a.src1), 0, a.src2 ? a.src2_bytes : 0u, 0x00020000);
+        SHARE ? rs1 : __builtin_amdgcn_make_buffer_rsrc(const_cast<float*>(a.src2 ? a.src2 : a.src1), 0, a.src2 ? a.src2_bytes : 0u, 0x00020000);
     const __amdgpu_buffer_rsrc_t rsw = __builtin_amdgcn_make_buffer_rsrc(const_cast<float*>(a.wpack), 0, a.wpack_bytes, 0x00020000);
 
     int aCol[2][6];
@@ -423,7 +423,21 @@
         return false;
     };
     bool has_next = more_passes() || item + (int)gridDim.x < total_items;
-    WinoTileId tile = wino_tile_id<T>(a, item), ntile = tile;
+    static_assert(!SHARE || (T::TS == 1 && T::TH == 32 && !HEAD && !PART), "the plain one-slice 32x32 tile");
+    [[maybe_unused]] const float* const share_ptr = a.share_planes;
+    [[maybe_unused]] const uint32_t share_bytes = a.share_bytes;
+    [[maybe_unused]] const __attribute__((address_space(4))) uint32_t* const share_items =
+        reinterpret_cast<const __attribute__((address_space(4))) uint32_t*>((uintptr_t)a.share_items);
+    [[maybe_unused]] uint32_t shf = 0u, shb = 0u;
+    WinoTileId tile, ntile;
+    if constexpr (SHARE) {
+        int p;
+        tile = wino_tile_id_passes<T>(a, item, a.share_passes, a.magic_share_passes, a.n_images, p);
+        shf = shb = share_items[item];
+    } else {
+        tile = wino_tile_id<T>(a, item);
+    }
+    ntile = tile;
     uint32_t dp[T::NA], dpn[T::NA], geo[T::NA];
     int dp_wtile = tile.wtile, dpn_wtile = tile.wtile;
 #pragma unroll
@@ -440,11 +454,16 @@
         __amdgpu_buffer_rsrc_t rs;
         uint32_t cb, wso, lb;
     };
-    auto dma_job = [&](int wtile, int kc, int buf, bool active) {
+    auto dma_job = [&](int wtile, int kc, int buf, bool active, [[maybe_unused]] uint32_t sh) {
         DmaJob j;
         const int c0 = kc * KC;
-        const bool first = c0 < a.C1;
+        const bool first = SHARE || c0 < a.C1;
         j.rs = first ? rs1 : rs2;
+        if constexpr (SHARE) {
+            const uint32_t back = sh & ~255u;
+            if (((sh >> kc) & 1u) != 0u)
+                j.rs = __builtin_amdgcn_make_buffer_rsrc(reinterpret_cast<float*>((uintptr_t)share_ptr - (uintptr_t)back), 0, share_bytes + back, 0x00020000);
+        }
         j.cb = active ? wino_chunk_offset(in_chunk_bytes, first ? c0 : c0 - a.C1) : WINO_OOB;
         j.wso = active ? (uint32_t)kc * wchunk_bytes + (uint32_t)wtile * (T::W_DW * 4u) : WINO_OOB;
         j.lb = (uint32_t)buf * (T::BUF_DW * 4u);
@@ -469,7 +488,7 @@
     constexpr int PB = (T::TS == 1 && T::TH == 32) ? 4 : 0;
     static_assert(PB <= T::NA, "the back part consists of input pieces");
     {
-        const DmaJob job = dma_job(dp_wtile, 0, 0, true);
+        const DmaJob job = dma_job(dp_wtile, 0, 0, true, shf);
         wino_static_for<0, T::NW + T::NA>([&](auto i_c) { dma_piece(job, dp, i_c); });
     }
     if constexpr (HEAD) {
@@ -478,7 +497,7 @@
     __builtin_amdgcn_s_waitcnt(0x0F70);
     __syncthreads();
     {
-        const DmaJob job = dma_job(dp_wtile, 1, 1, true);
+        const DmaJob job = dma_job(dp_wtile, 1, 1, true, shf);
         wino_static_for<0, PB>([&](auto i_c) { dma_piece(job, dp, i_c); });
     }
 
@@ -560,10 +579,20 @@
         const float* const An = smem + (BUF ^ 1) * T::BUF_DW;
         const bool more = kc + 1 < nchunks, more2 = kc + 2 < nchunks;
         if (kc == nchunks - 2 && has_next) {
+            [[maybe_unused]] int sh_passes = 0, sh_images = 0;
+            [[maybe_unused]] uint32_t sh_magic = 0u;
+            if constexpr (SHARE) {
+                const ConvArgs& c = wino_cold_args();
+                sh_passes = c.share_passes, sh_images = c.n_images, sh_magic = c.magic_share_passes;
+                shb = share_items[item + (int)gridDim.x];
+            }
             const WinoTileConsts ca = wino_tile_consts(wino_cold_args());
             if (more_passes()) {
                 ntile = tile;
                 ntile.n0 = tile.n0 + wino_cold_args().head_images;
+            } else if constexpr (SHARE) {
+                int p;
+                ntile = wino_tile_id_passes<T>(ca, item + (int)gridDim.x, sh_passes, sh_magic, sh_images, p);
             } else {
                 ntile = wino_tile_id<T>(ca, item + (int)gridDim.x);
             }
@@ -574,12 +603,13 @@
         }
         if (!more) {
             dp_wtile = dpn_wtile;
+            shf = shb;
 #pragma unroll
             for (int j = 0; j < T::NA; ++j) dp[j] = dpn[j];
         }
         if (kc == nchunks - 2) epr = wino4_epilogue_load<T>(wino_cold_args(), tile.wtile, tile.n0, wave, lane);
-        const DmaJob job = dma_job(dp_wtile, more ? kc + 1 : 0, BUF ^ 1, more || has_next);
-        const DmaJob jobb = dma_job(dpn_wtile, more2 ? kc + 2 : kc + 2 - nchunks, BUF, more2 || has_next);
+        const DmaJob job = dma_job(dp_wtile, more ? kc + 1 : 0, BUF ^ 1, more || has_next, shf);
+        const DmaJob jobb = dma_job(dpn_wtile, more2 ? kc + 2 : kc + 2 - nchunks, BUF, more2 || has_next, shb);
         transform_head(d);
         wino_static_for<0, 18>([&](auto g_c) {
             constexpr int G = decltype(g_c)::value;
@@ -673,6 +703,12 @@
 #endif
 }
 
+template <class T, bool HEAD = false, bool PART = false>
+__global__ __launch_bounds__(256, 1) void conv_wino4_stream(const ConvArgs a, const int total_items)
+{
+    conv_wino4_body<T, HEAD, PART, false>(a, total_items);
+}
+
 using W4Cfg0 = Wino4Tile<1, 2, 8, 1, 4>;
 using W4Cfg1 = Wino4Tile<1, 2, 8, 2, 2>;
 using W4Cfg2 = Wino4Tile<2, 2, 4, 4, 1, true>;
@@ -691,6 +727,21 @@
 };
 
 const ConvConfigInfo& wino4_config_info(int cfg) { return kWino4Info[cfg - CONV_CFG_WINO4_T32x32_N32]; }
+
+__global__ __launch_bounds__(256, 1) void conv_wino4_shared_first(const ConvArgs a, const int total_items)
+{
+    conv_wino4_body<W4Cfg0, false, false, true>(a, total_items);
+}
+
+static hipError_t launch_wino4_shared_first(const ConvArgs& a, hipStream_t stream)
+{
+    using T = W4Cfg0;
+    hipError_t e = set_max_dynamic_lds(reinterpret_cast<const void*>(&conv_wino4_shared_first), T::LDS_BYTES);
+    if (e != hipSuccess) return e;
+    const unsigned items = (unsigned)a.NT * a.tiles_x * a.tiles_y * a.slice_groups;
+    hipLaunchKernelGGL(conv_wino4_shared_first, dim3(wino_persistent_grid(items)), dim3(T::THREADS), T::LDS_BYTES, stream, a, (int)items);
+    return hipGetLastError();
+}
 
 template <class T, bool HEAD, bool PART>
 static hipError_t launch_wino4_kernel(const ConvArgs& a, hipStream_t stream)
@@ -721,6 +772,13 @@
                    (size_t)a.N * a.out_H * a.out_W * a.CoutP * 4 >= ((size_t)1 << 31) ||
                    (a.pooled != nullptr && (a.pool_H < (a.Hr >> 1) || a.pool_W < (a.Wr >> 1)))))
         return hipErrorInvalidValue;
+    if (a.share_planes != nullptr) {
+        if (HEAD || T::TS != 1 || T::TH != 32 || a.part || a.C2 != 0 || nchunks > 8 || a.share_items == nullptr || a.in_pix_bytes != 32u || a.share_passes < 2 ||
+            a.n_images < 1 || a.n_images * a.share_passes != a.N || (size_t)a.share_bytes * a.share_passes != (size_t)a.src1_bytes ||
+            ((size_t)a.H * a.W * a.C1 * 4) % 256 != 0)
+            return hipErrorInvalidValue;
+        return launch_wino4_shared_first(a, stream);
+    }
     if (a.part) return launch_wino4_kernel<T, HEAD, true>(a, stream);
     return launch_wino4_kernel<T, HEAD, false>(a, stream);
 }
diff --git a/reliability-challenges-uncertainty_amd/csrc/rcu_wino_common.h b/reliability-challenges-uncertainty_amd/csrc/rcu_wino_common.h
--- a/reliability-challenges-uncertainty_amd/csrc/rcu_wino_common.h
+++ b/reliability-challenges-uncertainty_amd/csrc/rcu_wino_common.h
@@ -163,6 +163,17 @@
     return t;
 }
 
+template <class T, class A>
+__device__ __forceinline__ WinoTileId wino_tile_id_passes(const A& a, int item, int passes, uint32_t magic_passes, int n_images, int& pass)
+{
+    static_assert(T::TS == 1, "a slice group is a sample");
+    const int rest = magic_passes ? (int)__umulhi((uint32_t)item, magic_passes) : item / passes;
+    WinoTileId t = wino_tile_id<T>(a, rest);
+    pass = item - rest * passes;
+    t.n0 += pass * n_images;
+    return t;
+}
+
 constexpr int WINO_POS_DW = 4;
 template <class T>
 __device__ __forceinline__ uint32_t wino_slot_geometry(int j, int wave, int lane)
diff --git a/reliability-challenges-uncertainty_amd/model.py b/reliability-challenges-uncertainty_amd/model.py
--- a/reliability-challenges-uncertainty_amd/model.py
+++ b/reliability-challenges-uncertainty_amd/model.py
@@ -42,7 +42,8 @@
     DEFAULT_START_FILTERS = 16
     DEFAULT_DROPOUT = 0.2
     MAX_HANDLES = 6
-    PLAN_DEFAULTS = dict(conv_winograd=1, conv_winograd4=1, conv_first=1, act_layout=0, head_winograd4=1, pad_levels=1, upconv_winograd4=1)
+    PLAN_DEFAULTS = dict(conv_winograd=1, conv_winograd4=1, conv_first=1, act_layout=0, head_winograd4=1, pad_levels=1, upconv_winograd4=1,
+                         share_first_unit=1)
     _generations = itertools.count(1)
 
     def __init__(self, nb_classes, in_channels, depth=DEFAULT_DEPTH, start_filters=DEFAULT_START_FILTERS,
@@ -191,7 +192,10 @@
                              dropout_center=-1 if self.dropout_center is None else int(self.dropout_center),
                              sigma_out=int(self.sigma_out), bn=int(self.bn), height=h, width=w, max_batch=max_batch,
                              residual=int(self.residual), provide_features=int(bool(self.provide_features)))
-        opts = _lib.UnetOptions(fuse_head=int(self.fuse_head), **options)
+        fields = {k: v for k, v in options.items() if k != 'share_first_unit'}
+        if fields['conv_first'] == 1 and not options['share_first_unit']:
+            fields['conv_first'] = 2
+        opts = _lib.UnetOptions(fuse_head=int(self.fuse_head), **fields)
         handle = ctypes.c_void_p()
         _lib.check(lib.rcu_unet_create_with(ctypes.byref(desc), ctypes.byref(opts), donor_handle, ctypes.byref(handle)))
         try:
```

New measurement: 189.7 MC-sample-volumes/s, median of 6. No clear change (+0.3%).
